# tkwa/iit

Hardware: AMD Instinct MI355X
Metric: IIT (base,source) intervened pairs/sec, IOI GPT-2-small, IOI_ModelPair IIT+strict+behavior step (higher is better)
Workload: dtype bf16; 1 GPU; model=gpt2-small 12L/768d/12H (TL GPT-2 cfg, LNPre, gelu_new, V=50257), global_batch=256, seq_len=16, parallelism=dp1, engine=native, graphs=True

## Files before the change

csrc/gemm_glds_body.h:

```cpp
#pragma once
#include <type_traits>

#include "common.h"

namespace {

enum : int { E_BF16 = 0, E_BF16_BIAS3 = 1, E_F32_RESID = 2, E_GELU = 3, E_DGELU = 4, E_F32_ACC = 5,
             E_F32_STORE = 7, E_GELU_ERF = 8, E_DGELU_ERF = 9, E_BF16_CS = 10 };

struct G2Args {
  const __bf16* A;
  const __bf16* B;
  void* C;
  void* C2;
  const float* bias0;
  const float* bias1;
  const float* bias2;
  const float* resid;
  long lda, ldb, ldc, ldc2, ldr;
  int M, N, K, bias_cols;
  int k_per_split;
  float* csum;
  float* ws;
  int* counters;
// ... 90 lines not shown
};

__device__ __forceinline__ unsigned lds_addr(const char* p) {
  return (unsigned)(uintptr_t)(const __attribute__((address_space(3))) char*)p;
}

template <bool KMAJ, int R>
struct Panels {
  static constexpr bool ON = KMAJ && (R > 128 || R % 64 != 0);
  static constexpr int PR = !ON ? R : (R % 64 == 0 ? 64 : 32);
  static constexpr int NP = R / PR;
};

template <bool KMAJ, int R, int NW = 4, int BK = 64, bool LEAN = false>
struct OperandStager {
  static constexpr bool PANELS = Panels<KMAJ, R>::ON;
  static constexpr int NP = Panels<KMAJ, R>::NP;
  static constexpr int PR = Panels<KMAJ, R>::PR;
  static constexpr int N = NP * Stager<KMAJ, PR, NW, BK, LEAN>::N;
  Stager<KMAJ, PR, NW, BK, LEAN> st[NP];

  __device__ __forceinline__ void init(const __bf16* base, long ld, int r0g, int kbeg, int wave, int lane) {
#pragma unroll
    for (int q = 0; q < NP; ++q) st[q].init(base, ld, r0g + q * PR, kbeg, wave, lane);
  }
  __device__ __forceinline__ void stage(int kt, char* img) const {
#pragma unroll
    for (int q = 0; q < NP; ++q) st[q].stage(kt, img + q * PR * BK * 2);
  }
};

typedef int i32x4 __attribute__((ext_vector_type(4)));
template <bool KMAJ> struct RawFrag;
template <> struct RawFrag<false> { i32x4 v; };
template <> struct RawFrag<true> { i16x4 lo, hi; };

template <bool KMAJ, int R, int BK = 64>
__device__ __forceinline__ void frag_issue(const char* img, int row0, int kbase, int lane, RawFrag<KMAJ>& f) {
  if constexpr (!KMAJ) {
    const int row = row0 + (lane & 15);
    const int c = (kbase >> 3) + (lane >> 4);
    const unsigned a = lds_addr(img + row * (BK * 2) + ((c ^ kcont_swz<BK>(row)) << 4));
    asm volatile("ds_read_b128 %0, %1" : "=v"(f.v) : "v"(a));
  } else {
    const int g = lane >> 4, q = (lane >> 2) & 3, pp = lane & 3;
    const int kr = kbase + 8 * g + q;
    const int col = row0 + 4 * pp;
    const unsigned a0 = lds_addr(img + kr * (R * 2) + ((((col >> 4) ^ kmaj_swz<R>(kr))) << 5) + ((col & 15) << 1));
    asm volatile("ds_read_b64_tr_b16 %0, %1" : "=v"(f.lo) : "v"(a0));
    asm volatile("ds_read_b64_tr_b16 %0, %1 offset:%2" : "=v"(f.hi) : "v"(a0), "i"(4 * R * 2));
  }
}

template <bool KMAJ, int R, int BK = 64>
__device__ __forceinline__ void frag_issue_t(const char* img, int row0, int kbase, int lane, RawFrag<KMAJ>& f) {
  using PN = Panels<KMAJ, R>;
  if constexpr (PN::ON) {
    frag_issue<KMAJ, PN::PR, BK>(img + (row0 / PN::PR) * PN::PR * BK * 2, row0 % PN::PR, kbase, lane, f);
  } else {
    frag_issue<KMAJ, R, BK>(img, row0, kbase, lane, f);
  }
}

template <bool KMAJ>
__device__ __forceinline__ bf16x8 frag_use(const RawFrag<KMAJ>& f) {
  if constexpr (!KMAJ) {
    return __builtin_bit_cast(bf16x8, f.v);
  } else {
    const i16x8 w = __builtin_shufflevector(f.lo, f.hi, 0, 1, 2, 3, 4, 5, 6, 7);
    return __builtin_bit_cast(bf16x8, w);
  }
}

template <bool TR>
__device__ __forceinline__ f32x4 mfma_tile(const bf16x8 a, const bf16x8 b, const f32x4 c) {
  if constexpr (TR) return __builtin_amdgcn_mfma_f32_16x16x32_bf16(b, a, c, 0, 0, 0);
  else return __builtin_amdgcn_mfma_f32_16x16x32_bf16(a, b, c, 0, 0, 0);
}

__device__ __forceinline__ int xcd_remap(int bid, int nwg) {
  const int xcd = bid % 8;
  const int q = nwg / 8, r = nwg % 8;
  return (xcd < r ? xcd * (q + 1) : r * (q + 1) + (xcd - r) * q) + bid / 8;
}

__device__ __forceinline__ void grouped_tile(int t, int tiles_m, int tiles_n, int& tm, int& tn, int GM = 8) {
  const int per_group = GM * tiles_n;
  const int first_m = (t / per_group) * GM;
  const int gsize = min(tiles_m - first_m, GM);
  const int r = t % per_group;
  tm = first_m + r % gsize;
  tn = r / gsize;
}

__device__ __forceinline__ float gelu_new_dev(float x) { return gelu_new_f(x); }

__device__ __forceinline__ void add8v(float* v, const float4 x, const float4 y) {
  v[0] += x.x; v[1] += x.y; v[2] += x.z; v[3] += x.w;
  v[4] += y.x; v[5] += y.y; v[6] += y.z; v[7] += y.w;
}

__device__ __forceinline__ void add8(float* v, const float* b) {
  const float4 x = *(const float4*)b, y = *(const float4*)(b + 4);
  v[0] += x.x; v[1] += x.y; v[2] += x.z; v[3] += x.w;
  v[4] += y.x; v[5] += y.y; v[6] += y.z; v[7] += y.w;
}

__device__ __forceinline__ void store16(void* dst, const f32x4 x, int mode) {
  if (mode == 1) {
    __builtin_nontemporal_store(x, (f32x4*)dst);
  } else if (mode == 2) {
    asm volatile("global_store_dwordx4 %0, %1, off sc1" ::"v"(dst), "v"(x) : "memory");
  } else {
    *(f32x4*)dst = x;
  }
}

__device__ __forceinline__ void store8_bf16(void* dst, const float* v, int mode = 0) {
  bf16x8 o;
#pragma unroll
  for (int e = 0; e < 8; ++e) o[e] = f2bf(v[e]);
  store16(dst, __builtin_bit_cast(f32x4, o), mode);
}

__device__ __forceinline__ void store8_f32(void* dst, const float* v, int mode = 0) {
  store16(dst, f32x4{v[0], v[1], v[2], v[3]}, mode);
  store16((float*)dst + 4, f32x4{v[4], v[5], v[6], v[7]}, mode);
}

template <int L>
__device__ __forceinline__ void wait_tiles(int tiles_in_flight) {
  constexpr int CAP = 63 / L;
  if (tiles_in_flight > CAP) tiles_in_flight = CAP;
  if (tiles_in_flight >= 7) asm volatile("s_waitcnt vmcnt(%0)" ::"n"((7 * L) < 63 ? 7 * L : 63) : "memory");
  else if (tiles_in_flight == 6) asm volatile("s_waitcnt vmcnt(%0)" ::"n"((6 * L) < 63 ? 6 * L : 63) : "memory");
  else if (tiles_in_flight == 5) asm volatile("s_waitcnt vmcnt(%0)" ::"n"((5 * L) < 63 ? 5 * L : 63) : "memory");
  else if (tiles_in_flight == 4) asm volatile("s_waitcnt vmcnt(%0)" ::"n"((4 * L) < 63 ? 4 * L : 63) : "memory");
  else if (tiles_in_flight == 3) asm volatile("s_waitcnt vmcnt(%0)" ::"n"((3 * L) < 63 ? 3 * L : 63) : "memory");
  else if (tiles_in_flight == 2) asm volatile("s_waitcnt vmcnt(%0)" ::"n"(2 * L) : "memory");
  else if (tiles_in_flight == 1) asm volatile("s_waitcnt vmcnt(%0)" ::"n"(L) : "memory");
  else asm volatile("s_waitcnt vmcnt(0)" ::: "memory");
}

template <int BM, int BN, int NS, int NW, int BK, int OCC>
struct GldsSmem {
  static constexpr int STAGE = (BM + BN) * BK * 2;
  static constexpr int EPS = BN + 4;
  static constexpr int LDS_BUDGET = 160 * 1024 / OCC;
  static constexpr int ECH = BM * EPS * 4 > LDS_BUDGET ? 2 : 1;
  static constexpr int EPI_BYTES = BM / ECH * EPS * 4;
  static constexpr int BYTES = NS * STAGE > EPI_BYTES ? NS * STAGE : EPI_BYTES;
};

template <int BM, int BN, int EPI, int NT, int ECH, int EPS, class WriteAcc>
__device__ __forceinline__ void glds_epilogue(const G2Args& p, char* smem, const int m0, const int n0, const int lin,
                                              WriteAcc&& write_acc) {
  const int tid = threadIdx.x, lane = tid & 63, wave = tid >> 6;
  constexpr int NW = NT / 64;
  float* E = (float*)smem;
  constexpr int ER = BM / ECH;
  constexpr int CPR = BN / 8;
  constexpr int ITEMS = (ER * CPR + NT - 1) / NT;
  constexpr bool PF32 = EPI == E_F32_RESID || EPI == E_F32_ACC;
  constexpr bool PF16 = EPI == E_DGELU || EPI == E_DGELU_ERF;
  float sq = 0.f;
  float cpiv = 0.f, cs1 = 0.f, cs2 = 0.f;
  for (int ch = 0; ch < ECH; ++ch) {
  float4 pf[PF32 ? 2 * ITEMS : 1];
  bf16x8 pb[PF16 ? ITEMS : 1];
#pragma unroll
  for (int k = 0; k < ITEMS; ++k) {
    const int id = tid + k * NT;
    if (id < ER * CPR) {
      const int row = m0 + ch * ER + id / CPR, col = n0 + (id % CPR) * 8;
      if constexpr (EPI == E_F32_RESID) {
        const float* src = p.resid + (long)row * p.ldr + col;
        pf[2 * k] = *(const float4*)src;
        pf[2 * k + 1] = *(const float4*)(src + 4);
      } else if constexpr (EPI == E_F32_ACC) {
        const float* src = (const float*)p.C + (long)row * p.ldc + col;
        pf[2 * k] = *(const float4*)src;
        pf[2 * k + 1] = *(const float4*)(src + 4);
      } else if constexpr (PF16) {
        pb[k] = *(const bf16x8*)((const __bf16*)p.C2 + (long)row * p.ldc2 + col);
      }
    }
  }
  __syncthreads();
  write_acc(E, ch);
  __syncthreads();
#pragma unroll
  for (int k = 0; k < ITEMS; ++k) {
    const int id = tid + k * NT;
    if (id >= ER * CPR) break;
    const int lr = id / CPR, lc = (id % CPR) * 8;
    const int row = m0 + ch * ER + lr, col = n0 + lc;
    float v[8];
    {
      const float4 x = *(const float4*)(E + lr * EPS + lc), y = *(const float4*)(E + lr * EPS + lc + 4);
      v[0] = x.x; v[1] = x.y; v[2] = x.z; v[3] = x.w; v[4] = y.x; v[5] = y.y; v[6] = y.z; v[7] = y.w;
    }
    if constexpr (EPI == E_BF16) {
      if (p.bias0) add8(v, p.bias0 + col);
      store8_bf16((__bf16*)p.C + (long)row * p.ldc + col, v, p.store_mode);
    } else if constexpr (EPI == E_BF16_CS) {
      if (p.bias0) add8(v, p.bias0 + col);
      store8_bf16((__bf16*)p.C + (long)row * p.ldc + col, v, p.store_mode);
#pragma unroll
      for (int e = 0; e < 8; ++e) v[e] = bf2f(f2bf(v[e]));
      *(float4*)(E + lr * EPS + lc) = make_float4(v[0], v[1], v[2], v[3]);
      *(float4*)(E + lr * EPS + lc + 4) = make_float4(v[4], v[5], v[6], v[7]);
    } else if constexpr (EPI == E_BF16_BIAS3) {
      const int w = col / p.bias_cols, o = col - w * p.bias_cols;
      const float* bb = w == 0 ? p.bias0 : (w == 1 ? p.bias1 : p.bias2);
      if (bb) add8(v, bb + o);
      store8_bf16((__bf16*)p.C + (long)row * p.ldc + col, v, p.store_mode);
    } else if constexpr (EPI == E_F32_RESID) {
      if (p.bias0) add8(v, p.bias0 + col);
      add8v(v, pf[2 * k], pf[2 * k + 1]);
      store8_f32((float*)p.C + (long)row * p.ldc + col, v, p.store_mode);
    } else if constexpr (EPI == E_GELU || EPI == E_GELU_ERF) {
      if (p.bias0) add8(v, p.bias0 + col);
      if (p.C2) store8_bf16((__bf16*)p.C2 + (long)row * p.ldc2 + col, v, p.store_mode);
      float g[8];
#pragma unroll
      for (int e = 0; e < 8; ++e) {
        const float x = bf2f(f2bf(v[e]));
        g[e] = EPI == E_GELU ? gelu_new_dev(x) : gelu_erf_f(x);
      }
      store8_bf16((__bf16*)p.C + (long)row * p.ldc + col, g, p.store_mode);
    } else if constexpr (EPI == E_DGELU || EPI == E_DGELU_ERF) {
      const bf16x8 pr = pb[k];
#pragma unroll
      for (int e = 0; e < 8; ++e) {
        const float x = bf2f(pr[e]);
        v[e] = bf2f(f2bf(v[e] * (EPI == E_DGELU ? gelu_new_grad_f(x) : gelu_erf_grad_f(x))));
      }
      store8_bf16((__bf16*)p.C + (long)row * p.ldc + col, v, p.store_mode);
      if (p.csum) {
        *(float4*)(E + lr * EPS + lc) = make_float4(v[0], v[1], v[2], v[3]);
        *(float4*)(E + lr * EPS + lc + 4) = make_float4(v[4], v[5], v[6], v[7]);
      }
    } else if constexpr (EPI == E_F32_ACC) {
      float* dst = (float*)p.C + (long)row * p.ldc + col;
      add8v(v, pf[2 * k], pf[2 * k + 1]);
      store8_f32(dst, v, p.store_mode);
    } else {
      if (p.bias0) add8(v, p.bias0 + col);
      store8_f32((float*)p.C + (long)row * p.ldc + col, v, p.store_mode);
      if (p.gsq) {
#pragma unroll
        for (int e = 0; e < 8; ++e) sq += v[e] * v[e];
      }
    }
  }
  if constexpr (EPI == E_DGELU || EPI == E_DGELU_ERF) {
    if (p.csum) {
      __syncthreads();
      constexpr int G = NT / BN > 0 ? NT / BN : 1;
      for (int c = tid; c < BN * G; c += NT) {
        const int col = c % BN, g = c / BN;
        float s[8] = {0.f, 0.f, 0.f, 0.f, 0.f, 0.f, 0.f, 0.f};
#pragma unroll
        for (int r0 = g; r0 < ER; r0 += 8 * G)
#pragma unroll
          for (int u = 0; u < 8; ++u)
            if (r0 + u * G < ER) s[u] += E[(r0 + u * G) * EPS + col];
        atomicAdd(p.csum + n0 + col, ((s[0] + s[1]) + (s[2] + s[3])) + ((s[4] + s[5]) + (s[6] + s[7])));
      }
    }
  }
  if constexpr (EPI == E_BF16_CS) {
    __syncthreads();
    static_assert(NT % BN == 0, "column groups");
    constexpr int G = NT / BN;
    const int col = tid % BN, g = tid / BN;
    if (ch == 0) cpiv = E[col];
    for (int r = g; r < ER; r += G) {
      const float d = E[r * EPS + col] - cpiv;
      cs1 += d;
      cs2 = __builtin_fmaf(d, d, cs2);
    }
  }
  }
  if constexpr (EPI == E_BF16_CS) {
    constexpr int G = NT / BN;
    float* red = (float*)smem;
    __syncthreads();
    red[tid] = cs1;
    red[NT + tid] = cs2;
    __syncthreads();
    if (tid < BN) {
      float a = 0.f, b = 0.f;
#pragma unroll
      for (int g = 0; g < G; ++g) {
        a += red[g * BN + tid];
        b += red[NT + g * BN + tid];
      }
      const long T = p.M / BM, tm = m0 / BM, c = n0 + tid;
      p.cstat[c * T + tm] = cpiv;
      p.cstat[((long)p.N + c) * T + tm] = a;
      p.cstat[(2L * p.N + c) * T + tm] = b;
    }
  }
  if constexpr (EPI == E_F32_STORE) {
    if (p.gsq) {
      sq = wave_sum(sq);
      float* red = (float*)smem;
      __syncthreads();
      if (lane == 0) red[wave] = sq;
      __syncthreads();
      if (tid == 0) {
        float t = 0.f;
#pragma unroll
        for (int w = 0; w < NW; ++w) t += red[w];
        atomicAdd(p.gsq + (lin & 63), t);
      }
    }
  }
}

template <int BM, int BN, int NS, bool AKM, bool BKM, int EPI, int NW, int BK = 64, int OCC = 1, bool LEAN = false,
          class ASTG = void, class BSTG = void>
__device__ __forceinline__ void gemm_glds_body(const G2Args& p, const int lin, const int nlin, const int split,
                                               const int nsplit, char* smem) {
  using SA = std::conditional_t<std::is_void_v<ASTG>, OperandStager<AKM, BM, NW, BK, LEAN>, ASTG>;
  using SB = std::conditional_t<std::is_void_v<BSTG>, OperandStager<BKM, BN, NW, BK, LEAN>, BSTG>;
  constexpr int HALVES = BK / 64;
  constexpr int NT = NW * 64;
  constexpr int WMR = NW / 2;
  constexpr int WM = BM / WMR, WN = BN / 2;
  constexpr int TM = WM / 16, TN = WN / 16;
  constexpr int A_BYTES = BM * BK * 2, B_BYTES = BN * BK * 2;
  constexpr int STAGE = A_BYTES + B_BYTES;
  constexpr int LOADS = SA::N + SB::N;
  using SM = GldsSmem<BM, BN, NS, NW, BK, OCC>;
  constexpr int EPS = SM::EPS;
  constexpr int ECH = SM::ECH;
  static_assert(SM::BYTES <= SM::LDS_BUDGET, "LDS budget");
  static_assert(STAGE == SM::STAGE, "stage size");

  constexpr bool TR = EPI != E_F32_ACC;
  const int tid = threadIdx.x, lane = tid & 63, wave = tid >> 6;
  const int wm = wave >> 1, wn = wave & 1;
  const int tiles_n = p.N / BN;
  const int t = xcd_remap(lin, nlin);
  int tm, tn;
  grouped_tile(t, p.M / BM, tiles_n, tm, tn, p.group_m > 0 ? p.group_m : 8);
  const int m0 = tm * BM, n0 = tn * BN;
  const int kbeg = split * p.k_per_split;
  const int nt = p.k_per_split / BK;
  const bool prof_on = p.prof != nullptr && tid == 0;
  const int prof_slot = split * nlin + lin;
  if (prof_on) {
    p.prof[(long)prof_slot * 64 + 63] = wall_clock64();
    prof_mark(p.prof, prof_slot, 0, true);
  }

  f32x4 acc[TM][TN];
  constexpr bool CS = AKM && BKM && (EPI == E_F32_ACC || EPI == E_F32_STORE);
  const bool do_cs = CS && p.bsum != nullptr && tm == 0 && wm == 0;
  float cs[CS ? TN : 1];
#pragma unroll
  for (int j = 0; j < (CS ? TN : 1); ++j) cs[j] = 0.f;
#pragma unroll
  for (int i = 0; i < TM; ++i)
#pragma unroll
    for (int j = 0; j < TN; ++j) acc[i][j] = f32x4{0.f, 0.f, 0.f, 0.f};

  RawFrag<AKM> ca[TM], na[TM];
  RawFrag<BKM> cb[TN], nb[TN];
  SA stA;
  SB stB;
  if constexpr (std::is_void_v<ASTG>) stA.init(p.A, p.lda, m0, kbeg, wave, lane);
  else stA.init(p, m0, kbeg, wave, lane);
  if constexpr (std::is_void_v<BSTG>) stB.init(p.B, p.ldb, n0, kbeg, wave, lane);
  else stB.init(p, n0, kbeg, wave, lane);
#pragma unroll
  for (int s = 0; s < NS; ++s)
    if (s < nt) {
      char* buf = smem + s * STAGE;
      stA.stage(s, buf);
      stB.stage(s, buf + A_BYTES);
    }
  wait_tiles<LOADS>(min(NS - 1, nt - 1));
  __builtin_amdgcn_s_barrier();
  prof_mark(p.prof, prof_slot, 1, prof_on);
#pragma unroll
  for (int i = 0; i < TM; ++i) frag_issue_t<AKM, BM, BK>(smem, wm * WM + i * 16, 0, lane, ca[i]);
#pragma unroll
  for (int j = 0; j < TN; ++j) frag_issue_t<BKM, BN, BK>(smem + A_BYTES, wn * WN + j * 16, 0, lane, cb[j]);

  for (int kt = 0; kt < nt; ++kt) {
    const char* sa = smem + (kt % NS) * STAGE;
    const char* sb = sa + A_BYTES;
#pragma unroll
    for (int h = 0; h < HALVES; ++h) {
    asm volatile("s_waitcnt lgkmcnt(0)" ::: "memory");
    __builtin_amdgcn_sched_barrier(0);
#pragma unroll
    for (int i = 0; i < TM; ++i) frag_issue_t<AKM, BM, BK>(sa, wm * WM + i * 16, h * 64 + 32, lane, na[i]);
#pragma unroll
    for (int j = 0; j < TN; ++j) frag_issue_t<BKM, BN, BK>(sb, wn * WN + j * 16, h * 64 + 32, lane, nb[j]);
    __builtin_amdgcn_sched_barrier(0);
    {
      bf16x8 a[TM], b[TN];
#pragma unroll
      for (int i = 0; i < TM; ++i) a[i] = frag_use<AKM>(ca[i]);
#pragma unroll
      for (int j = 0; j < TN; ++j) b[j] = frag_use<BKM>(cb[j]);
#pragma unroll
      for (int i = 0; i < TM; ++i)
#pragma unroll
        for (int j = 0; j < TN; ++j) acc[i][j] = mfma_tile<TR>(a[i], b[j], acc[i][j]);
      if constexpr (CS) {
        if (do_cs) {
#pragma unroll
          for (int j = 0; j < TN; ++j) {
            const i32x4 w = __builtin_bit_cast(i32x4, b[j]);
            float t = 0.f;
#pragma unroll
            for (int q = 0; q < 4; ++q)
              t += __builtin_bit_cast(float, (unsigned)w[q] << 16) + __builtin_bit_cast(float, (unsigned)w[q] & 0xffff0000u);
            cs[j] += t;
          }
        }
      }
    }
    __builtin_amdgcn_sched_barrier(0);
    asm volatile("s_waitcnt lgkmcnt(0)" ::: "memory");
    __builtin_amdgcn_sched_barrier(0);
    if (h + 1 < HALVES) {
#pragma unroll
      for (int i = 0; i < TM; ++i) frag_issue_t<AKM, BM, BK>(sa, wm * WM + i * 16, (h + 1) * 64, lane, ca[i]);
#pragma unroll
      for (int j = 0; j < TN; ++j) frag_issue_t<BKM, BN, BK>(sb, wn * WN + j * 16, (h + 1) * 64, lane, cb[j]);
    } else if (kt + 1 < nt) {
      wait_tiles<LOADS>(min(NS - 2, nt - 2 - kt));
      __builtin_amdgcn_s_barrier();
      if (kt + 2 < 61) prof_mark(p.prof, prof_slot, kt + 2, prof_on);
      if (kt + NS < nt) {
        char* buf = smem + (kt % NS) * STAGE;
        stA.stage(kt + NS, buf);
        stB.stage(kt + NS, buf + A_BYTES);
      }
      const char* ta = smem + ((kt + 1) % NS) * STAGE;
#pragma unroll
      for (int i = 0; i < TM; ++i) frag_issue_t<AKM, BM, BK>(ta, wm * WM + i * 16, 0, lane, ca[i]);
#pragma unroll
      for (int j = 0; j < TN; ++j) frag_issue_t<BKM, BN, BK>(ta + A_BYTES, wn * WN + j * 16, 0, lane, cb[j]);
    }
    __builtin_amdgcn_sched_barrier(0);
    {
      bf16x8 a[TM], b[TN];
#pragma unroll
      for (int i = 0; i < TM; ++i) a[i] = frag_use<AKM>(na[i]);
#pragma unroll
      for (int j = 0; j < TN; ++j) b[j] = frag_use<BKM>(nb[j]);
#pragma unroll
      for (int i = 0; i < TM; ++i)
#pragma unroll
        for (int j = 0; j < TN; ++j) acc[i][j] = mfma_tile<TR>(a[i], b[j], acc[i][j]);
      if constexpr (CS) {
        if (do_cs) {
#pragma unroll
          for (int j = 0; j < TN; ++j) {
            const i32x4 w = __builtin_bit_cast(i32x4, b[j]);
            float t = 0.f;
#pragma unroll
            for (int q = 0; q < 4; ++q)
              t += __builtin_bit_cast(float, (unsigned)w[q] << 16) + __builtin_bit_cast(float, (unsigned)w[q] & 0xffff0000u);
            cs[j] += t;
          }
        }
      }
    }
    __builtin_amdgcn_sched_barrier(0);
    }
  }
  prof_mark(p.prof, prof_slot, 61, prof_on);
  if constexpr (CS) {
    if (do_cs) {
#pragma unroll
      for (int j = 0; j < TN; ++j) {
        float v = cs[j];
        v += __shfl_xor(v, 16);
        v += __shfl_xor(v, 32);
        if (lane < 16) atomicAdd(p.bsum + n0 + wn * WN + j * 16 + lane, v);
      }
    }
  }
  if constexpr (EPI == E_F32_ACC || EPI == E_F32_STORE || EPI == E_F32_RESID || EPI == E_BF16 || EPI == E_BF16_CS) {
    if (p.ws != nullptr) {
      const long tile_elems = (long)BM * BN;
      f32x4* mine = (f32x4*)(p.ws + ((long)split * nlin + t) * tile_elems);
#pragma unroll
      for (int i = 0; i < TM; ++i)
#pragma unroll
        for (int j = 0; j < TN; ++j)
          asm volatile("global_store_dwordx4 %0, %1, off sc1" ::"v"(mine + (i * TN + j) * NT + tid), "v"(acc[i][j])
                       : "memory");
      asm volatile("s_waitcnt vmcnt(0)" ::: "memory");
      __syncthreads();
      int* flag = (int*)smem;
      if (tid == 0) {
        const int last = atomicAdd(p.counters + t, 1) == nsplit - 1;
        if (last) __hip_atomic_store(p.counters + t, 0, __ATOMIC_RELAXED, __HIP_MEMORY_SCOPE_AGENT);
        flag[0] = last;
      }
      __syncthreads();
      if (!flag[0]) return;
      f32x4 sum[TM][TN];
#pragma unroll
      for (int i = 0; i < TM; ++i)
#pragma unroll
        for (int j = 0; j < TN; ++j) sum[i][j] = f32x4{0.f, 0.f, 0.f, 0.f};
      for (int sp = 0; sp < nsplit; ++sp) {
        if (sp == split) {
#pragma unroll
          for (int i = 0; i < TM; ++i)
#pragma unroll
            for (int j = 0; j < TN; ++j) sum[i][j] += acc[i][j];
          continue;
        }
        const f32x4* other = (const f32x4*)(p.ws + ((long)sp * nlin + t) * tile_elems);
        f32x4 v[TM][TN];
#pragma unroll
        for (int i = 0; i < TM; ++i)
#pragma unroll
          for (int j = 0; j < TN; ++j)
            asm volatile("global_load_dwordx4 %0, %1, off sc1" : "=v"(v[i][j]) : "v"(other + (i * TN + j) * NT + tid)
                         : "memory");
        asm volatile("s_waitcnt vmcnt(0)" ::: "memory");
#pragma unroll
        for (int i = 0; i < TM; ++i)
#pragma unroll
          for (int j = 0; j < TN; ++j) sum[i][j] += v[i][j];
      }
#pragma unroll
      for (int i = 0; i < TM; ++i)
#pragma unroll
        for (int j = 0; j < TN; ++j) acc[i][j] = sum[i][j];
    }
  }
  if constexpr (EPI == E_F32_ACC) {
    if (nsplit > 1 && p.ws == nullptr) {
#pragma unroll
      for (int i = 0; i < TM; ++i)
#pragma unroll
        for (int j = 0; j < TN; ++j) {
          const int col = n0 + wn * WN + j * 16 + (lane & 15);
          const int row = m0 + wm * WM + i * 16 + 4 * (lane >> 4);
#pragma unroll
          for (int r = 0; r < 4; ++r) unsafeAtomicAdd((float*)p.C + (long)(row + r) * p.ldc + col, acc[i][j][r]);
        }
      return;
    }
  }
  glds_epilogue<BM, BN, EPI, NT, ECH, SM::EPS>(p, smem, m0, n0, lin, [&](float* E, int ch) {
    if (wm / (WMR / ECH) == ch) {
#pragma unroll
      for (int i = 0; i < TM; ++i)
#pragma unroll
        for (int j = 0; j < TN; ++j) {
          if constexpr (TR) {
            const int col = wn * WN + j * 16 + 4 * (lane >> 4);
            const int row = (wm % (WMR / ECH)) * WM + i * 16 + (lane & 15);
            *(f32x4*)(E + row * EPS + col) = acc[i][j];
          } else {
            const int col = wn * WN + j * 16 + (lane & 15);
            const int row = (wm % (WMR / ECH)) * WM + i * 16 + 4 * (lane >> 4);
#pragma unroll
            for (int r = 0; r < 4; ++r) E[(row + r) * EPS + col] = acc[i][j][r];
          }
        }
    }
  });
  if (p.prof != nullptr) {
    asm volatile("s_waitcnt vmcnt(0)" ::: "memory");
    __syncthreads();
    prof_mark(p.prof, prof_slot, 62, prof_on);
    if (prof_on) p.prof[(long)prof_slot * 64 + 60] = wall_clock64();
  }
}

}
```

csrc/kernels.hip:

```cpp
#include "common.h"
#include <stdlib.h>

__global__ void embed_pos_fwd_kernel(const long* __restrict__ tok, const float* __restrict__ WE,
                                     const float* __restrict__ Wpos, float* __restrict__ out, int T, int S, int d) {
  const int t = blockIdx.x;
  if (t >= T) return;
  const long v = tok[t];
  const int s = t % S;
  const float4* e = (const float4*)(WE + v * (long)d);
  const float4* p = (const float4*)(Wpos + (long)s * d);
  float4* o = (float4*)(out + (long)t * d);
  for (int i = threadIdx.x; i < d / 4; i += blockDim.x) {
    float4 a = e[i], b = p[i];
    o[i] = make_float4(a.x + b.x, a.y + b.y, a.z + b.z, a.w + b.w);
  }
}

IIT_EXPORT int iit_embed_pos_fwd(const long* tok, const float* WE, const float* Wpos, float* out, int T, int S,
                                 int d, void* stream) {
  hipLaunchKernelGGL(embed_pos_fwd_kernel, dim3(T), dim3(d >= 256 ? 64 : 64), 0, (hipStream_t)stream, tok, WE, Wpos,
                     out, T, S, d);
  return hipGetLastError();
}

// ... 815 lines not shown
  const int P = dh + 1, SP = S + 1;
  float* q = sm;
  float* k = q + S * P;
  float* v = k + S * P;
  float* g = v + S * P;
  float* pm = g + S * P;
  float* ds = pm + S * SP;
  for (int i = lane; i < S * dh; i += 64) {
    const int s = i / dh, e = i % dh;
    const __bf16* r = qkv + (row0 + s) * ld_qkv + h * dh + e;
    q[s * P + e] = bf2f(r[0]);
    k[s * P + e] = bf2f(r[HD]);
    v[s * P + e] = bf2f(r[2 * HD]);
    g[s * P + e] = bf2f(dz[(row0 + s) * ld_dz + h * dh + e]);
  }
  __syncthreads();
  for (int i = lane; i < S * S; i += 64) {
    const int qi = i / S, kj = i % S;
    float p = 0.f, dp = 0.f;
    if (!causal || kj <= qi) {
      float sc = 0.f;
      for (int e = 0; e < dh; ++e) sc += q[qi * P + e] * k[kj * P + e];
      p = __expf(sc * scale - lse[(long)bh * S + qi]);
      for (int e = 0; e < dh; ++e) dp += g[qi * P + e] * v[kj * P + e];
    }
    pm[qi * SP + kj] = p;
    ds[qi * SP + kj] = dp;
  }
  __syncthreads();
  for (int qi = lane; qi < S; qi += 64) {
    float dsum = 0.f;
    for (int kj = 0; kj < S; ++kj) dsum += pm[qi * SP + kj] * ds[qi * SP + kj];
    for (int kj = 0; kj < S; ++kj) ds[qi * SP + kj] = pm[qi * SP + kj] * (ds[qi * SP + kj] - dsum) * scale;
  }
  __syncthreads();
  for (int i = lane; i < S * dh; i += 64) {
    const int s = i / dh, e = i % dh;
    float dq = 0.f, dk = 0.f, dv = 0.f;
    for (int j = 0; j < S; ++j) {
      dq += ds[s * SP + j] * k[j * P + e];
      dk += ds[j * SP + s] * q[j * P + e];
      dv += pm[j * SP + s] * g[j * P + e];
    }
    __bf16* r = dqkv + (row0 + s) * ld_qkv + h * dh + e;
    r[0] = f2bf(dq);
    r[HD] = f2bf(dk);
    r[2 * HD] = f2bf(dv);
  }
}

IIT_EXPORT int iit_attn_small_bwd(const void* qkv, const void* dz, const float* lse, void* dqkv,
                                  unsigned long long head_mask, int B, int S, int H, int dh, long ld_qkv, long ld_dz,
                                  float scale, int causal, void* stream) {
  if (S > 64 || dh > 128) return (int)hipErrorInvalidValue;
  const size_t lds = (size_t)(4 * S * (dh + 1) + 2 * S * (S + 1)) * sizeof(float);
  if (lds > kAttnSmallLdsMax) return (int)hipErrorInvalidValue;
  hipLaunchKernelGGL(attn_small_bwd_kernel, dim3(B * H), dim3(64), lds, (hipStream_t)stream, (const __bf16*)qkv,
                     (const __bf16*)dz, lse, (__bf16*)dqkv, head_mask, B, S, H, dh, ld_qkv, ld_dz, scale, causal);
  return hipGetLastError();
}

__device__ __forceinline__ void online_add(float& m, float& s, int& mi, float v, int i) {
  if (v > m) {
    s = s * __expf(m - v) + 1.f;
    m = v;
    mi = i;
  } else {
    s += __expf(v - m);
  }
}

__device__ __forceinline__ void online_merge(float& m, float& s, int& mi, float om, float os, int oi) {
  if (om > m || (om == m && oi < mi)) {
    s = os + (m == -INFINITY ? 0.f : s * __expf(m - om));
    m = om;
    mi = oi;
  } else {
    s += (om == -INFINITY ? 0.f : os * __expf(om - m));
  }
}

__global__ __launch_bounds__(1024) void ce_fwd_kernel(const float* __restrict__ logits, long ld, const long* __restrict__ labels,
                                                      float* __restrict__ loss, float* __restrict__ lse_out,
                                                      long* __restrict__ amax, int V) {
  __shared__ float sm_m[16], sm_s[16];
  __shared__ int sm_i[16];
  const int row = blockIdx.x, tid = threadIdx.x, lane = tid & 63, w = tid >> 6;
  const float* x = logits + (long)row * ld;
  float m = -INFINITY, s = 0.f;
  int mi = 0x7fffffff;
  int head = 0;
  if ((((uintptr_t)x) & 15) == 0) {
    const int v4 = V / 4;
    for (int i = tid; i < v4; i += 1024) {
      const float4 q = ((const float4*)x)[i];
      online_add(m, s, mi, q.x, 4 * i);
      online_add(m, s, mi, q.y, 4 * i + 1);
      online_add(m, s, mi, q.z, 4 * i + 2);
      online_add(m, s, mi, q.w, 4 * i + 3);
    }
    head = v4 * 4;
  }
  for (int i = head + tid; i < V; i += 1024) online_add(m, s, mi, x[i], i);
#pragma unroll
  for (int o = 32; o > 0; o >>= 1) {
    const float om = __shfl_xor(m, o, 64), os = __shfl_xor(s, o, 64);
    const int oi = __shfl_xor(mi, o, 64);
    online_merge(m, s, mi, om, os, oi);
  }
  if (lane == 0) { sm_m[w] = m; sm_s[w] = s; sm_i[w] = mi; }
  __syncthreads();
  if (tid == 0) {
    for (int j = 1; j < 16; ++j) online_merge(m, s, mi, sm_m[j], sm_s[j], sm_i[j]);
    const float l = m + __logf(s);
    if (lse_out) lse_out[row] = l;
    if (loss && labels) loss[row] = l - x[labels[row]];
    if (amax) amax[row] = mi;
  }
}

IIT_EXPORT int iit_ce_fwd(const float* logits, long ld, const long* labels, float* loss, float* lse, long* amax, int R,
                          int V, void* stream) {
  hipLaunchKernelGGL(ce_fwd_kernel, dim3(R), dim3(1024), 0, (hipStream_t)stream, logits, ld, labels, loss, lse, amax, V);
  return hipGetLastError();
}

template <typename OUT>
__global__ __launch_bounds__(256) void ce_bwd_kernel(const float* __restrict__ logits, long ld, const long* __restrict__ labels,
                                                     const float* __restrict__ lse, const float* __restrict__ gscale,
                                                     float inv_rows, OUT* __restrict__ out, long ld_out, int V,
                                                     __bf16* __restrict__ out16) {
  const int row = blockIdx.y;
  const int i = blockIdx.x * 256 + threadIdx.x;
  if (i >= ld_out) return;
  float v = 0.f;
  if (i < V) {
    const float p = __expf(logits[(long)row * ld + i] - lse[row]);
    v = (p - (i == labels[row] ? 1.f : 0.f)) * gscale[0] * inv_rows;
  }
  out[(long)row * ld_out + i] = (OUT)v;
  if (out16) out16[(long)row * ld_out + i] = f2bf(v);
}

IIT_EXPORT int iit_ce_bwd(const float* logits, long ld, const long* labels, const float* lse, const float* gscale,
                          float inv_rows, void* out, long ld_out, int R, int V, int out_bf16, void* out16,
                          void* stream) {
  dim3 grid((unsigned)((ld_out + 255) / 256), R);
  if (out_bf16)
    hipLaunchKernelGGL(ce_bwd_kernel<__bf16>, grid, dim3(256), 0, (hipStream_t)stream, logits, ld, labels, lse, gscale,
                       inv_rows, (__bf16*)out, ld_out, V, (__bf16*)nullptr);
  else
    hipLaunchKernelGGL(ce_bwd_kernel<float>, grid, dim3(256), 0, (hipStream_t)stream, logits, ld, labels, lse, gscale,
                       inv_rows, (float*)out, ld_out, V, (__bf16*)out16);
  return hipGetLastError();
}

struct Span {
  long start4;
  long local4;
  int len4;
  int pad;
};

__global__ __launch_bounds__(256) void sumsq_span_kernel(const float* __restrict__ g, const Span* __restrict__ spans,
                                                         int nspans, float* __restrict__ part, int do_norm,
                                                         int* __restrict__ step, float* __restrict__ gsq) {
  __shared__ float sm[4];
  if (blockIdx.x == 0 && threadIdx.x == 0 && step) step[0] += 1;
  float s = 0.f;
  if (gsq && blockIdx.x == 0 && threadIdx.x < 64) {
    s = gsq[threadIdx.x];
    gsq[threadIdx.x] = 0.f;
  }
  if (!do_norm) return;
  const float4* g4 = (const float4*)g;
  for (int e = blockIdx.x; e < nspans; e += gridDim.x) {
    const Span sp = spans[e];
    for (int i = threadIdx.x; i < sp.len4; i += 256) {
      const float4 v = g4[sp.local4 + i];
      s += (v.x * v.x + v.y * v.y) + (v.z * v.z + v.w * v.w);
    }
  }
  s = wave_sum(s);
  if ((threadIdx.x & 63) == 0) sm[threadIdx.x >> 6] = s;
  __syncthreads();
  if (threadIdx.x == 0) part[blockIdx.x] = sm[0] + sm[1] + sm[2] + sm[3];
}

template <bool NT, int U>
__global__ __launch_bounds__(256) void adam_span_kernel(float* __restrict__ p, const float* __restrict__ g,
                                                        float* __restrict__ m, float* __restrict__ v,
                                                        __bf16* __restrict__ mirror, const Span* __restrict__ spans,
                                                        int nspans, const float* __restrict__ part, int nparts,
                                                        float clip, float lr, float b1, float b2, float eps, float wd,
                                                        const float* __restrict__ hyper, int* __restrict__ step,
                                                        int* __restrict__ skipped) {
  if (hyper) {
    lr = hyper[0];
    b1 = hyper[1];
    b2 = hyper[2];
    eps = hyper[3];
    wd = hyper[4];
  }
  __shared__ float coef_s;
  __shared__ int bad_s;
  if (threadIdx.x < 64) {
    float s = 0.f;
    if (clip > 0.f || skipped)
      for (int i = threadIdx.x; i < nparts; i += 64) s += part[i];
    s = wave_sum(s);
    if (threadIdx.x == 0) {
      coef_s = clip > 0.f ? fminf(1.f, clip / (sqrtf(s) + 1e-6f)) : 1.f;
      bad_s = skipped != nullptr && !isfinite(s);
    }
  }
  __syncthreads();
  if (bad_s) {
    if (blockIdx.x == 0 && threadIdx.x == 0) {
      step[0] -= 1;
      skipped[0] += 1;
    }
    return;
  }
  const float coef = coef_s;
  const float t = (float)step[0];
  const float bc1 = 1.f - powf(b1, t);
  const float bc2_sqrt = sqrtf(1.f - powf(b2, t));
  const float stepsz = lr / bc1;
  const float4* g4 = (const float4*)g;
  float4* p4 = (float4*)p;
  float4* m4 = (float4*)m;
  float4* v4 = (float4*)v;
  for (int e = blockIdx.x; e < nspans; e += gridDim.x) {
    const Span sp = spans[e];
    for (int j0 = threadIdx.x; j0 < sp.len4; j0 += 256 * U) {
      float4 gg[U], pp[U], mm[U], vv[U];
#pragma unroll
      for (int u = 0; u < U; ++u) {
        const int j = j0 + u * 256;
        if (j < sp.len4) {
          const long i = sp.start4 + j;
          const long li = sp.local4 + j;
          pp[u] = p4[i];
          if (NT) {
            gg[u] = __builtin_bit_cast(float4, __builtin_nontemporal_load((const f32x4*)g4 + li));
            mm[u] = __builtin_bit_cast(float4, __builtin_nontemporal_load((const f32x4*)m4 + li));
            vv[u] = __builtin_bit_cast(float4, __builtin_nontemporal_load((const f32x4*)v4 + li));
          } else {
            gg[u] = g4[li];
            mm[u] = m4[li];
            vv[u] = v4[li];
          }
        }
      }
#pragma unroll
      for (int u = 0; u < U; ++u) {
        const int j = j0 + u * 256;
        if (j >= sp.len4) break;
        const long i = sp.start4 + j;
        const long li = sp.local4 + j;
        float* gs = (float*)&gg[u];
        float* ps = (float*)&pp[u];
        float* ms = (float*)&mm[u];
        float* vs = (float*)&vv[u];
#pragma unroll
        for (int k = 0; k < 4; ++k) {
          float gr = gs[k] * coef;
          if (wd != 0.f) gr += wd * ps[k];
          ms[k] = b1 * ms[k] + (1.f - b1) * gr;
          vs[k] = b2 * vs[k] + (1.f - b2) * gr * gr;
          ps[k] -= stepsz * ms[k] / (sqrtf(vs[k]) / bc2_sqrt + eps);
        }
        p4[i] = pp[u];
        if (NT) {
          __builtin_nontemporal_store(__builtin_bit_cast(f32x4, mm[u]), (f32x4*)m4 + li);
          __builtin_nontemporal_store(__builtin_bit_cast(f32x4, vv[u]), (f32x4*)v4 + li);
        } else {
          m4[li] = mm[u];
          v4[li] = vv[u];
        }
        if (mirror) {
          bf16x4 o = {f2bf(ps[0]), f2bf(ps[1]), f2bf(ps[2]), f2bf(ps[3])};
          ((bf16x4*)mirror)[i] = o;
        }
      }
    }
  }
}

IIT_EXPORT int iit_adam_flat(float* p, float* g, float* m, float* v, void* mirror, const void* spans, int nspans,
                             float* part, int nparts, float clip, float lr, float b1, float b2, float eps, float wd,
                             const float* hyper, int* step, int* skipped, const void* sq_spans, int n_sq_spans,
                             float* gsq, void* stream) {
  hipStream_t s = (hipStream_t)stream;
  const bool norm = clip > 0.f || skipped != nullptr;
  const Span* sp = (const Span*)spans;
  const Span* ssp = sq_spans ? (const Span*)sq_spans : sp;
  hipLaunchKernelGGL(sumsq_span_kernel, dim3(norm ? nparts : 1), dim3(256), 0, s, g, ssp,
                     sq_spans ? n_sq_spans : nspans, part, (int)norm, step, gsq);
  static const int max_blocks = [] {
    const char* e = getenv("IIT_ADAM_MAX_BLOCKS");
    return e ? atoi(e) : 65536;
  }();
  const int blocks = min(nspans, max_blocks);
  static const int nt = [] {
    const char* e = getenv("IIT_ADAM_NT");
// ... 565 lines not shown
```

iit_amd/model_pairs/iit_behavior_model_pair.py:

```python
from __future__ import annotations

import torch
from torch import Tensor

from ..core.metric import MetricStore, MetricStoreCollection, MetricType
from .iit_model_pair import IITModelPair, labels_of


class IITBehaviorModelPair(IITModelPair):
    def __init__(self, hl_model, ll_model, corr, training_args=None):
        defaults = {
            "lr": 0.001,
            "atol": 5e-2,
            "early_stop": True,
            "use_single_loss": False,
            "iit_weight": 1.0,
            "behavior_weight": 1.0,
        }
        super().__init__(hl_model, ll_model, corr=corr, training_args={**defaults, **(training_args or {})})
        self.wandb_method = "iit_and_behavior"

    def _categorical(self) -> bool:
        try:
            return bool(self.hl_model.is_categorical())
        except AttributeError:
            return True

    @property
    def loss_fn(self):
        if self._loss_fn_override is not None:
            return self._loss_fn_override
        return torch.nn.CrossEntropyLoss() if self._categorical() else torch.nn.MSELoss()

    @loss_fn.setter
    def loss_fn(self, value):
        self._loss_fn_override = value

    @staticmethod
    def make_train_metrics():
        return MetricStoreCollection([
            MetricStore("train/iit_loss", MetricType.LOSS),
            MetricStore("train/behavior_loss", MetricType.LOSS),
        ])

    @staticmethod
    def make_test_metrics():
        return MetricStoreCollection([
            MetricStore("val/iit_loss", MetricType.LOSS),
            MetricStore("val/IIA", MetricType.ACCURACY),
            MetricStore("val/accuracy", MetricType.ACCURACY),
        ])

    def get_behaviour_loss_over_batch(self, base_input, loss_fn):
        base_x, base_y = base_input[0], base_input[1]
        output = self.ll_forward(base_x)
        if output.dim() > 1 and output.shape[0] == 1:
            return loss_fn(output, base_y)
        return loss_fn(output.squeeze(), base_y)

    def step_on_loss(self, loss: Tensor, optimizer) -> None:
        optimizer.zero_grad()
        self.backward(loss)
        self.clip_grad_fn(optimizer)
        self.optimizer_step(optimizer)

    def run_train_step(self, base_input, ablation_input, loss_fn, optimizer):
        args = self.training_args
        hl_node = self.sample_hl_name()

        def iit():
            return self.get_IIT_loss_over_batch(base_input, ablation_input, hl_node, loss_fn) * args["iit_weight"]

        def behavior():
            return self.get_behaviour_loss_over_batch(base_input, loss_fn) * args["behavior_weight"]

        if args["use_single_loss"]:
            def total():
                parts = {"iit": iit(), "behavior": behavior()}
                return parts["iit"] + parts["behavior"], parts

            _, parts = self.run_phase(("single", hl_node.name), total, optimizer, self.step_on_loss)
            return {"train/iit_loss": parts["iit"], "train/behavior_loss": parts["behavior"]}
        iit_loss = self.run_phase(("iit", hl_node.name), iit, optimizer, self.step_on_loss)
        behavior_loss = self.run_phase(("behavior",), behavior, optimizer, self.step_on_loss)
        return {"train/iit_loss": iit_loss, "train/behavior_loss": behavior_loss}

    def run_eval_step(self, base_input, ablation_input, loss_fn):
        atol = self.training_args["atol"]
        hl_node = self.sample_hl_name()
        hl_output, ll_output = self.do_intervention(base_input, ablation_input, hl_node)
        loss = loss_fn(ll_output, hl_output)
        if self._categorical():
            top1 = torch.argmax(ll_output, dim=-1)
            iia = (top1 == labels_of(hl_output, ll_output)).float().mean()
        else:
            iia = ((ll_output - hl_output).abs() < atol).float().mean()
        base_x, base_y = base_input[0], base_input[1]
        output = self.ll_forward(base_x)
        if self._categorical():
            accuracy = (torch.argmax(output, dim=-1) == labels_of(base_y, output)).float().mean()
        else:
            accuracy = ((output.squeeze() - base_y).abs() < atol).float().mean()
        return {"val/iit_loss": loss.detach(), "val/IIA": iia, "val/accuracy": accuracy}
```

iit_amd/model_pairs/strict_iit_model_pair.py:

```python
from __future__ import annotations

from ..core.metric import MetricStore, MetricStoreCollection, MetricType
from ..core.nodes import LLNode
from ..utils import node_picker
from .iit_behavior_model_pair import IITBehaviorModelPair


class StrictIITModelPair(IITBehaviorModelPair):
    def __init__(self, hl_model, ll_model, corr, training_args=None):
        defaults = {
            "batch_size": 256,
            "lr": 0.001,
            "num_workers": 0,
            "use_single_loss": False,
            "iit_weight": 1.0,
            "behavior_weight": 1.0,
            "strict_weight": 1.0,
            "clip_grad_norm": 1.0,
        }
        super().__init__(hl_model, ll_model, corr=corr, training_args={**defaults, **(training_args or {})})
        self.nodes_not_in_circuit = node_picker.get_nodes_not_in_circuit(self.ll_model, self.corr)

    @staticmethod
    def make_train_metrics():
        return MetricStoreCollection([
            MetricStore("train/iit_loss", MetricType.LOSS),
            MetricStore("train/behavior_loss", MetricType.LOSS),
            MetricStore("train/strict_loss", MetricType.LOSS),
        ])

    def sample_ll_node(self) -> LLNode:
        return self.rng.choice(self.nodes_not_in_circuit)

    def get_strict_loss_over_batch(self, base_input, ablation_input, ll_node: LLNode, loss_fn):
        base_x, base_y = base_input[0], base_input[1]
        out = self.ll_paired_intervention(base_x, ablation_input[0], [ll_node])
        if out is None:
            self.ll_cache = self.ll_source_cache(ablation_input[0], [ll_node])
            out = self.ll_intervened_forward(base_x, [ll_node])
        if out.dim() > 1 and out.shape[0] == 1:
            return loss_fn(out, base_y)
        return loss_fn(out.squeeze(), base_y)

    def run_train_step(self, base_input, ablation_input, loss_fn, optimizer):
        args = self.training_args
        hl_node = self.sample_hl_name()

        def iit():
            return self.get_IIT_loss_over_batch(base_input, ablation_input, hl_node, loss_fn) * args["iit_weight"]

        if args["use_single_loss"]:
            ll_node = self.sample_ll_node()

            def total():
                parts = {"iit": iit(),
                         "strict": self.get_strict_loss_over_batch(base_input, ablation_input, ll_node, loss_fn)
                         * args["strict_weight"],
                         "behavior": self.get_behaviour_loss_over_batch(base_input, loss_fn) * args["behavior_weight"]}
                return parts["iit"] + parts["behavior"] + parts["strict"], parts

            _, parts = self.run_phase(("single", hl_node.name, ll_node.name, repr(ll_node.index)), total, optimizer,
                                      self.step_on_loss)
            return {"train/iit_loss": parts["iit"], "train/behavior_loss": parts["behavior"],
                    "train/strict_loss": parts["strict"]}
        iit_loss = self.run_phase(("iit", hl_node.name), iit, optimizer, self.step_on_loss)
        ll_node = self.sample_ll_node()
        strict_loss = self.run_phase(
            ("strict", ll_node.name, repr(ll_node.index)),
            lambda: self.get_strict_loss_over_batch(base_input, ablation_input, ll_node, loss_fn) * args["strict_weight"],
            optimizer, self.step_on_loss)
        behavior_loss = self.run_phase(
            ("behavior",), lambda: self.get_behaviour_loss_over_batch(base_input, loss_fn) * args["behavior_weight"],
            optimizer, self.step_on_loss)
        return {"train/iit_loss": iit_loss, "train/behavior_loss": behavior_loss, "train/strict_loss": strict_loss}
```

iit_amd/ops/build.py:

```python
from __future__ import annotations

import hashlib
import os
import subprocess
import sys

ROOT = os.path.dirname(os.path.dirname(os.path.dirname(os.path.abspath(__file__))))
CSRC = os.path.join(ROOT, "csrc")
OUT_DIR = os.path.join(ROOT, "iit_amd", "_native")
LIB = os.path.join(OUT_DIR, "libiit_hip.so")
OBJ_CACHE = os.path.join(ROOT, "build", "objcache")
SOURCES = ["gemm.hip", "gemm_glds.hip", "gemm_dual.hip", "gemm_8ph.hip", "gemm_4w.hip", "conv_nhwc.hip", "kernels.hip", "attn_mfma.hip", "flash_attn.hip", "llama_ops.hip",
           "splice.hip", "ioi_hl.hip", "bn_nhwc.hip", "gemm_f32.hip"]
EXTRA_FLAGS = {"gemm_glds.hip": ["-mllvm", "-amdgpu-mfma-vgpr-form"], "conv_nhwc.hip": ["-mllvm", "-amdgpu-mfma-vgpr-form"], "gemm_dual.hip": ["-mllvm", "-amdgpu-mfma-vgpr-form"],
               "gemm_8ph.hip": ["-mllvm", "-amdgpu-mfma-vgpr-form"]}
HEADERS = ["common.h", "gemm_glds_body.h", "gemm_w4.h", "splice_spec.h"]
ARCH = os.environ.get("IIT_OFFLOAD_ARCH", "gfx950")


def _hipcc() -> str:
    for c in (os.environ.get("HIPCC"), "/opt/rocm/bin/hipcc"):
        if c and os.path.exists(c):
            return c
    return "hipcc"


def sources():
    return [os.path.join(CSRC, s) for s in SOURCES if os.path.exists(os.path.join(CSRC, s))]


def source_hash() -> str:
    h = hashlib.sha256()
    for p in sources() + [os.path.join(CSRC, h) for h in HEADERS]:
        with open(p, "rb") as f:
            h.update(f.read())
    h.update(ARCH.encode())
    h.update(repr(sorted(EXTRA_FLAGS.items())).encode())
    return h.hexdigest()[:16]


def is_up_to_date() -> bool:
    stamp = LIB + ".stamp"
    return os.path.exists(LIB) and os.path.exists(stamp) and open(stamp).read().strip() == source_hash()


def _obj_key(src: str) -> str:
    h = hashlib.sha256()
    for p in [src] + [os.path.join(CSRC, x) for x in HEADERS]:
        with open(p, "rb") as f:
            h.update(f.read())
    h.update(ARCH.encode())
    h.update(repr(EXTRA_FLAGS.get(os.path.basename(src), [])).encode())
    return h.hexdigest()[:16]


def build(force: bool = False, verbose: bool = False) -> str:
    if not force and is_up_to_date():
        return LIB
    os.makedirs(OBJ_CACHE, exist_ok=True)
    objs = []
    procs = []
    for src in sources():
        obj = os.path.join(OBJ_CACHE, f"{os.path.basename(src)}.{_obj_key(src)}.o")
        objs.append(obj)
        if os.path.exists(obj) and not force:
            continue
        cmd = [_hipcc(), f"--offload-arch={ARCH}", "-O3", "-std=c++17", "-fPIC", "-munsafe-fp-atomics",
               "-I", CSRC, "-c", src, "-o", obj + ".tmp"] + EXTRA_FLAGS.get(os.path.basename(src), [])
        procs.append((cmd, obj, subprocess.Popen(cmd, stdout=subprocess.PIPE, stderr=subprocess.STDOUT)))
    for cmd, obj, p in procs:
        out, _ = p.communicate()
        if p.returncode != 0:
            raise RuntimeError(f"hipcc failed: {' '.join(cmd)}\n{out.decode(errors='replace')}")
        os.replace(obj + ".tmp", obj)
        if verbose and out:
            print(out.decode(errors="replace"))
    tmp = LIB + ".tmp"
    cmd = [_hipcc(), f"--offload-arch={ARCH}", "-shared", "-fPIC", "-o", tmp] + objs
    res = subprocess.run(cmd, stdout=subprocess.PIPE, stderr=subprocess.STDOUT)
    if res.returncode != 0:
        raise RuntimeError(f"link failed: {res.stdout.decode(errors='replace')}")
    os.replace(tmp, LIB)
    keep = set(objs)
    for f in os.listdir(OBJ_CACHE):
        if os.path.join(OBJ_CACHE, f) not in keep:
            os.remove(os.path.join(OBJ_CACHE, f))
    with open(LIB + ".stamp", "w") as f:
        f.write(source_hash())
    return LIB


if __name__ == "__main__":
    print(build(force="--force" in sys.argv, verbose=True))
```

iit_amd/ops/gemm_dispatch.py:

```python
from __future__ import annotations

import os
import re
from typing import Dict, Optional, Tuple

import torch
import torch.nn.functional as F

from . import hip_kernels as K

POLICY = os.environ.get("IIT_GEMM", "auto")
DECISIONS: Dict[Tuple, Tuple[str, Dict[str, float]]] = {}
FORCE: Dict[Tuple, str] = {}
TIMING = None
BF16, F32 = torch.bfloat16, torch.float32
_BLAS_OK = {}
_BLAS_SELECTED = False


def select_graph_safe_blas() -> None:
    global _BLAS_SELECTED
    if _BLAS_SELECTED or not torch.cuda.is_available():
        return
    _BLAS_SELECTED = True
# ... 131 lines not shown
        if bias is None:
            torch.mm(a, b, out=c)
        else:
            torch.addmm(bias, a, b, out=c)
    elif epi == K.EPI_F32_RESID:
        c = _as(C, M, N, ldc)
        _addmm_f32(c, _as(resid, M, N, ldr), a, b)
        if bias0 is not None:
            c.add_(bias0.reshape(-1)[:N])
    elif epi in (K.EPI_GELU, K.EPI_GELU_ERF):
        pre = _as(C2, M, N, ldc2) if C2 is not None else torch.empty(M, N, dtype=BF16, device=A.device)
        torch.addmm(bias0.reshape(-1)[:N].to(BF16), a, b, out=pre)
        _gelu_into(pre, _as(C, M, N, ldc), erf=epi == K.EPI_GELU_ERF)
    elif epi in (K.EPI_DGELU, K.EPI_DGELU_ERF):
        tmp = torch.mm(a, b)
        K.dgelu(tmp, _as(aux, M, N, ldc2).contiguous(), _as(C, M, N, ldc), erf=epi == K.EPI_DGELU_ERF)
    elif epi == K.EPI_F32_ACC:
        c = _as(C, M, N, ldc)
        _addmm_f32(c, c, a, b)
    elif epi == K.EPI_F32_STORE:
        c = _as(C, M, N, ldc)
        if bias0 is not None:
            _addmm_f32(c, bias0.reshape(-1)[:N].float(), a, b)
        else:
            _mm_f32_into(c, a, b)
    else:
        raise NotImplementedError(epi)


def _blas_supported(epi, C) -> bool:
    if epi == K.EPI_F32_ACC_QKV:
        return False
    if epi in (K.EPI_DGELU, K.EPI_DGELU_ERF):
        return True
    return True


def _scratch(t, rows, ld):
    if t is None:
        return None
    return torch.zeros(rows * ld, dtype=t.dtype, device=t.device)


def _time(fn, reps: int = 10) -> float:
    fn()
    torch.cuda.synchronize()
    s, e = torch.cuda.Event(enable_timing=True), torch.cuda.Event(enable_timing=True)
    try:
        from ..engine.graphs import _CaptureGC
        g = torch.cuda.CUDAGraph()
        with _CaptureGC(collect=False), torch.cuda.graph(g, capture_error_mode="thread_local"):
            for _ in range(reps):
                fn()
        g.replay()
        s.record()
        g.replay()
        e.record()
        e.synchronize()
        return s.elapsed_time(e) / reps * 1e3
    except Exception:
        torch.cuda.synchronize()
        s.record()
        for _ in range(reps):
            fn()
        e.record()
        e.synchronize()
        return s.elapsed_time(e) / reps * 1e3


def _blas16(A, B, C, M, N, Kd, lda, ldb, ldc, mode, epi, bias0, resid, ldr):
    a, b = _operands(A, B, M, N, Kd, lda, ldb, mode)
    y = torch.mm(a, b)
    bias = None if bias0 is None else bias0.reshape(-1)[:N].float().contiguous()
    if epi == K.EPI_F32_RESID:
        K.add_bf16(C, ldc, resid, ldr, y, N, bias, M, N)
    else:
        K.add_bf16(C, ldc, C, ldc, y, N, None, M, N)


_BLAS16_EPIS = (K.EPI_F32_RESID, K.EPI_F32_ACC)


_EXCLUDE = [re.compile(x) for x in os.environ.get("IIT_GEMM_EXCLUDE", "").split(";" if ";" in
                                                                                 os.environ.get("IIT_GEMM_EXCLUDE", "")
                                                                                 else ",") if x]
_TRACE = os.environ.get("IIT_GEMM_TRACE", "0") == "1"
_TAIL_LIBRARY = os.environ.get("IIT_GEMM_TAIL_LIBRARY", "0") == "1"
_TRACED = set()


def _excluded(name: str, key=None) -> bool:
    if name == "hip":
        return False
    tagged = f"{name}@{key!r}"
    return any(r.fullmatch(tagged) if "@" in r.pattern else r.fullmatch(name) for r in _EXCLUDE)


def _candidates(A, B, C, C2, M, N, Kd, lda, ldb, ldc, mode, epi, bias0, bias1, bias2, resid, ldr, aux, ldc2,
                bias_cols, qkv, splits, blas_bias, policy, csum_box=None):
    calls = _candidates_plain(A, B, C, C2, M, N, Kd, lda, ldb, ldc, mode, epi, bias0, bias1, bias2, resid, ldr, aux,
                              ldc2, bias_cols, qkv, splits, blas_bias, policy, csum_box)
    if _EXCLUDE:
        calls = {n: f for n, f in calls.items() if not _excluded(n)}
    if csum_box is not None:
        for name in list(calls):
            if not name.startswith("glds"):
                calls[name] = lambda c=C, c2=C2, c3=None, f=calls[name]: (
                    f(c, c2, c3), K_.colsum_accum(c, ldc, csum_box[0], M, N))
    return calls


def _candidates_plain(A, B, C, C2, M, N, Kd, lda, ldb, ldc, mode, epi, bias0, bias1, bias2, resid, ldr, aux, ldc2,
                      bias_cols, qkv, splits, blas_bias, policy, csum_box):
    det = deterministic()
    if det:
        splits = 1
    hip_call = lambda c=C, c2=C2, c3=None: K_.gemm(
        A, B, c, M=M, N=N, K=Kd, lda=lda, ldb=ldb, ldc=ldc, mode=mode, epi=epi, C2=c2, C3=c3, bias0=bias0,
        bias1=bias1, bias2=bias2, resid=resid, ldr=ldr, aux=aux, ldc2=ldc2, bias_cols=bias_cols, qkv=qkv,
        splits=splits)
    calls = {"hip": hip_call}
    if not _blas_supported(epi, C):
        return calls
    calls["blas"] = lambda c=C, c2=C2, c3=None: _blas(A, B, c, M, N, Kd, lda, ldb, ldc, mode, epi, c2, c3,
                                                     bias0, bias1, bias2, resid, ldr, aux, ldc2, bias_cols, qkv,
                                                     blas_bias)
    if policy in ("auto", "glds") and A.is_cuda:
        split_opts = (1,)
        if epi == K_.EPI_F32_ACC and (M // 64) * (N // 64) < 1024 and not det:
            split_opts = (1, 2, 4, 8, 16) if (M // 64) * (N // 64) < 64 else (1, 2, 4)
        dg = epi in (K_.EPI_DGELU, K_.EPI_DGELU_ERF)
        for tile in K_.GLDS_DISPATCH_TILES:
            for sp in split_opts:
                if K_.gemm_glds_ok(A, B, C, M=M, N=N, K=Kd, lda=lda, ldb=ldb, ldc=ldc, mode=mode, epi=epi,
                                   C2=aux if dg else C2, resid=resid, ldc2=ldc2, ldr=ldr, bias_cols=bias_cols,
                                   tile=tile, splits=sp):
                    calls[f"glds{tile}" + (f"k{sp}" if sp > 1 else "")] = \
                        lambda c=C, c2=C2, c3=None, t=tile, sp=sp, bs=None, sq=None: K_.gemm_glds(
                            A, B, c, M=M, N=N, K=Kd, lda=lda, ldb=ldb, ldc=ldc, mode=mode, epi=epi,
                            C2=aux if dg else c2, bias0=bias0, bias1=bias1, bias2=bias2, resid=resid, ldc2=ldc2,
                            ldr=ldr, bias_cols=bias_cols, tile=t, splits=sp,
                            csum=csum_box[0] if csum_box is not None else None, bsum=bs, gsq=sq)
            if (mode == 3 and epi in (K_.EPI_F32_ACC, K_.EPI_F32_STORE)) or \
                    (mode == 2 and epi == K_.EPI_F32_RESID and Kd >= 2048 and bias_cols == 0):
                for sp in (2, 4):
                    if Kd // sp < 256 or not K_.gemm_glds_ok(A, B, C, M=M, N=N, K=Kd, lda=lda, ldb=ldb, ldc=ldc,
                                                             mode=mode, epi=epi, resid=resid, ldr=ldr, tile=tile,
                                                             splits=sp, reduce=True):
                        continue
                    calls[f"glds{tile}r{sp}"] = lambda c=C, c2=C2, c3=None, t=tile, sp=sp, bs=None, sq=None: \
                        K_.gemm_glds(A, B, c, M=M, N=N, K=Kd, lda=lda, ldb=ldb, ldc=ldc, mode=mode, epi=epi,
                                     bias0=bias0, resid=resid, ldr=ldr, tile=t, splits=sp, reduce=True, bsum=bs,
                                     gsq=sq)
    if epi in _BLAS16_EPIS:
        calls["blas16"] = lambda c=C, c2=C2, c3=None: _blas16(A, B, c, M, N, Kd, lda, ldb, ldc, mode, epi,
                                                             bias0, resid, ldr)
    mode_ss = _SPLIT_STORE
    if _SPLIT_STORE_KEY and (M, N, Kd) != _SPLIT_STORE_KEY:
        mode_ss = ""
    if (mode_ss and not det and epi in (K_.EPI_F32_STORE, K_.EPI_F32_RESID) and A.is_cuda and mode in (0, 2, 3)
            and Kd >= 256 and Kd % 64 == 0 and ((M + 63) // 64) * ((N + 63) // 64) < 64):
        sp = 1 if mode_ss in ("nosplit", "atomic1") else min(16, Kd // 64)

        def split_store(c=C, c2=C2, c3=None):
            cv = _as(c, M, N, ldc)
            b = None if bias0 is None else bias0.reshape(-1)[:N].float()
            if epi == K_.EPI_F32_RESID:
                r = _as(resid, M, N, ldr)
                if b is None:
                    cv.copy_(r)
                else:
                    torch.add(r, b, out=cv)
            elif b is not None:
                cv.copy_(b.expand(M, N))
            else:
                cv.zero_()
            if mode_ss == "sync" and not torch.cuda.is_current_stream_capturing():
                torch.cuda.synchronize()
            K_.gemm(A, B, c, M=M, N=N, K=Kd, lda=lda, ldb=ldb, ldc=ldc, mode=mode, epi=K_.EPI_F32_ACC, splits=sp,
                    atomic=mode_ss == "atomic1")

        calls["s+hip"] = split_store
    return calls


_SPLIT_STORE = os.environ.get("IIT_GEMM_SPLIT_STORE", "")
_FREEZE = os.environ.get("IIT_GEMM_FREEZE", "0") == "1"


def _frozen_miss(key) -> None:
    if _FREEZE:
        raise RuntimeError(f"IIT_GEMM_FREEZE=1: GEMM problem {key!r} is not in the decision table "
                           f"({os.environ.get('IIT_GEMM_TABLE', _TABLE_PATH)}); export one with IIT_GEMM_TABLE_EXPORT")
_SPLIT_STORE_KEY = tuple(int(x) for x in os.environ.get("IIT_GEMM_SPLIT_STORE_KEY", "").split(",") if x) or None


def _shift(t, off: int):
    if t is None:
        return None
    n = t.untyped_storage().nbytes() // t.element_size() - t.storage_offset() - off
    return torch.as_strided(t, (n,), (1,), t.storage_offset() + off)


RAGGED = {}


def _ragged_split(A, B, C, *, M, N, K, lda, ldb, mode, epi, C2, bias0, resid, aux, bsum=None, gsq=None):
    if epi in (K_.EPI_BF16, K_.EPI_F32_STORE, K_.EPI_F32_ACC) and N >= 4096 and N % 128:
        n0 = N // 128 * 128
        boff = n0 if mode & K_.MODE_BKM else n0 * ldb
        return [dict(A=A, B=B, C=C, M=M, N=n0, K=K, C2=C2, bias0=bias0, resid=resid, aux=aux, bsum=bsum, gsq=gsq),
                dict(A=A, B=_shift(B, boff), C=_shift(C, n0), M=M, N=N - n0, K=K, C2=_shift(C2, n0),
                     bias0=_shift(bias0, n0), resid=_shift(resid, n0), aux=_shift(aux, n0), bsum=_shift(bsum, n0),
                     gsq=gsq)]
    if epi == K_.EPI_F32_ACC and K >= 16384 and K % 1024:
        k0 = K // 1024 * 1024
        aoff = k0 * lda if mode & K_.MODE_AKM else k0
        boff = k0 * ldb if mode & K_.MODE_BKM else k0
        return [dict(A=A, B=B, C=C, M=M, N=N, K=k0, C2=C2, bias0=bias0, resid=resid, aux=aux, bsum=bsum, gsq=gsq),
                dict(A=_shift(A, aoff), B=_shift(B, boff), C=C, M=M, N=N, K=K - k0, C2=C2, bias0=None,
                     resid=resid, aux=aux, bsum=bsum, gsq=gsq)]
    return None


def gemm(A, B, C, *, M, N, K: int, lda, ldb, ldc, mode=0, epi=0, C2=None, C3=None, bias0=None, bias1=None,
         bias2=None, resid=None, ldr=0, aux=None, ldc2=0, bias_cols=0, qkv=(0, 0, 0), splits=None, blas_bias=None,
         fresh: bool = False, colsum=None, bsum=None, gsq=None, _decide_only: bool = False,
         _no_split: bool = False, _tail: bool = False):
    Kd = K
    if not _BLAS_SELECTED:
        select_graph_safe_blas()
        enable_tuned_library_gemms()
    policy = POLICY
    if policy in ("auto", "glds") and A.is_cuda and qkv[0] == 0 and colsum is None and not _no_split:
        parts = _ragged_split(A, B, C, M=M, N=N, K=K, lda=lda, ldb=ldb, mode=mode, epi=epi, C2=C2, bias0=bias0,
                              resid=resid, aux=aux, bsum=bsum, gsq=gsq)
        if parts is not None:
            bulk, tail = parts

            def run(kw, decide=False, tail=False):
                kw = dict(kw)
                return gemm(kw.pop("A"), kw.pop("B"), kw.pop("C"), lda=lda, ldb=ldb, ldc=ldc, mode=mode, epi=epi,
                            ldr=ldr, ldc2=ldc2, blas_bias=None, fresh=fresh, _decide_only=decide, _tail=tail, **kw)

            rkey = (M, N, K, mode, epi, bias0 is not None, fresh, deterministic())
            split = RAGGED.get(rkey)
            if split is None:
                shipped = _ragged_table().get(repr(rkey))
                if shipped is not None:
                    split = RAGGED[rkey] = (bool(shipped), float("nan"), [])
            if split is None and _FREEZE:
                split = RAGGED[rkey] = (True, float("nan"), [])
            if split is None and not torch.cuda.is_current_stream_capturing():
                whole = gemm(A, B, C, M=M, N=N, K=K, lda=lda, ldb=ldb, ldc=ldc, mode=mode, epi=epi, C2=C2, C3=C3,
                             bias0=bias0, bias1=bias1, bias2=bias2, resid=resid, ldr=ldr, aux=aux, ldc2=ldc2,
                             bias_cols=bias_cols, qkv=qkv, splits=splits, blas_bias=blas_bias, fresh=fresh,
                             bsum=bsum, gsq=gsq, _decide_only=True, _no_split=True)
                pieces = [run(bulk, True), run(tail, True, True)]
                split = RAGGED[rkey] = (None not in pieces and whole is not None and sum(pieces) < whole,
                                        whole, pieces)
            if split is not None and split[0]:
                choice = run(bulk)
                run(tail, tail=True)
                return choice
    fresh = fresh and epi == K_.EPI_F32_STORE and bias0 is None
    assert colsum is None or epi in (K_.EPI_DGELU, K_.EPI_DGELU_ERF), "fused column sums need a DGELU epilogue"
    box = [colsum] if colsum is not None else None
    args = (A, B, C, C2, M, N, Kd, lda, ldb, ldc, mode, epi, bias0, bias1, bias2, resid, ldr, aux, ldc2, bias_cols,
            qkv, splits, blas_bias, policy)
    calls = _candidates(*args, csum_box=box)
    if _tail and not _TAIL_LIBRARY:
        calls = {n: f for n, f in calls.items() if not n.startswith("blas")}
    hip_call = calls["hip"]
    if _decide_only and (policy != "auto" or (len(calls) == 1 and not _tail)):
        return None
    if bsum is not None or gsq is not None:
        assert bsum is None or mode == 3, "fused bias sums are the column sums of a weight gradient's dY"
        assert gsq is None or epi == K_.EPI_F32_STORE, "fused norm sums are of a stored gradient"
        def _run(name):
            if name.startswith("glds"):
                calls[name](C, C2, C3, bs=bsum, sq=gsq)
            else:
                calls[name](C, C2, C3)
                if bsum is not None:
                    K_.colsum_accum(B, ldb, bsum, Kd, N)
                if gsq is not None:
                    K_.sumsq_2d(C, ldc, M, N, gsq)
            return name
    else:
        def _run(name):
            calls[name](C, C2, C3)
            return name
    if policy == "hip" or (len(calls) == 1 and not _decide_only):
        _run("hip")
        return None
    if fresh:
        acc = _candidates(A, B, C, C2, M, N, Kd, lda, ldb, ldc, mode, K_.EPI_F32_ACC, None, None, None, resid, ldr,
                          aux, ldc2, bias_cols, qkv, None, blas_bias, policy)
        for name, f in acc.items():
            if _tail and not _TAIL_LIBRARY and name.startswith("blas"):
                continue
            calls["z+" + name] = lambda c=C, c2=C2, c3=None, f=f: (_as(c, M, N, ldc).zero_(), f(c, c2, c3))
    if policy == "glds":
        glds = [k for k in calls if k.startswith("glds")]
        _run(glds[0] if glds else "hip")
        return None
    if policy in calls:
        _run(policy)
        return None
    key = (M, N, Kd, mode, epi, bias0 is not None, fresh or (colsum is not None), deterministic())
    if _EXCLUDE:
        calls = {n: f for n, f in calls.items() if not _excluded(n, key)}
    choice = DECISIONS.get(key)
    if choice is None:
        shipped = None if _decide_only else _table().get(repr(key))
        if shipped in calls:
            choice = DECISIONS[key] = (shipped, {shipped: float("nan")})
    if choice is None:
        if torch.cuda.is_current_stream_capturing():
            if _decide_only:
                return None
            _run("hip")
            return None
        _frozen_miss(key)
        sc = _scratch(C, M, max(ldc, N))
        sc2 = _scratch(C2, M, max(ldc2, N))
        sc3 = _scratch(C3, M, max(ldc, N))
        if box is not None:
            box[0] = torch.zeros_like(colsum)
        timed = calls
        if bsum is not None or gsq is not None:
            sc_bs = torch.zeros_like(bsum) if bsum is not None else None
            sc_sq = torch.zeros_like(gsq) if gsq is not None else None

            def _passes(c):
                if sc_bs is not None:
                    K_.colsum_accum(B, ldb, sc_bs, Kd, N)
                if sc_sq is not None:
                    K_.sumsq_2d(c, ldc, M, N, sc_sq)

            timed = {name: (lambda c, c2, c3, f=f: f(c, c2, c3, bs=sc_bs, sq=sc_sq)) if name.startswith("glds") else
                     (lambda c, c2, c3, f=f: (f(c, c2, c3), _passes(c)))
                     for name, f in calls.items()}
        try:
            times = {name: min(_time(lambda f=f: f(sc, sc2, sc3)) for _ in range(2)) for name, f in timed.items()}
            for name in sorted(times, key=times.get)[:3] if len(times) > 1 else ():
                f = timed[name]
                times[name] = min(_time(lambda f=f: f(sc, sc2, sc3), reps=30) for _ in range(3))
        finally:
            if box is not None:
                box[0] = colsum
        best = min(times, key=times.get)
        choice = DECISIONS[key] = (best, times)
    if _decide_only:
        return choice[1][choice[0]]
    name = FORCE.get(key, choice[0])
    if name not in calls:
        name = choice[0]
    if _SPLIT_STORE and "s+hip" in calls:
        name = "s+hip"
    if _TRACE and key not in _TRACED:
        _TRACED.add(key)
        print(f"[gemm] {key!r} -> {name}", flush=True)
    if TIMING is not None:
        s_ev, e_ev = torch.cuda.Event(enable_timing=True), torch.cuda.Event(enable_timing=True)
        s_ev.record()
        _run(name)
        e_ev.record()
        TIMING.append((key, name, s_ev, e_ev))
        return name
    return _run(name)


K_ = K

DUAL = os.environ.get("IIT_GEMM_DUAL", "1") != "0"
DUAL_DECISIONS: Dict[Tuple, Tuple[str, Dict[str, float]]] = {}
_DUAL_X_EPIS = (K.EPI_BF16, K.EPI_DGELU)
_DUAL_W_EPIS = (K.EPI_F32_STORE, K.EPI_F32_ACC)


def _dual_eligible(x: dict, w: dict) -> bool:
    return (DUAL and POLICY == "auto" and x["A"].is_cuda and x.get("mode", 0) == 0 and x.get("epi", 0) in _DUAL_X_EPIS
            and w.get("mode") == (K.MODE_AKM | K.MODE_BKM) and w.get("epi") in _DUAL_W_EPIS
            and all(x.get(k) is None for k in ("bias0", "resid", "C2", "splits"))
            and all(w.get(k) is None for k in ("bias0", "resid", "C2", "splits", "aux", "colsum")))


def _dual_specs(x: dict, w: dict, xc, wc, csum, bsum=None, gsq=None):
    ws = dict(A=w["A"], B=w["B"], C=wc, M=w["M"], N=w["N"], K=w["K"], lda=w["lda"], ldb=w["ldb"], ldc=w["ldc"],
              epi=w["epi"], bsum=bsum, gsq=gsq)
    xs = dict(A=x["A"], B=x["B"], C=xc, C2=x.get("aux"), M=x["M"], N=x["N"], K=x["K"], lda=x["lda"], ldb=x["ldb"],
              ldc=x["ldc"], ldc2=x.get("ldc2", 0), epi=x["epi"], csum=csum)
    return ws, xs


def _dual_candidates(x: dict, w: dict, xc, wc, csum, bsum=None, gsq=None):
    ws, xs = _dual_specs(x, w, xc, wc, csum, bsum, gsq)
    det = deterministic()
    out = {}
    for wt in K.DUAL_W_TILES:
        for xt in K.DUAL_X_TILES:
            if not K.dual_family_ok(wt, xt):
                continue
            for sp, red in ((1, False), (2, True), (4, True), (8, True), (2, False), (4, False), (8, False)):
                if not red and sp > 1 and (w["epi"] != K.EPI_F32_ACC or det):
                    continue
                if sp > 1 and w["K"] // sp < 256:
                    continue
                if K.gemm_dual_ok(ws, xs, wt, xt, sp, red) and not _excluded(
                        f"dual{wt}.{xt}" + (f"{'r' if red else 'k'}{sp}" if sp > 1 else "")):
                    out[f"dual{wt}.{xt}" + (f"{'r' if red else 'k'}{sp}" if sp > 1 else "")] = \
                        lambda wt=wt, xt=xt, sp=sp, red=red: K.gemm_dual(ws, xs, wt, xt, sp, red)
    return out


def gemm_pair(x: dict, w: dict, prefetch=None) -> Optional[str]:
    def serial():
        gemm(**x)
        return gemm(**w)

    if not _dual_eligible(x, w):
        return serial()
    fresh = bool(w.get("fresh")) and w["epi"] == K.EPI_F32_STORE
    key = ("dual", x["M"], x["N"], x["K"], x["epi"], x.get("colsum") is not None,
           w["M"], w["N"], w["K"], w["epi"], fresh, deterministic())
    choice = DUAL_DECISIONS.get(key)
    if choice is None:
        shipped = _table().get(repr(key))
        if shipped is not None and not _excluded(shipped):
            choice = DUAL_DECISIONS[key] = (shipped, {shipped: float("nan")})
    if choice is None:
        if torch.cuda.is_current_stream_capturing():
            return serial()
        _frozen_miss(key)
        xc = _scratch(x["C"], x["M"], max(x["ldc"], x["N"]))
        wc = _scratch(w["C"], w["M"], max(w["ldc"], w["N"]))
        cs = torch.zeros_like(x["colsum"]) if x.get("colsum") is not None else None
        bs = torch.zeros_like(w["bsum"]) if w.get("bsum") is not None else None
        sq = torch.zeros_like(w["gsq"]) if w.get("gsq") is not None else None
        calls = _dual_candidates(x, w, xc, wc, cs, bs, sq)
        calls["serial"] = lambda: (gemm(**{**x, "C": xc, "colsum": cs}),
                                   gemm(**{**w, "C": wc, "bsum": bs, "gsq": sq}))
        times = {n: min(_time(f) for _ in range(2)) for n, f in calls.items()}
        for n in sorted(times, key=times.get)[:3] if len(times) > 1 else ():
            times[n] = min(_time(calls[n], reps=30) for _ in range(3))
        best = min(times, key=times.get)
        choice = DUAL_DECISIONS[key] = (best, times)
    name = FORCE.get(key, choice[0])
    cfg = _parse_dual(name)
    ws, xs = _dual_specs(x, w, x["C"], w["C"], x.get("colsum"), w.get("bsum"), w.get("gsq"))
    if cfg is None or not K.gemm_dual_ok(ws, xs, *cfg):
        name, cfg = "serial", None
    s_ev = e_ev = None
    if TIMING is not None:
        s_ev, e_ev = torch.cuda.Event(enable_timing=True), torch.cuda.Event(enable_timing=True)
        s_ev.record()
    if cfg is None:
        res = serial()
    else:
        K.gemm_dual(ws, xs, *cfg, prefetch=prefetch)
        res = name
    if TIMING is not None:
        e_ev.record()
        TIMING.append((key, name, s_ev, e_ev))
    return res


def _parse_dual(name: str):
    import re
    m = re.fullmatch(r"dual(\d+)\.(\d+)(?:([rk])(\d+))?", name)
    if m is None:
        return None
    return int(m.group(1)), int(m.group(2)), int(m.group(4) or 1), m.group(3) == "r"

_TABLE_PATH = os.path.join(os.path.dirname(os.path.abspath(__file__)), "tuned", "gemm_decisions_gfx950.json")
_TABLE = None
_RAGGED_TABLE: Dict[str, bool] = {}


def _ragged_table() -> Dict[str, bool]:
    _table()
    return _RAGGED_TABLE


def _table() -> Dict[str, str]:
    global _TABLE
    if _TABLE is None:
        _TABLE = {}
        _RAGGED_TABLE.clear()
        path = os.environ.get("IIT_GEMM_TABLE", _TABLE_PATH)
        if path != "0" and os.path.exists(path) and torch.cuda.is_available():
            import json
            try:
                with open(path) as f:
                    data = json.load(f)
                arch = getattr(torch.cuda.get_device_properties(0), "gcnArchName", "").split(":")[0]
                if data.get("arch") == arch:
                    _TABLE = dict(data.get("decisions", {}))
                    _RAGGED_TABLE.update({k: bool(v) for k, v in data.get("ragged", {}).items()})
            except (OSError, ValueError) as e:
                print(f"[iit] GEMM decision table not loaded ({e})")
    return _TABLE


def sync_decisions(group=None) -> int:
    import torch.distributed as dist
    if not (dist.is_available() and dist.is_initialized()) or dist.get_world_size(group) == 1:
        return 0
    ws = dist.get_world_size(group)
    mine = {"gemm": dict(DECISIONS), "dual": dict(DUAL_DECISIONS), "ragged": dict(RAGGED)}
    every = [None] * ws
    dist.all_gather_object(every, mine, group=group)
    changed = 0
    for name, table in (("gemm", DECISIONS), ("dual", DUAL_DECISIONS), ("ragged", RAGGED)):
        merged = {}
        for r in reversed(range(ws)):
            merged.update(every[r][name])
        for k, v in merged.items():
            old = table.get(k)
            if old is None or old[0] != v[0]:
                changed += 1
            table[k] = v
    return changed


def export_table(path: str) -> int:
    import json
    dec = {repr(k): v[0] for k, v in DECISIONS.items()}
    dec.update({repr(k): v[0] for k, v in DUAL_DECISIONS.items()})
    ragged = {repr(k): bool(v[0]) for k, v in RAGGED.items() if v[0] is not None}
    arch = getattr(torch.cuda.get_device_properties(0), "gcnArchName", "").split(":")[0] \
        if torch.cuda.is_available() else None
    with open(path, "w") as f:
        json.dump({"arch": arch, "device": torch.cuda.get_device_name(0) if torch.cuda.is_available() else None,
                   "decisions": dec, "ragged": ragged}, f, indent=0, sort_keys=True)
    return len(dec) + len(ragged)


def report() -> str:
    lines = [f"library fast paths: {dict(_BLAS_OK) or 'all available'}"]
    for (M, N, Kd, mode, epi, bias, fresh, _det), (c, times) in sorted(DECISIONS.items()):
        ts = "  ".join(f"{k} {v:8.1f}us" for k, v in times.items())
        lines.append(f"M={M:6d} N={N:6d} K={Kd:6d} mode={mode:2d} epi={epi}{'f' if fresh else ''} bias={int(bias)} "
                     f"-> {c:6s} {ts}")
    for (M, N, Kd, mode, epi, bias, fresh, _), (split, whole, pieces) in sorted(RAGGED.items()):
        lines.append(f"M={M:6d} N={N:6d} K={Kd:6d} mode={mode:2d} epi={epi}{'f' if fresh else ''} bias={int(bias)} "
                     f"-> {'bulk+tail' if split else 'whole'}  whole {whole}us  bulk+tail {pieces}us")
    for key, (c, times) in sorted(DUAL_DECISIONS.items()):
        ts = "  ".join(f"{k} {v:8.1f}us" for k, v in sorted(times.items(), key=lambda kv: kv[1])[:6])
        lines.append(f"pair dX {key[1:6]} dW {key[6:11]} -> {c}  {ts}")
    return "\n".join(lines)
```

iit_amd/ops/hip_kernels.py:

```python
from __future__ import annotations

import ctypes
import math
import os
from typing import Optional, Sequence

import numpy as np
import torch

from . import build as _build

c_void_p, c_long, c_int, c_float, c_ull = ctypes.c_void_p, ctypes.c_long, ctypes.c_int, ctypes.c_float, ctypes.c_ulonglong

EPI_BF16, EPI_BF16_BIAS3, EPI_F32_RESID, EPI_GELU, EPI_DGELU, EPI_F32_ACC, EPI_F32_ACC_QKV, EPI_F32_STORE = range(8)
EPI_GELU_ERF = 8
EPI_DGELU_ERF = 9
MODE_NN, MODE_AKM, MODE_BKM, MODE_AF32, MODE_BF32 = 0, 1, 2, 4, 8

_LIB = None
GEMM_GROUP_M = 4
GEMM_DUAL_GROUP_M = 2

_SIGS = {
    "iit_gemm": [c_void_p] * 10 + [c_long] * 5 + [c_int] * 12 + [c_void_p],
    "iit_gemm_f32": [c_void_p] * 6 + [c_long] * 4 + [c_int] * 7 + [c_void_p],
    "iit_gemm_f32_ok": [c_void_p] * 6 + [c_long] * 4 + [c_int] * 7,
    "iit_gemm_glds": [c_void_p] * 8 + [c_long] * 5 + [c_int] * 8 + [c_void_p] * 4,
    "iit_gemm_glds_ok": [c_void_p] * 5 + [c_long] * 5 + [c_int] * 9,
    "iit_gemm_glds_sm": [c_void_p] * 8 + [c_long] * 5 + [c_int] * 8 + [c_void_p] * 3 + [c_int] + [c_void_p] * 3,
    "iit_embed_pos_fwd": [c_void_p, c_void_p, c_void_p, c_void_p, c_int, c_int, c_int, c_void_p],
    "iit_embed_pos_bwd": [c_void_p, c_void_p, c_void_p, c_void_p, c_int, c_int, c_int, c_void_p],
    "iit_ln_fwd": [c_void_p] * 6 + [c_int, c_int, c_float, c_void_p],
    "iit_ln_bwd": [c_void_p, c_int] + [c_void_p] * 9 + [c_int, c_int, c_int, c_void_p],
    "iit_ln_fwd_sel": [c_void_p] * 6 + [c_int, c_int, c_float, c_ull, c_int, c_int, c_void_p],
    "iit_ln_bwd_xh16": [c_void_p, c_int] + [c_void_p] * 5 + [c_int, c_int, c_int, c_void_p],
    "iit_ln_bwd_sel": [c_void_p, c_int] + [c_void_p] * 9 + [c_int, c_int, c_int, c_ull, c_int, c_void_p],
    "iit_ln_bwd_part": [c_void_p, c_int] + [c_void_p] * 10 + [c_int, c_int, c_int, c_ull, c_int, c_void_p, c_void_p],
    "iit_ln_fwd_twin": [c_void_p] * 7 + [c_int, c_int, c_float, c_void_p],
    "iit_ln_bwd_part_rows": [],
    "iit_attn_small_fwd": [c_void_p] * 4 + [c_ull, c_int, c_int, c_int, c_int, c_long, c_long, c_long, c_float, c_int,
                                            c_void_p],
    "iit_attn_small_bwd": [c_void_p] * 4 + [c_ull, c_int, c_int, c_int, c_int, c_long, c_long, c_float, c_int, c_void_p],
    "iit_attn_mfma_fwd": [c_void_p] * 4 + [c_ull, c_int, c_int, c_int, c_int, c_long, c_long, c_long, c_float, c_int,
                                           c_void_p],
    "iit_attn_mfma_fwd_pair": [c_void_p] * 4 + [c_ull, c_int, c_int, c_int, c_int, c_long, c_long, c_long, c_float,
                                                c_int, c_void_p, c_int, c_ull, c_void_p],
    "iit_attn_mfma_bwd": [c_void_p] * 4 + [c_ull, c_int, c_int, c_int, c_int, c_long, c_long, c_float, c_int, c_void_p],
    "iit_attn_mfma_fwd_spec": [c_void_p] * 3 + [c_int] * 4 + [c_long, c_long, c_float, c_int, c_int, c_void_p,
                                                               c_void_p],
    "iit_attn_mfma_bwd_spec": [c_void_p] * 4 + [c_int] * 4 + [c_long, c_long, c_float, c_int, c_void_p, c_void_p],
    "iit_ce_fwd": [c_void_p, c_long, c_void_p, c_void_p, c_void_p, c_void_p, c_int, c_int, c_void_p],
    "iit_ce_bwd": [c_void_p, c_long, c_void_p, c_void_p, c_void_p, c_float, c_void_p, c_long, c_int, c_int, c_int,
                   c_void_p, c_void_p],
    "iit_adam_flat": [c_void_p] * 6 + [c_int, c_void_p, c_int] + [c_float] * 6 + [c_void_p] * 3
                     + [c_void_p, c_int, c_void_p, c_void_p],
    "iit_sumsq_2d": [c_void_p, c_long, c_int, c_int, c_void_p, c_void_p],
    "iit_kl_rows": [c_void_p, c_long, c_void_p, c_long, c_int, c_int, c_void_p, c_void_p],
    "iit_adam_span_size": [],
    "iit_sumsq_spans": [c_void_p, c_void_p, c_int, c_void_p, c_int, c_int, c_void_p, c_void_p],
    "iit_adam_spans": [c_void_p] * 6 + [c_int, c_void_p] + [c_float] * 6 + [c_void_p] * 4,
    "iit_gelu_fwd": [c_void_p, c_long, c_void_p, c_long, c_int, c_int, c_int, c_void_p],
    "iit_shadow_refresh": [c_void_p, c_int, c_void_p],
    "iit_shadow_desc_size": [],
    "iit_colsum_accum": [c_void_p, c_int, c_long, c_void_p, c_int, c_int, c_void_p],
    "iit_dgelu": [c_void_p, c_void_p, c_void_p, c_long, c_int, c_void_p],
    "iit_add_bf16": [c_void_p, c_long, c_void_p, c_long, c_void_p, c_long, c_void_p, c_int, c_int, c_void_p],
    "iit_device_sync": [],
    "iit_zero_chunks": [c_void_p, c_void_p, c_int, c_void_p],
    "iit_zero_ranges": [c_void_p, c_void_p, c_void_p, c_int, c_void_p],
    "iit_colsum_multi": [c_void_p] * 6 + [c_int, c_void_p],
    "iit_rms_fwd": [c_void_p, c_int, c_void_p, c_void_p, c_void_p, c_int, c_int, c_float, c_void_p],
    "iit_rms_bwd": [c_void_p, c_void_p, c_int, c_void_p, c_void_p, c_void_p, c_void_p, c_int, c_int, c_void_p],
    "iit_rms_bwd_res": [c_void_p, c_void_p, c_int, c_void_p, c_void_p, c_void_p, c_void_p, c_void_p, c_int, c_int,
                        c_void_p],
    "iit_rotary": [c_void_p, c_long, c_long, c_long, c_void_p, c_void_p, c_void_p] + [c_int] * 8 + [c_void_p],
    "iit_swiglu_fwd": [c_void_p, c_void_p, c_void_p, c_long, c_void_p],
    "iit_swiglu_bwd": [c_void_p] * 5 + [c_long, c_void_p],
    "iit_swiglu_splice_fwd": [c_void_p] * 4 + [c_long, c_void_p, c_void_p],
    "iit_sparse_pair": [c_void_p, c_long, c_long, c_void_p, c_int, c_void_p],
    "iit_gemm_dual_set_group_m": [c_int],
    "iit_swiglu_splice_bwd": [c_void_p] * 5 + [c_long, c_void_p, c_void_p],
    "iit_embed_splice_fwd": [c_void_p, c_void_p, c_long, c_void_p, c_void_p, c_long, c_int, c_void_p, c_void_p],
    "iit_embed_splice_bwd": [c_void_p, c_void_p, c_int, c_void_p, c_long, c_long, c_int, c_void_p, c_void_p],
    "iit_flash_fwd": [c_void_p] * 3 + [c_void_p, c_void_p, c_void_p, c_void_p, c_void_p, c_void_p, c_ull] + [c_int] * 5
                     + [c_float, c_int, c_void_p, c_void_p],
    "iit_flash_bwd": [c_void_p] * 3 + [c_void_p] * 11 + [c_ull] + [c_int] * 5 + [c_float, c_int, c_void_p, c_void_p],
    "iit_flash_fwd_blocks": [c_void_p] * 3 + [c_void_p, c_void_p, c_void_p, c_void_p, c_void_p, c_void_p, c_ull]
                            + [c_int] * 5 + [c_float, c_int, c_void_p, c_void_p, c_int],
    "iit_flash_bwd_blocks": [c_void_p] * 3 + [c_void_p] * 11 + [c_ull] + [c_int] * 5 + [c_float, c_int, c_void_p,
                                                                                       c_void_p, c_int],
    "iit_flash_plan": [c_int] * 6 + [c_void_p],
    "iit_splice": [c_void_p, c_void_p, c_void_p, c_long, c_void_p, c_int, c_int, c_float, c_void_p],
    "iit_splice_spec_size": [],
    "iit_bn_fwd": [c_void_p] * 8 + [c_long, c_int, c_float, c_int, c_int, c_void_p, c_float, c_void_p, c_void_p,
                                    c_void_p, c_int, c_int, c_int, c_int, c_void_p],
    "iit_bn_bwd": [c_void_p] * 7 + [c_long, c_int, c_int, c_void_p, c_void_p, c_void_p, c_void_p, c_void_p, c_void_p,
                                    c_int, c_int, c_int, c_int, c_void_p],
    "iit_gemm_glds_set_prof": [c_void_p],
    "iit_maxpool3s2_fwd": [c_void_p] * 3 + [c_int] * 5 + [c_void_p],
    "iit_bn_ws_floats": [c_int],
    "iit_maxpool3s2_bwd": [c_void_p] * 3 + [c_int] * 5 + [c_void_p],
    "iit_gemm_dual_ok": [c_void_p] * 3 + [c_long] * 3 + [c_int] * 7 + [c_void_p] * 4 + [c_long] * 4 + [c_int] * 5,
    "iit_gemm_dual": [c_void_p] * 3 + [c_long] * 3 + [c_int] * 6 + [c_void_p] * 2 + [c_void_p] * 4 + [c_long] * 4
                     + [c_int] * 5 + [c_void_p] * 3 + [c_void_p, c_long, c_void_p, c_long, c_int, c_void_p],
    "iit_gemm_glds_set_group_m": [c_int],
    "iit_ioi_hl_label": [c_void_p, c_void_p, c_void_p, c_int, c_int, c_int, c_int, c_int, c_void_p, c_void_p],
    "iit_conv3x3_tiles": [],
    "iit_conv3x3_ok": [c_long, c_int, c_int, c_int, c_int, c_int, c_int],
    "iit_conv3x3": [c_void_p] * 4 + [c_long, c_int, c_int, c_int, c_int, c_int, c_int, c_int, c_void_p, c_void_p,
                                     c_void_p, c_void_p],
    "iit_conv3x3_rows": [c_int],
    "iit_conv2d_ok": [c_long] + [c_int] * 12,
    "iit_conv2d": [c_void_p] * 4 + [c_long] + [c_int] * 12 + [c_void_p] * 4,
    "iit_conv2d_wgrad_ok": [c_long] + [c_int] * 11,
    "iit_conv2d_wgrad": [c_void_p] * 4 + [c_long] + [c_int] * 12 + [c_void_p] * 3,
    "iit_bn_fwd_tiles": [c_void_p] * 4 + [c_int, c_int] + [c_void_p] * 4 + [c_long, c_int, c_float, c_int, c_void_p,
                                                                           c_float, c_void_p, c_void_p],
    "iit_conv3x3_wgrad_tiles": [],
    "iit_conv3x3_wgrad_ok": [c_long, c_int, c_int, c_int, c_int, c_int, c_int],
    "iit_conv3x3_wgrad": [c_void_p] * 4 + [c_long, c_int, c_int, c_int, c_int, c_int, c_int, c_int, c_void_p, c_void_p,
                                           c_void_p],
}


def lib():
    global _LIB
    if _LIB is None:
        if not _build.is_up_to_date():
            _build.build()
        L = ctypes.CDLL(_build.LIB)
        for name, argtypes in _SIGS.items():
            fn = getattr(L, name)
            fn.argtypes = argtypes
            fn.restype = c_int
        _LIB = L
        gm = os.environ.get("IIT_GEMM_GROUP_M", str(GEMM_GROUP_M))
        if gm:
            L.iit_gemm_glds_set_group_m(int(gm))
        dgm = os.environ.get("IIT_GEMM_DUAL_GROUP_M", str(GEMM_DUAL_GROUP_M))
        if dgm:
            L.iit_gemm_dual_set_group_m(int(dgm))
    return _LIB


def available() -> bool:
    try:
        lib()
        return True
    except Exception:
        return False


def _p(t: Optional[torch.Tensor]):
    return None if t is None else t.data_ptr()


def _stream():
    return torch.cuda.current_stream().cuda_stream


CHECK_BOUNDS = os.environ.get("IIT_CHECK_BOUNDS", "0") == "1"


def _avail(t: torch.Tensor) -> int:
    st = t.untyped_storage()
    return (st.nbytes() - (t.data_ptr() - st.data_ptr())) // t.element_size()


def _bounds(what: str, *spans):
    for name, t, rows, cols, ld in spans:
        if t is None or rows <= 0 or cols <= 0:
            continue
        need = (rows - 1) * ld + cols
        have = _avail(t)
        if need > have or ld < cols and rows > 1:
            raise RuntimeError(f"{what}: operand {name} needs {rows}x{cols} (ld {ld}) = {need} elements, "
                               f"storage holds {have} (shape {tuple(t.shape)}, stride {t.stride()})")


def _check(rc: int, what: str):
    if rc != 0:
        raise RuntimeError(f"{what} failed with hip error {rc}")


N_CU = 256


def _tiling(M: int, N: int, K: int, allow_split: bool):
    t128 = math.ceil(M / 128) * math.ceil(N / 128)
    if t128 >= 240:
        return 1, 1
    t64 = math.ceil(M / 64) * math.ceil(N / 64)
    splits = 1
    if allow_split and t64 < 240 and K >= 1024:
        splits = max(1, min(math.ceil(480 / t64), K // 512))
    return 0, splits


def gemm(A, B, C, *, M: int, N: int, K: int, lda: int, ldb: int, ldc: int, mode: int = MODE_NN, epi: int = EPI_BF16,
         C2=None, C3=None, bias0=None, bias1=None, bias2=None, resid=None, ldr: int = 0, aux=None, ldc2: int = 0,
         bias_cols: int = 0, qkv=(0, 0, 0), atomic: bool = False, splits: Optional[int] = None):
    can_split = epi in (EPI_F32_ACC, EPI_F32_ACC_QKV)
    big, auto_splits = _tiling(M, N, K, can_split)
    if splits is None:
        splits = auto_splits
    if CHECK_BOUNDS:
        _gemm_bounds("iit_gemm", A, B, C, C2, resid, M, N, K, lda, ldb, ldc, ldc2, ldr, mode, qkv)
    rc = lib().iit_gemm(_p(A), _p(B), _p(C), _p(C2), _p(C3), _p(bias0), _p(bias1), _p(bias2), _p(resid), _p(aux),
                        lda, ldb, ldc, ldc2, ldr, M, N, K, mode, epi, splits, big, bias_cols, qkv[0], qkv[1], qkv[2],
                        int(atomic), _stream())
    _check(rc, "iit_gemm")


GLDS_TILES = {0: (128, 128), 1: (128, 64), 2: (64, 128), 3: (64, 64), 4: (128, 128),
              5: (256, 192),
              6: (128, 128), 7: (256, 128),
              8: (96, 96),
              9: (128, 96),
              10: (96, 192), 11: (192, 96),
              12: (96, 96), 13: (128, 96), 14: (64, 64),
              15: (128, 96), 16: (96, 96), 17: (64, 64), 18: (128, 128),
              20: (192, 192),
              21: (192, 128), 22: (128, 192),
              23: (128, 96), 24: (64, 96), 25: (128, 128), 26: (96, 96), 27: (128, 192), 28: (64, 192),
              29: (64, 96), 30: (64, 64), 31: (64, 128),
              32: (256, 128), 33: (128, 256), 34: (256, 256),
              40: (256, 256),
              41: (256, 256), 42: (256, 256)}
GLDS_DISPATCH_TILES = tuple(t for t in GLDS_TILES if t not in (12, 13, 14, 32, 33, 34, 42))


def _gemm_bounds(what, A, B, C, C2, resid, M, N, K, lda, ldb, ldc, ldc2, ldr, mode, qkv=(0, 0, 0)):
    a = ("A", A, K, M, lda) if mode & MODE_AKM else ("A", A, M, K, lda)
    b = ("B", B, K, N, ldb) if mode & MODE_BKM else ("B", B, N, K, ldb)
    if qkv[0]:
        dh, H, d = qkv
        per = ("C", C, 1, H * d * dh, H * d * dh)
        _bounds(what, a, b, per, ("C2",) + per[1:] if C2 is None else ("C2", C2, 1, H * d * dh, H * d * dh))
        return
    _bounds(what, a, b, ("C", C, M, N, ldc), ("C2", C2, M, N, ldc2 or ldc), ("resid", resid, M, N, ldr or ldc))


def gemm_glds_ok(A, B, C, *, M, N, K, lda, ldb, ldc, mode, epi, C2=None, resid=None, ldc2=0, ldr=0, bias_cols=0,
                 tile=0, splits=1, reduce=False) -> bool:
    if any(t is not None and (not t.is_cuda or t.dtype not in (torch.bfloat16,)) for t in (A, B)):
        return False
    return bool(lib().iit_gemm_glds_ok(_p(A), _p(B), _p(C), _p(C2), _p(resid), lda, ldb, ldc, ldc2, ldr, M, N, K,
                                       mode, epi, bias_cols, tile, splits, int(reduce)))


_SPLIT_WS = {}


def split_workspace(M: int, N: int, tile, splits: int, device) -> tuple:
    stream = torch.cuda.current_stream(device).cuda_stream
    key = (str(device), stream)
    ent = _SPLIT_WS.get(key)
    bm, bn = GLDS_TILES[tile] if isinstance(tile, int) else tile
    need_ws, need_cnt = splits * M * N, (M // bm) * (N // bn)
    if ent is None:
        ent = _SPLIT_WS[key] = [None, None, []]
    if ent[0] is None or ent[0].numel() < need_ws:
        if ent[0] is not None:
            ent[2].append(ent[0])
        ent[0] = torch.empty(need_ws, dtype=torch.float32, device=device)
    if ent[1] is None or ent[1].numel() < need_cnt:
        if ent[1] is not None:
            ent[2].append(ent[1])
        ent[1] = torch.zeros(max(need_cnt, 1024), dtype=torch.int32, device=device)
    return ent[0], ent[1]


GLDS_STORE_MODE = int(os.environ.get("IIT_GEMM_STORE", "0"))


def gemm_glds(A, B, C, *, M, N, K, lda, ldb, ldc, mode, epi, C2=None, bias0=None, bias1=None, bias2=None, resid=None,
              ldc2=0, ldr=0, bias_cols=0, tile=0, splits=1, csum=None, reduce=False, store_mode=None, bsum=None,
              gsq=None):
    ws = cnt = None
    if reduce:
        ws, cnt = split_workspace(M, N, tile, splits, A.device)
    if CHECK_BOUNDS:
        _gemm_bounds("iit_gemm_glds", A, B, C, C2, resid, M, N, K, lda, ldb, ldc, ldc2, ldr, mode)
        _bounds("iit_gemm_glds", ("csum", csum, 1, N, N))
    sm = GLDS_STORE_MODE if store_mode is None else store_mode
    _check(lib().iit_gemm_glds_sm(_p(A), _p(B), _p(C), _p(C2), _p(bias0), _p(bias1), _p(bias2), _p(resid), lda, ldb,
                                  ldc, ldc2, ldr, M, N, K, mode, epi, bias_cols, tile, splits, _p(csum), _p(ws),
                                  _p(cnt), int(sm), _p(bsum) if mode == 3 else None,
                                  _p(gsq) if epi == EPI_F32_STORE else None, _stream()),
           "iit_gemm_glds")


GEMM_F32_TILES = {0: (64, 64), 1: (128, 128)}


def _f32_cuda(*ts) -> bool:
    return all(t is None or (t.is_cuda and t.dtype == torch.float32) for t in ts)


def gemm_f32_ok(A, B, C, *, M, N, K, lda, ldb, ldc, mode, epi, bias=None, resid=None, ldr=0, tile=0, splits=1) -> bool:
    if not _f32_cuda(A, B, C, bias, resid) or tile not in GEMM_F32_TILES:
        return False
    ws = 16 if splits > 1 else None
    return bool(lib().iit_gemm_f32_ok(_p(A), _p(B), _p(C), _p(bias), _p(resid), ws, lda, ldb, ldc, ldr, M, N, K, mode,
                                      epi, tile, splits))


def gemm_f32_splits(M: int, N: int, K: int, tile: int = 0) -> int:
    bm, bn = GEMM_F32_TILES[tile]
    tiles = math.ceil(M / bm) * math.ceil(N / bn)
    return max(1, min(N_CU // tiles, K // 128, 64))


def gemm_f32(A, B, C, *, M, N, K, lda, ldb, ldc, mode, epi, bias=None, resid=None, ldr=0, tile=0, splits=1):
    if not gemm_f32_ok(A, B, C, M=M, N=N, K=K, lda=lda, ldb=ldb, ldc=ldc, mode=mode, epi=epi, bias=bias, resid=resid,
                       ldr=ldr, tile=tile, splits=splits):
        raise RuntimeError(f"iit_gemm_f32: unsupported problem M={M} N={N} K={K} lda={lda} ldb={ldb} ldc={ldc} "
                           f"ldr={ldr} mode={mode} epi={epi} tile={tile} splits={splits} (fp32 GPU operands, 16-byte "
                           f"aligned pointers, leading dimensions multiples of 4)")
    if CHECK_BOUNDS:
        _gemm_bounds("iit_gemm_f32", A, B, C, None, resid, M, N, K, lda, ldb, ldc, 0, ldr, mode)
        _bounds("iit_gemm_f32", ("bias", bias, 1, N, N))
    ws = torch.empty(splits * M * N, dtype=torch.float32, device=A.device) if splits > 1 else None
    _check(lib().iit_gemm_f32(_p(A), _p(B), _p(C), _p(bias), _p(resid), _p(ws), lda, ldb, ldc, ldr, M, N, K, mode, epi,
                              tile, splits, _stream()), "iit_gemm_f32")


DUAL_W_TILES = {0: (128, 96), 1: (128, 128), 2: (96, 96), 3: (64, 96), 4: (64, 64),
                5: (256, 128), 6: (128, 128), 7: (128, 128), 8: (128, 96)}
DUAL_X_TILES = {0: (128, 96), 1: (64, 96), 2: (128, 192), 3: (128, 128),
                4: (256, 192), 5: (256, 128), 6: (128, 128), 7: (128, 128), 8: (128, 192)}


def _dual_family(t: int, first_big: int) -> int:
    return 2 if t >= 7 else (1 if t >= first_big else 0)


def dual_family_ok(wtile: int, xtile: int) -> bool:
    return _dual_family(wtile, 5) == _dual_family(xtile, 4)


def _bf16_cuda(*ts) -> bool:
    return all(t is not None and t.is_cuda and t.dtype == torch.bfloat16 for t in ts)


def gemm_dual_ok(w: dict, x: dict, wtile: int, xtile: int, splits: int = 1, reduce: bool = False) -> bool:
    if not _bf16_cuda(w["A"], w["B"], x["A"], x["B"]):
        return False
    return bool(lib().iit_gemm_dual_ok(
        _p(w["A"]), _p(w["B"]), _p(w["C"]), w["lda"], w["ldb"], w["ldc"], w["M"], w["N"], w["K"], w["epi"], wtile,
        splits, int(reduce), _p(x["A"]), _p(x["B"]), _p(x["C"]), _p(x.get("C2")), x["lda"], x["ldb"], x["ldc"],
        x.get("ldc2", 0), x["M"], x["N"], x["K"], x["epi"], xtile))


def gemm_dual(w: dict, x: dict, wtile: int, xtile: int, splits: int = 1, reduce: bool = False,
              prefetch=None) -> None:
    ws = cnt = None
    if reduce:
        ws, cnt = split_workspace(w["M"], w["N"], DUAL_W_TILES[wtile], splits, w["A"].device)
    if CHECK_BOUNDS:
        _gemm_bounds("iit_gemm_dual(dW)", w["A"], w["B"], w["C"], None, None, w["M"], w["N"], w["K"], w["lda"],
                     w["ldb"], w["ldc"], 0, 0, MODE_AKM | MODE_BKM)
        _gemm_bounds("iit_gemm_dual(dX)", x["A"], x["B"], x["C"], x.get("C2"), None, x["M"], x["N"], x["K"],
                     x["lda"], x["ldb"], x["ldc"], x.get("ldc2", 0), 0, MODE_NN)
        _bounds("iit_gemm_dual", ("csum", x.get("csum"), 1, x["N"], x["N"]))
    _check(lib().iit_gemm_dual(
        _p(w["A"]), _p(w["B"]), _p(w["C"]), w["lda"], w["ldb"], w["ldc"], w["M"], w["N"], w["K"], w["epi"], wtile,
        splits, _p(ws), _p(cnt), _p(x["A"]), _p(x["B"]), _p(x["C"]), _p(x.get("C2")), x["lda"], x["ldb"], x["ldc"],
        x.get("ldc2", 0), x["M"], x["N"], x["K"], x["epi"], xtile, _p(x.get("csum")), _p(w.get("bsum")),
        _p(w.get("gsq")) if w["epi"] == EPI_F32_STORE else None, *_prefetch_args(prefetch), _stream()),
        "iit_gemm_dual")


_PF_PER_MB = float(os.environ.get("IIT_DUAL_PREFETCH_WGS_PER_MB", "16"))


def _prefetch_args(prefetch):
    ts = [t for t in (prefetch or ()) if t is not None and t.is_cuda and t.is_contiguous()
          and t.numel() * t.element_size() >= 64][:2]
    if not ts or _PF_PER_MB <= 0:
        return (None, 0, None, 0, 0)
    ts += [None] * (2 - len(ts))
    nb = [t.numel() * t.element_size() // 64 * 64 if t is not None else 0 for t in ts]
    wgs = max(8, min(1024, int(sum(nb) / 2 ** 20 * _PF_PER_MB)))
    return (_p(ts[0]), nb[0], _p(ts[1]), nb[1], wgs)


def kl_rows(a, b):
    R, V = a.shape
    out = torch.empty(R, 4, dtype=torch.float32, device=a.device)
    if CHECK_BOUNDS:
        _bounds("kl_rows", ("a", a, R, V, a.stride(0)), ("b", b, R, V, b.stride(0)))
    _check(lib().iit_kl_rows(_p(a), a.stride(0), _p(b), b.stride(0), R, V, _p(out), _stream()), "kl_rows")
    return out


_ADAM_SPAN4 = int(os.environ.get("IIT_ADAM_SPAN4", "1024"))


def sumsq_2d(c, ldc: int, M: int, N: int, gsq) -> None:
    if CHECK_BOUNDS:
        _bounds("sumsq_2d", ("c", c, M, N, ldc))
    _check(lib().iit_sumsq_2d(_p(c), ldc, M, N, _p(gsq), _stream()), "sumsq_2d")


def sumsq_spans(g, spans, nspans, part, step_dev, do_norm: bool):
    _check(lib().iit_sumsq_spans(_p(g), _p(spans), nspans, _p(part), part.numel(), int(do_norm), _p(step_dev),
                                 _stream()), "sumsq_spans")


def adam_spans(flat, g, m, v, spans, nspans, total, step_dev, *, lr, b1, b2, eps, wd, clip_norm, skipped=None,
               hyper=None):
    _check(lib().iit_adam_spans(_p(flat.data), _p(g), _p(m), _p(v), _p(flat.shadow), _p(spans), nspans, _p(total),
                                float(clip_norm or 0.0), lr, b1, b2, eps, wd, _p(hyper), _p(step_dev), _p(skipped),
                                _stream()), "adam_spans")


def splice(act, src, out, n, spec_ptr, f32, mode, scale=1.0):
    if CHECK_BOUNDS:
        _bounds("iit_splice", ("act", act, 1, n, n), ("out", out, 1, n, n))
    _check(lib().iit_splice(_p(act), _p(src), _p(out), n, spec_ptr, int(f32), int(mode), float(scale), _stream()),
           "iit_splice")


def embed_pos_fwd(tokens, W_E, W_pos, out, B, S, d):
    _check(lib().iit_embed_pos_fwd(_p(tokens), _p(W_E), _p(W_pos), _p(out), B * S, S, d, _stream()), "embed_pos_fwd")


def embed_pos_bwd(tokens, g, dWE, dWpos, B, S, d):
    _check(lib().iit_embed_pos_bwd(_p(tokens), _p(g), _p(dWE), _p(dWpos), B, S, d, _stream()), "embed_pos_bwd")


def ln_fwd(x, w, b, y, mean, rstd, T, d, eps):
    if CHECK_BOUNDS:
        _bounds("ln_fwd", ("x", x, T, d, d), ("y", y, T, d, d), ("mean", mean, 1, T, T), ("rstd", rstd, 1, T, T))
    _check(lib().iit_ln_fwd(_p(x), _p(w), _p(b), _p(y), _p(mean), _p(rstd), T, d, eps, _stream()), "ln_fwd")


def ln_fwd_twin(x, w, b, y, y32, mean, rstd, T, d, eps) -> bool:
    if CHECK_BOUNDS:
        _bounds("ln_fwd_twin", ("x", x, T, d, d), ("y", y, T, d, d), ("y32", y32, T, d, d))
    return lib().iit_ln_fwd_twin(_p(x), _p(w), _p(b), _p(y), _p(y32), _p(mean), _p(rstd), T, d, eps, _stream()) == 0


def _ln_part(dw, T: int, d: int):
# ... 274 lines not shown

CONV_WG_TILES = {0: (64, 64), 1: (128, 64), 2: (128, 128), 3: (64, 128)}


def conv3x3_wgrad_splits(pixels: int) -> list:
    nkt = pixels // 64
    out = []
    for target in (1, 2, 4, 8, 16, 32, 64):
        d = max(x for x in range(1, target + 1) if nkt % x == 0)
        if d not in out:
            out.append(d)
    return out


def conv3x3_wgrad_ok(N: int, H: int, W: int, Cin: int, Cout: int, tile: int, splits: int) -> bool:
    return bool(lib().iit_conv3x3_wgrad_ok(N, H, W, Cin, Cout, tile, splits))


def conv3x3_wgrad(dy, x, dw, N: int, H: int, W: int, Cin: int, Cout: int, acc: bool, tile: int, splits: int = 1):
    ws = cnt = None
    if splits > 1:
        ws, cnt = split_workspace(Cout, 9 * Cin, CONV_WG_TILES[tile], splits, dy.device)
    if CHECK_BOUNDS:
        assert dw.dtype == torch.float32 and dw.numel() >= 9 * Cin * Cout
        assert dy.numel() >= N * H * W * Cout and x.numel() >= N * H * W * Cin
    _check(lib().iit_conv3x3_wgrad(_p(dy), _p(x), _p(dw), _p(zero_page(x.device)), N, H, W, Cin, Cout, int(acc), tile,
                                   splits, _p(ws), _p(cnt), _stream()), "conv3x3_wgrad")


def maxpool3s2_bwd(dy, idx, dx, N: int, H: int, W: int, C: int):
    _check(lib().iit_maxpool3s2_bwd(_p(dy), _p(idx), _p(dx), N, H, W, C, int(dy.dtype == torch.float32), _stream()),
           "maxpool3s2_bwd")


def bn_two_level() -> bool:
    if os.environ.get("IIT_BN_REDUCE", "") == "two":
        return True
    return os.environ.get("IIT_DETERMINISTIC", "0") == "1" or torch.are_deterministic_algorithms_enabled()


def bn_fwd(x, res, y, ws, rmean, rvar, w, b, M: int, C: int, eps: float, relu: bool, training: bool, save,
           momentum: float, nbt, src=None, spec=None, H: int = 0, W: int = 0):
    if CHECK_BOUNDS:
        for t in (x, y) + ((res,) if res is not None else ()):
            assert _avail(t) >= M * C and t.dtype == x.dtype, "bn_fwd: activation smaller than M x C / dtype"
        assert ws.numel() >= bn_ws_floats(C) and save.numel() >= 2 * C
    _check(lib().iit_bn_fwd(_p(x), _p(res), _p(y), _p(ws), _p(rmean), _p(rvar), _p(w), _p(b), M, C, eps, int(relu),
                            int(training), _p(save), momentum, _p(nbt), _p(src), None if spec is None else spec.ptr,
                            H, W, int(x.dtype == torch.float32), int(bn_two_level()), _stream()), "bn_fwd")


def bn_fwd_tiles(x, res, y, cstat, T: int, R: int, rmean, rvar, w, b, M: int, C: int, eps: float, relu: bool, save,
                 momentum: float, nbt):
    if CHECK_BOUNDS:
        for t in (x, y) + ((res,) if res is not None else ()):
            assert _avail(t) >= M * C and t.dtype == torch.bfloat16, "bn_fwd_tiles: activation smaller than M x C"
        assert T * R == M and cstat.numel() >= 3 * C * T and save.numel() >= 2 * C
    _check(lib().iit_bn_fwd_tiles(_p(x), _p(res), _p(y), _p(cstat), T, R, _p(rmean), _p(rvar), _p(w), _p(b), M, C,
                                  eps, int(relu), _p(save), momentum, _p(nbt), _stream()), "bn_fwd_tiles")


def bn_bwd(dy, y, x, save, w, ws, coef, M: int, C: int, training: bool, dx, dres, dw, db, src=None, spec=None,
           H: int = 0, W: int = 0):
    if CHECK_BOUNDS:
        for t in (dy, x, dx):
            assert _avail(t) >= M * C, "bn_bwd: activation smaller than M x C"
    _check(lib().iit_bn_bwd(_p(dy), _p(y), _p(x), _p(save), _p(w), _p(ws), _p(coef), M, C, int(training), _p(dx),
                            _p(dres), _p(dw), _p(db), _p(src), None if spec is None else spec.ptr, H, W,
                            int(x.dtype == torch.float32), int(bn_two_level()), _stream()), "bn_bwd")


def zero_ranges(base, starts, lens):
    import numpy as np
    starts = np.ascontiguousarray(starts, dtype=np.int64)
    lens = np.ascontiguousarray(lens, dtype=np.int64)
    if CHECK_BOUNDS and len(lens):
        assert int((starts + lens).max()) <= _avail(base) and int(starts.min()) >= 0, "zero_ranges out of bounds"
    _check(lib().iit_zero_ranges(_p(base), starts.ctypes.data, lens.ctypes.data, len(lens), _stream()),
           "zero_ranges")


def zero_chunks(base, chunks, n: int):
    _check(lib().iit_zero_chunks(_p(base), _p(chunks), n, _stream()), "zero_chunks")


def rms_fwd(x, w, y, rstd, T: int, d: int, eps: float):
    _check(lib().iit_rms_fwd(_p(x), int(x.dtype == torch.float32), _p(w), _p(y), _p(rstd), T, d, eps, _stream()),
           "rms_fwd")


def rms_bwd(dy, x, rstd, w, dx, dw, T: int, d: int, dres=None):
    _check(lib().iit_rms_bwd_res(_p(dy), _p(x), int(x.dtype == torch.float32), _p(rstd), _p(w), _p(dx), _p(dres),
                                 _p(dw), T, d, _stream()), "rms_bwd")


def rotary(x, out, cos, sin, rd: int, offset: int, adjacent: bool, inverse: bool):
    B, S, H, D = x.shape
    _check(lib().iit_rotary(_p(x), x.stride(0), x.stride(1), x.stride(2), _p(out), _p(cos), _p(sin), int(inverse),
                            B, S, H, D, rd, offset, int(adjacent), _stream()), "rotary")


def swiglu_fwd(gate, up, post):
    _check(lib().iit_swiglu_fwd(_p(gate), _p(up), _p(post), gate.numel(), _stream()), "swiglu_fwd")


def sparse_pair(act, T: int, ld: int, spec_ptr, mode: int) -> None:
    if CHECK_BOUNDS:
        _bounds("sparse_pair", ("act", act, 2 * T if mode == 0 else T, ld, ld))
    _check(lib().iit_sparse_pair(_p(act), T, ld, spec_ptr, int(mode), _stream()), "sparse_pair")


def swiglu_splice_fwd(gate, up, post, src, spec_ptr):
    _check(lib().iit_swiglu_splice_fwd(_p(gate), _p(up), _p(post), _p(src), gate.numel(), spec_ptr, _stream()),
           "swiglu_splice_fwd")


def embed_splice_fwd(tokens, W16, out, src, spec_ptr):
    T, d = tokens.numel(), out.shape[-1]
    if CHECK_BOUNDS:
        _bounds("embed_splice_fwd", ("out", out, T, d, d))
    _check(lib().iit_embed_splice_fwd(_p(tokens), _p(W16), W16.stride(0), _p(out), _p(src), T, d, spec_ptr,
                                      _stream()), "embed_splice_fwd")


def embed_splice_bwd(tokens, dout, grad, spec_ptr):
    T, d = tokens.numel(), dout.shape[-1]
    _check(lib().iit_embed_splice_bwd(_p(tokens), _p(dout), int(dout.dtype == torch.float32), _p(grad),
                                      grad.stride(0), T, d, spec_ptr, _stream()), "embed_splice_bwd")


def swiglu_splice_bwd(dpost, gate, up, dgate, dup, spec_ptr):
    _check(lib().iit_swiglu_splice_bwd(_p(dpost), _p(gate), _p(up), _p(dgate), _p(dup), gate.numel(), spec_ptr,
                                       _stream()), "swiglu_splice_bwd")


def swiglu_bwd(dpost, gate, up, dgate, dup):
    _check(lib().iit_swiglu_bwd(_p(dpost), _p(gate), _p(up), _p(dgate), _p(dup), gate.numel(), _stream()),
           "swiglu_bwd")


def ce_fwd(logits, ld, labels, loss, lse, amax, R, V):
    if CHECK_BOUNDS:
        _bounds("ce_fwd", ("logits", logits, R, V, ld))
    _check(lib().iit_ce_fwd(_p(logits), ld, _p(labels), _p(loss), _p(lse), _p(amax), R, V, _stream()), "ce_fwd")


def ce_bwd(logits, ld, labels, lse, gscale, inv_rows, out, ld_out, R, V, out16=None):
    if CHECK_BOUNDS:
        _bounds("ce_bwd", ("logits", logits, R, V, ld), ("out", out, R, V, ld_out))
    _check(lib().iit_ce_bwd(_p(logits), ld, _p(labels), _p(lse), _p(gscale), inv_rows, _p(out), ld_out, R, V,
                            int(out.dtype == torch.bfloat16), _p(out16), _stream()), "ce_bwd")


def colsum_accum(x, ld, out, T, N):
    if CHECK_BOUNDS:
        _bounds("colsum", ("x", x, T, N, ld), ("out", out, 1, N, N))
    _check(lib().iit_colsum_accum(_p(x), int(x.dtype == torch.float32), ld, _p(out), T, N, _stream()), "colsum")


def colsum_vec_ok(x, ld, out, N) -> bool:
    cpt = 4 if x.dtype == torch.float32 else 8
    return (x.dtype in (torch.float32, torch.bfloat16) and out.dtype == torch.float32 and N % cpt == 0
            and ld % cpt == 0 and x.data_ptr() % 16 == 0)


def colsum_multi(items):
    import numpy as np
    if not items:
        return
    xs = np.array([it[0].data_ptr() for it in items], dtype=np.int64)
    outs = np.array([it[2].data_ptr() for it in items], dtype=np.int64)
    lds = np.array([it[1] for it in items], dtype=np.int64)
    Ts = np.array([it[3] for it in items], dtype=np.int32)
    Ns = np.array([it[4] for it in items], dtype=np.int32)
    f32s = np.array([int(it[0].dtype == torch.float32) for it in items], dtype=np.int32)
    if CHECK_BOUNDS:
        for x, ld, out, T, N in items:
            _bounds("colsum_multi", ("x", x, T, N, ld), ("out", out, 1, N, N))
    _check(lib().iit_colsum_multi(xs.ctypes.data, outs.ctypes.data, lds.ctypes.data, Ts.ctypes.data, Ns.ctypes.data,
                                  f32s.ctypes.data, len(items), _stream()), "colsum_multi")


def colsum3_accum(x, ld, outs, T, N):
    for i, o in enumerate(outs):
        colsum_accum(x[:, i * N:], ld, o, T, N)


def gelu_fwd(pre, out, M, N, erf=False):
    _check(lib().iit_gelu_fwd(_p(pre), pre.stride(0), _p(out), out.stride(0), M, N, int(erf), _stream()), "gelu_fwd")


def dgelu(dpost, pre, out, erf=False):
    _check(lib().iit_dgelu(_p(dpost), _p(pre), _p(out), dpost.numel(), int(erf), _stream()), "dgelu")


def add_bf16(out, ldo, base, ldb, y, ldy, bias, M, N):
    if CHECK_BOUNDS:
        _bounds("add_bf16", ("out", out, M, N, ldo), ("base", base, M, N, ldb), ("y", y, M, N, ldy))
    _check(lib().iit_add_bf16(_p(out), ldo, _p(base), ldb, _p(y), ldy, _p(bias), M, N, _stream()), "add_bf16")


def shadow_refresh(descs: torch.Tensor, n: int):
    _check(lib().iit_shadow_refresh(_p(descs), n, _stream()), "shadow_refresh")


_SHADOW_DTYPE = np.dtype([("src", np.uint64), ("dst", np.uint64), ("rows", np.int32), ("cols", np.int32),
                          ("ld", np.int64), ("heads", np.int32), ("transpose", np.int32), ("src_hs", np.int64),
                          ("dst_hs", np.int64)])


def make_shadow_descs(entries, device) -> torch.Tensor:
    assert _SHADOW_DTYPE.itemsize == lib().iit_shadow_desc_size()
    arr = np.zeros(len(entries), dtype=_SHADOW_DTYPE)
    for i, e in enumerate(entries):
        src_ptr, dst_ptr, rows, cols, ld, tr = e[:6]
        heads, shs, dhs = (e[6], e[7], e[8]) if len(e) > 6 else (1, 0, 0)
        arr[i] = (src_ptr, dst_ptr, rows, cols, ld, heads, int(tr), shs, dhs)
    return torch.from_numpy(arr.view(np.uint8).copy()).to(device)


def adam_step(flat, exp_avg, exp_avg_sq, step_dev, *, lr, b1, b2, eps, wd, clip_norm, skipped=None, hyper=None):
    nparts = 1024
    part = getattr(flat, "_norm_parts", None)
    if part is None or part.numel() < nparts:
        part = flat._norm_parts = torch.zeros(nparts, dtype=torch.float32, device=flat.data.device)
    spans, nspans = flat.span_table(lib().iit_adam_span_size(), max_len4=_ADAM_SPAN4)
    sq_spans, n_sq, gsq = flat.norm_spans(lib().iit_adam_span_size())
    _check(lib().iit_adam_flat(_p(flat.data), _p(flat.grad), _p(exp_avg), _p(exp_avg_sq), _p(flat.shadow),
                               _p(spans), nspans, _p(part), nparts, float(clip_norm or 0.0), lr, b1, b2, eps, wd,
                               _p(hyper), _p(step_dev), _p(skipped), _p(sq_spans), n_sq, _p(gsq), _stream()),
           "adam_flat")
    flat.after_step(mirror_written=flat.shadow is not None)


IOI_HL_NODES = {"all_nodes_hook": 0, "hook_duplicate": 1, "hook_s_inhibition": 2, "hook_name_mover": 3}


def ioi_hl_label(base, src, name_table, V: int, node: int, out):
    B, S = base.shape
    _check(lib().iit_ioi_hl_label(_p(base), _p(src), _p(name_table), name_table.numel(), B, S, V, node, _p(out),
                                  _stream()), "ioi_hl_label")


def gemm_glds_set_prof(buf) -> None:
    lib().iit_gemm_glds_set_prof(_p(buf))


def gemm_glds_set_group_m(gm: int) -> None:
    lib().iit_gemm_glds_set_group_m(int(gm))


def gemm_dual_set_group_m(gm: int) -> None:
    lib().iit_gemm_dual_set_group_m(int(gm))
```

iit_amd/ops/hip_ops.py:

```python
from __future__ import annotations

import math
import os
from typing import Optional, Sequence

import torch
from torch.autograd import Function

from ..engine import grad_hooks
from . import hip_kernels as K
from .gemm_dispatch import gemm, gemm_pair
from .torch_ops import TorchOps, act_fn

BF16 = torch.bfloat16
F32 = torch.float32


def _pad8(n: int) -> int:
    return (n + 7) // 8 * 8


def _grad_slot(p: Optional[torch.Tensor]) -> Optional[torch.Tensor]:
    if p is None or not p.requires_grad:
        return None
# ... 795 lines not shown
    @staticmethod
    def backward(ctx, dpost):
        gate, up = ctx.saved_tensors
        dg, du = torch.empty_like(gate), torch.empty_like(up)
        K.swiglu_splice_bwd(_c16(dpost.to(BF16)), gate, up, dg, du, ctx.spec.ptr)
        return dg, du, None, None


def swiglu_spliced(pre, pre_linear, index, src) -> Optional[torch.Tensor]:
    from .splice import patch_spec
    if os.environ.get("IIT_SWIGLU_SPLICE", "1") == "0" or pre.shape[-1] % 8 or pre.dtype != BF16:
        return None
    if src.dtype != BF16 or src.device != pre.device:
        src = src.to(device=pre.device, dtype=BF16)
    spec = patch_spec(index, tuple(pre.shape), src)
    if spec is None or spec.dims[3][0] % 8:
        return None
    return SwiGLUSpliceFn.apply(pre, pre_linear, src, spec)


class EmbedSpliceFn(Function):

    @staticmethod
    def forward(ctx, tokens, W_E, flat, src, spec):
        tok = tokens.reshape(-1).to(torch.int64).contiguous()
        W16 = flat.shadow_view(W_E)
        out = torch.empty(*tokens.shape, W_E.shape[-1], dtype=BF16, device=W_E.device)
        K.embed_splice_fwd(tok, W16, out, src, spec.ptr)
        ctx.save_for_backward(tok)
        ctx.p, ctx.flat, ctx.spec = W_E, flat, spec
        return out

    @staticmethod
    def backward(ctx, g):
        (tok,) = ctx.saved_tensors
        from ..engine import grad_hooks
        W_E = ctx.p
        slot = W_E.grad
        if slot is None:
            slot = ctx.flat.bind_zero(W_E)
        g = g.reshape(-1, g.shape[-1])
        if g.dtype not in (BF16, torch.float32):
            g = g.float()
        K.embed_splice_bwd(tok, g.contiguous(), slot, ctx.spec.ptr)
        grad_hooks.notify(W_E)
        return None, None, None, None, None


def embed_spliced(tokens, W_E, flat, index, src) -> Optional[torch.Tensor]:
    from .splice import patch_spec
    d = W_E.shape[-1]
    if os.environ.get("IIT_EMBED_SPLICE", "1") == "0" or d % 8 or W_E.stride(-1) != 1 or W_E.stride(0) % 8:
        return None
    if src.dtype != BF16 or src.device != W_E.device:
        src = src.to(device=W_E.device, dtype=BF16)
    shape = tuple(tokens.shape) + (d,)
    spec = patch_spec(index, shape, src)
    if spec is None or spec.dims[3][0] % 8:
        return None
    return EmbedSpliceFn.apply(tokens, W_E, flat, src, spec)


def llama_fused_ok(x: torch.Tensor) -> bool:
    return x.is_cuda and x.dtype == BF16 and os.environ.get("IIT_LLAMA_FUSED", "1") != "0"


class LinearFn(Function):

    @staticmethod
    def forward(ctx, x, W, b, w, ldw, resid, out_kind):
        ctx.set_materialize_grads(False)
        lead = x.shape[:-1]
        Kd = x.shape[-1]
        N = W.shape[-1]
        x2 = _flat2(x.to(BF16).contiguous())
        T = x2.shape[0]
        dev = x.device
        if out_kind == "bf16":
            out = torch.empty(T, N, dtype=BF16, device=dev)
            gemm(x2, w, out, M=T, N=N, K=Kd, lda=Kd, ldb=ldw, ldc=N, mode=K.MODE_BKM, epi=K.EPI_BF16, bias0=b)
            res = out.view(*lead, N)
        elif out_kind == "f32":
            Np = _pad8(N)
            out = torch.empty(T, Np, dtype=F32, device=dev)
            gemm(x2, w, out, M=T, N=N, K=Kd, lda=Kd, ldb=ldw, ldc=Np, mode=K.MODE_BKM, epi=K.EPI_F32_STORE, bias0=b)
            res = out[:, :N]
            res = res.unflatten(0, lead) if len(lead) != 1 else res
        else:
            r2 = _flat2(resid.float().contiguous())
            out = torch.empty(T, N, dtype=F32, device=dev)
            gemm(x2, w, out, M=T, N=N, K=Kd, lda=Kd, ldb=ldw, ldc=N, mode=K.MODE_BKM, epi=K.EPI_F32_RESID, bias0=b,
                 resid=r2, ldr=N)
            res = out.view(*lead, N)
        ctx.save_for_backward(x2)
        ctx.params = (W, b)
        ctx.w = w
        _pf_register(ctx, x2, w)
        ctx.ldw = ldw
        ctx.meta = (lead, Kd, N, out_kind, x.dtype)
        return res

    @staticmethod
    def backward(ctx, gy):
        if gy is None:
            return (None,) * 7
        (x2,) = ctx.saved_tensors
        W, b = ctx.params
        lead, Kd, N, out_kind, x_dtype = ctx.meta
        T = x2.shape[0]
        gres = gy if out_kind == "resid" else None
        g16 = _bf16_of(gy)
        g2 = _aligned_rows(g16, T, N)
        ldg = g2.stride(0)
        dx = xspec = dxb = None
        if ctx.needs_input_grad[0]:
            amode = K.MODE_NN
            _, splits = K._tiling(T, Kd, N, True)
            if splits == 1:
                dxb = torch.empty(T, Kd, dtype=BF16, device=g2.device)
                xspec = dict(A=g2, B=ctx.w, C=dxb, M=T, N=Kd, K=N, lda=ldg, ldb=ctx.ldw, ldc=Kd, mode=amode,
                             epi=K.EPI_BF16)
            else:
                dxf = torch.zeros(T, Kd, dtype=F32, device=g2.device)
                gemm(g2, ctx.w, dxf, M=T, N=Kd, K=N, lda=ldg, ldb=ctx.ldw, ldc=Kd, mode=amode, epi=K.EPI_F32_ACC,
                     splits=splits)
                dx = dxf.to(x_dtype).view(*lead, Kd)
        store = _claim_store(W)
        gW = W.grad if store else _grad_slot(W)
        gb = _grad_slot(b)
        bs = _fused_bias(gb, N) if gW is not None else None
        if gW is not None:
            mode = K.MODE_AKM | K.MODE_BKM
            gW2 = gW.reshape(Kd, N) if gW.is_contiguous() else gW
            assert gW2.stride(-1) == 1 and gW2.dim() == 2, "weight gradient must have unit column stride"
            wspec = dict(A=x2, B=g2, C=gW2, M=Kd, N=N, K=T, lda=Kd, ldb=ldg, ldc=gW2.stride(0), mode=mode,
                         epi=K.EPI_F32_STORE if store else K.EPI_F32_ACC, fresh=store, bsum=bs,
                         gsq=_norm_slots(store, W))
            choice = gemm_pair(xspec, wspec, prefetch=_pf_next(ctx)) if xspec is not None else gemm(**wspec)
            if store:
                _settle_claim(choice, W)
        elif xspec is not None:
            gemm(**xspec)
        if dxb is not None:
            dx = (dxb if x_dtype == BF16 else dxb.to(x_dtype)).view(*lead, Kd)
        if gb is not None:
            if bs is not None:
                _done(b)
            else:
                _BIAS_SUMS.add(g2, ldg, gb, T, N, b)
        _done(W)
        return dx, None, None, None, None, gres, None


class MLPInFn(Function):

    @staticmethod
    def forward(ctx, x, W_in, b_in, w, erf=False):
        ctx.set_materialize_grads(False)
        ctx.erf = erf
        lead = x.shape[:-1]
        d = x.shape[-1]
        dm = W_in.shape[1]
        x2 = _flat2(x.to(BF16).contiguous())
        T = x2.shape[0]
        post = torch.empty(T, dm, dtype=BF16, device=x.device)
        pre = torch.empty(T, dm, dtype=BF16, device=x.device)
        gemm(x2, w, post, C2=pre, M=T, N=dm, K=d, lda=d, ldb=dm, ldc=dm, ldc2=dm, mode=K.MODE_BKM, epi=K.EPI_GELU_ERF if erf else K.EPI_GELU,
             bias0=b_in)
        ctx.save_for_backward(x2, pre)
        ctx.params = (W_in, b_in)
        ctx.w = w
        _pf_register(ctx, x2, w)
        ctx.meta = (lead, d, dm)
        return pre.view(*lead, dm), post.view(*lead, dm)

    @staticmethod
    def backward(ctx, gpre, gpost):
        if gpre is None and gpost is None:
            return None, None, None, None, None
        x2, pre = ctx.saved_tensors
        W_in, b_in = ctx.params
        lead, d, dm = ctx.meta
        T = x2.shape[0]
        if gpost is not None:
            dpre = torch.empty(T, dm, dtype=BF16, device=x2.device)
            K.dgelu(gpost.to(BF16).contiguous().view(T, dm), pre, dpre, erf=ctx.erf)
            zs = getattr(ctx, "zero_spec", None)
            if zs is not None:
                K.sparse_pair(dpre, T, dm, zs.ptr, 1)
            if gpre is not None:
                dpre = (dpre.float() + gpre.float().reshape(T, dm)).to(BF16)
        else:
            dpre = gpre.to(BF16).contiguous().view(T, dm)
        dx = torch.empty(T, d, dtype=BF16, device=x2.device)
        xspec = dict(A=dpre, B=ctx.w, C=dx, M=T, N=d, K=dm, lda=dm, ldb=dm, ldc=d, epi=K.EPI_BF16)
        store = W_in.is_contiguous() and _claim_store(W_in)
        gW = W_in.grad if store else _grad_slot(W_in)
        summed = _bias_sum_done(gpre if gpost is None else None, b_in)
        gb = None if summed else _grad_slot(b_in)
        bs = _fused_bias(gb, dm) if gW is not None else None
        if gW is not None:
            choice = gemm_pair(xspec, dict(A=x2, B=dpre, C=gW, M=d, N=dm, K=T, lda=d, ldb=dm, ldc=dm,
                                           mode=K.MODE_AKM | K.MODE_BKM,
                                           epi=K.EPI_F32_STORE if store else K.EPI_F32_ACC, fresh=store, bsum=bs,
                                           gsq=_norm_slots(store, W_in)), prefetch=_pf_next(ctx))
            if store:
                _settle_claim(choice, W_in)
        else:
            gemm(**xspec)
        if gb is not None and bs is None:
            _BIAS_SUMS.add(dpre, dm, gb, T, dm, b_in)
        else:
            _done(b_in)
        _done(W_in)
        return dx.view(*lead, d), None, None, None, None


def _bias_sum_done(g: Optional[torch.Tensor], b: Optional[torch.Tensor]) -> bool:
    tag = getattr(g, "_iit_bias_sum", None) if g is not None else None
    return tag is not None and b is not None and tag == (g.data_ptr(), g._version, id(b))


class MLPOutGeluFn(Function):

    @staticmethod
    def forward(ctx, pre, post, W, b, w, ldw, resid, b_in, erf=False):
        ctx.set_materialize_grads(False)
        ctx.erf = erf
        lead = post.shape[:-1]
        Kd = post.shape[-1]
        N = W.shape[-1]
        x2 = _flat2(post)
        T = x2.shape[0]
        r2 = _flat2(resid.float().contiguous())
        out = torch.empty(T, N, dtype=F32, device=post.device)
        gemm(x2, w, out, M=T, N=N, K=Kd, lda=Kd, ldb=ldw, ldc=N, mode=K.MODE_BKM, epi=K.EPI_F32_RESID, bias0=b,
             resid=r2, ldr=N)
        ctx.save_for_backward(x2, _flat2(pre))
        ctx.params = (W, b, b_in)
        ctx.w = w
        _pf_register(ctx, x2, w)
        ctx.ldw = ldw
        ctx.meta = (lead, Kd, N)
        return out.view(*lead, N)

    @staticmethod
    def backward(ctx, gy):
        if gy is None:
            return (None,) * 9
        x2, pre2 = ctx.saved_tensors
        W, b, b_in = ctx.params
        lead, Kd, N = ctx.meta
        T = x2.shape[0]
        g16 = _bf16_of(gy)
        g2 = _aligned_rows(g16, T, N)
        ldg = g2.stride(0)
        dpre = xspec = gbi = None
        if ctx.needs_input_grad[0]:
            dpre = torch.empty(T, Kd, dtype=BF16, device=g2.device)
            gbi = _grad_slot(b_in)
            xspec = dict(A=g2, B=ctx.w, C=dpre, M=T, N=Kd, K=N, lda=ldg, ldb=ctx.ldw, ldc=Kd, mode=K.MODE_NN,
                         epi=K.EPI_DGELU_ERF if ctx.erf else K.EPI_DGELU, aux=pre2, ldc2=pre2.stride(0), colsum=gbi)
        store = _claim_store(W)
        gW = W.grad if store else _grad_slot(W)
        gb = _grad_slot(b)
        bs = _fused_bias(gb, N) if gW is not None else None
        if gW is not None:
            gW2 = gW.reshape(Kd, N) if gW.is_contiguous() else gW
            assert gW2.stride(-1) == 1 and gW2.dim() == 2, "weight gradient must have unit column stride"
            wspec = dict(A=x2, B=g2, C=gW2, M=Kd, N=N, K=T, lda=Kd, ldb=ldg, ldc=gW2.stride(0),
                         mode=K.MODE_AKM | K.MODE_BKM, epi=K.EPI_F32_STORE if store else K.EPI_F32_ACC, fresh=store,
                         bsum=bs, gsq=_norm_slots(store, W))
            choice = gemm_pair(xspec, wspec, prefetch=_pf_next(ctx)) if xspec is not None else gemm(**wspec)
            if store:
                _settle_claim(choice, W)
        elif xspec is not None:
            gemm(**xspec)
        if dpre is not None:
            dpre = dpre.view(*lead, Kd)
            if gbi is not None:
                dpre._iit_bias_sum = (dpre.data_ptr(), dpre._version, id(b_in))
        if gb is not None:
            if bs is not None:
                _done(b)
            else:
                _BIAS_SUMS.add(g2, ldg, gb, T, N, b)
        _done(W)
        return dpre, None, None, None, None, None, gy, None, None


class CrossEntropyFn(Function):

    @staticmethod
    def forward(ctx, logits, labels):
        ctx.set_materialize_grads(False)
        R, V = logits.shape
        if logits.stride(1) != 1:
            logits = logits.contiguous()
        ld = logits.stride(0)
        loss = torch.empty(R, dtype=F32, device=logits.device)
        lse = torch.empty(R, dtype=F32, device=logits.device)
        lab = labels.contiguous()
        K.ce_fwd(logits, ld, lab, loss, lse, None, R, V)
        ctx.save_for_backward(logits, lab, lse)
        return loss.mean()

    @staticmethod
    def backward(ctx, g):
        if g is None:
            return None, None
        logits, lab, lse = ctx.saved_tensors
        R, V = logits.shape
        ld = logits.stride(0)
        ldo = _pad8(V)
        buf = torch.empty(R, ldo, dtype=F32, device=logits.device)
        buf16 = torch.empty(R, ldo, dtype=BF16, device=logits.device)
        gs = g.reshape(1).float().contiguous()
        K.ce_bwd(logits, ld, lab, lse, gs, 1.0 / R, buf, ldo, R, V, out16=buf16)
        res = buf[:, :V]
        _set_bf16_twin(res, buf16[:, :V])
        return res, None


def cross_entropy(logits: torch.Tensor, labels: torch.Tensor) -> torch.Tensor:
    return CrossEntropyFn.apply(logits.float(), labels)




class Paired:

    __slots__ = ("base", "full", "f32")

    def __init__(self, base: torch.Tensor, full: torch.Tensor, f32=None):
        self.base, self.full, self.f32 = base, full, f32

    def resid_operands(self):
        if self.f32 is not None:
            return self.f32
        return self.base, self.full.float().contiguous()

    @property
    def nb(self) -> int:
        return self.base.shape[0]

    @property
    def src(self) -> torch.Tensor:
        return self.full[self.nb:]


class EmbedPosPairFn(EmbedPosFn):
    @staticmethod
    def forward(ctx, tokens, W_E, W_pos, tokens_full, box):
        ctx.set_materialize_grads(False)
        B2, S = tokens_full.shape
        d = W_E.shape[1]
        B = tokens.shape[0]
        out = torch.empty(B2, S, d, dtype=F32, device=tokens.device)
        K.embed_pos_fwd(tokens_full, W_E, W_pos, out, B2, S, d)
        ctx.save_for_backward(tokens_full[:B])
        ctx.params = (W_E, W_pos)
        box.append(out)
        return out[:B]

    @staticmethod
    def backward(ctx, g):
        return EmbedPosFn.backward(ctx, g) + (None, None)


class LayerNormForkPairFn(LayerNormForkFn):
    @staticmethod
    def forward(ctx, x, w, b, eps, x_full, box):
        ctx.set_materialize_grads(False)
        d = x.shape[-1]
        B = x.shape[0]
        x2 = _flat2(x_full)
        T2 = x2.shape[0]
        T = T2 * B // x_full.shape[0]
        y = torch.empty(T2, d, dtype=BF16, device=x.device)
        mean = torch.empty(T2, dtype=F32, device=x.device)
        rstd = torch.empty(T2, dtype=F32, device=x.device)
        K.ln_fwd(x2, w, b, y, mean, rstd, T2, d, eps)
        ctx.save_for_backward(y[:T] if _xhat16(w, b, d) else x2[:T], mean[:T], rstd[:T])
        ctx.params = (w, b)
        ctx.in_dtype = x.dtype
        yf = y.view(*x_full.shape[:-1], d)
        box.append(yf)
        return yf[:B], x.view_as(x)

    @staticmethod
    def backward(ctx, dy, dpass):
        return LayerNormForkFn.backward(ctx, dy, dpass) + (None, None)


class LayerNormPairTwinFn(Function):

    @staticmethod
    def forward(ctx, x, w, b, eps, x_full, box):
        ctx.set_materialize_grads(False)
        d = x.shape[-1]
        B = x.shape[0]
        x2 = _flat2(x_full)
        T2 = x2.shape[0]
        T = T2 * B // x_full.shape[0]
        y = torch.empty(T2, d, dtype=BF16, device=x.device)
        y32 = torch.empty(T2, d, dtype=F32, device=x.device)
        mean = torch.empty(T2, dtype=F32, device=x.device)
        rstd = torch.empty(T2, dtype=F32, device=x.device)
        if not K.ln_fwd_twin(x2, w, b, y, y32, mean, rstd, T2, d, eps):
            K.ln_fwd(x2, w, b, y, mean, rstd, T2, d, eps)
            y32.copy_(y)
        ctx.save_for_backward(x2[:T], mean[:T], rstd[:T])
        ctx.params = (w, b)
        ctx.in_dtype = x.dtype
        yf = y.view(*x_full.shape[:-1], d)
        yf32 = y32.view(*x_full.shape[:-1], d)
        box.append((yf, yf32))
        return yf[:B], yf32[:B]

    @staticmethod
    def backward(ctx, dy, dy32):
        return LayerNormTwinFn.backward(ctx, dy, dy32) + (None, None)


class LayerNormPairFn(LayerNormFn):

    @staticmethod
    def forward(ctx, x, w, b, eps, x_full, box, pos_mask=0):
        ctx.set_materialize_grads(False)
        d = x.shape[-1]
        B = x.shape[0]
        x2 = _flat2(x_full)
        T2 = x2.shape[0]
        T = T2 * B // x_full.shape[0]
        y = torch.empty(T2, d, dtype=BF16, device=x.device)
        mean = torch.empty(T2, dtype=F32, device=x.device)
        rstd = torch.empty(T2, dtype=F32, device=x.device)
        S = x.shape[1] if x.dim() == 3 else 1
        if pos_mask:
            K.ln_fwd_sel(x2, w, b, y, mean, rstd, T2, d, eps, pos_mask, S, T)
        else:
            K.ln_fwd(x2, w, b, y, mean, rstd, T2, d, eps)
        ctx.save_for_backward(x2[:T], mean[:T], rstd[:T])
        ctx.params = (w, b)
        ctx.in_dtype = x.dtype
        ctx.sel = (pos_mask, S)
        yf = y.view(*x_full.shape[:-1], d)
        box.append(yf)
        return yf[:B]

    @staticmethod
    def backward(ctx, dy):
        pos_mask, S = ctx.sel
        if not pos_mask:
            return LayerNormFn.backward(ctx, dy) + (None, None, None)
        if dy is None:
            return (None,) * 7
        x2, mean, rstd = ctx.saved_tensors
        w, b = ctx.params
        T, d = x2.shape
        dx = torch.empty(T, d, dtype=F32, device=x2.device)
        dx16 = torch.empty(T, d, dtype=BF16, device=x2.device) if ctx.in_dtype == F32 else None
        dw = _grad_slot(w) if w is not None else None
        db = _grad_slot(b) if b is not None else None
        K.ln_bwd_sel(_flat2(dy.contiguous()), x2, mean, rstd, w, dx, dw, db, T, d, pos_mask, S, dx16=dx16)
        _done(w, b)
        dx = dx.view(*dy.shape[:-1], d)
        if dx16 is None:
            return (dx.to(ctx.in_dtype),) + (None,) * 6
        _set_bf16_twin(dx, dx16)
        return (dx,) + (None,) * 6


class QKVPairFn(QKVFn):
    @staticmethod
    def forward(ctx, x, layer, bias_bf16, W_Q, W_K, W_V, b_Q, b_K, b_V, x_full, box):
        ctx.set_materialize_grads(False)
        B, S, d = x.shape
# ... 183 lines not shown
        box.append(out)
        return out[:B]

    @staticmethod
    def backward(ctx, g):
        if g is None:
            return None, None, None, None, None
        g = g.contiguous()
        out = torch.empty_like(g)
        K.splice(g, None, out, g.numel(), ctx.spec.ptr, g.dtype == F32, 1)
        return out, None, None, None, None


def _one(fn, *args):
    box = []
    out = fn.apply(*args, box)
    return out, box[0]


class HipOps(TorchOps):
    name = "hip"
    fused = True

    def __init__(self, model):
        super().__init__(BF16)
        self.model = model
        self.shadow = ModelShadow(model)
        pol = os.environ.get("IIT_DUAL_PREFETCH", "auto")
        self.prefetch = pol == "1" or (pol == "auto" and type(model).__name__ != "HookedEncoder")
        self._layer_of = {}
        for i, blk in enumerate(model.blocks):
            self._layer_of[id(blk.attn.W_Q)] = i
            self._layer_of[id(blk.attn.W_O)] = i
            if not model.cfg.attn_only:
                self._layer_of[id(blk.mlp.W_in)] = i
                self._layer_of[id(blk.mlp.W_out)] = i

    def begin_forward(self):
        self.shadow.ensure()
        _PF_SEQ.clear()
        _PF_ON[0] = self.prefetch

    def _L(self, p):
        return self.shadow.layers[self._layer_of[id(p)]]

    def embed(self, tokens, W_E):
        return W_E[tokens]

    def pos_embed(self, batch, seq, W_pos, offset: int = 0):
        return W_pos[offset:offset + seq].unsqueeze(0).expand(batch, seq, W_pos.shape[-1])

    def embed_pos(self, tokens, W_E, W_pos):
        return EmbedPosFn.apply(tokens, W_E, W_pos)

    def residual(self, a, b):
        return a.float() + b.float()

    def w(self, p: torch.Tensor) -> torch.Tensor:
        return p.to(BF16)

    def layer_norm(self, x, w, b, eps):
        return LayerNormFn.apply(x, w, b, eps)

    def layer_norm_twin(self, x, w, b, eps):
        if os.environ.get("IIT_LN_TWIN", "1") == "0":
            return LayerNormFn.apply(x, w, b, eps)
        y, y32 = LayerNormTwinFn.apply(x, w, b, eps)
        y._iit_f32 = (y.data_ptr(), y._version, y32)
        return y

    def layer_norm_fork(self, x, w, b, eps):
        return LayerNormForkFn.apply(x, w, b, eps)

    def qkv(self, x, W_Q, W_K, W_V, b_Q, b_K, b_V):
        i = self._layer_of[id(W_Q)]
        packed = QKVFn.apply(x, self.shadow.layers[i], self.shadow.biases[i], W_Q, W_K, W_V, b_Q, b_K, b_V)
        q, k, v = packed[:, :, 0], packed[:, :, 1], packed[:, :, 2]
        q._iit_packed = k._iit_packed = v._iit_packed = packed
        return q, k, v

    def attention(self, q, k, v, causal, attn_scale, patch_heads: Optional[Sequence[int]] = None, patch_src=None,
                  hook_scores=None, hook_pattern=None, ignore=float("-inf")):
        S, dh = q.shape[1], q.shape[-1]
        if S > 16 and flash_supported(q):
            packed = getattr(q, "_iit_packed", None)
            if packed is not None and getattr(k, "_iit_packed", None) is packed and \
                    getattr(v, "_iit_packed", None) is packed and packed.is_contiguous():
                return FlashPackedFn.apply(packed, patch_src, K.heads_to_mask(patch_heads), causal, 1.0 / attn_scale)
            z = flash_attention(q, k, v, causal, attn_scale)
            if patch_heads:
                z = z.clone()
                z[:, :, list(patch_heads)] = patch_src[:, :, list(patch_heads)].to(z.dtype)
            return z
        if not K.attn_small_ok(S, dh):
            z = TorchOps.attention(self, q, k, v, causal, attn_scale)
            if patch_heads:
                z = z.clone()
                z[:, :, list(patch_heads)] = patch_src[:, :, list(patch_heads)].to(z.dtype)
            return z
        packed = getattr(q, "_iit_packed", None)
        if packed is None or getattr(k, "_iit_packed", None) is not packed or getattr(v, "_iit_packed", None) is not packed:
            packed = torch.stack([q, k, v], dim=2).to(BF16)
        mask = K.heads_to_mask(patch_heads)
        return AttnFn.apply(packed, patch_src, mask, causal, 1.0 / attn_scale)

    def o_proj(self, z, W_O, b_O):
        B, S, H, dh = z.shape
        return LinearFn.apply(z.reshape(B, S, H * dh), W_O, b_O, self._L(W_O)["o"], W_O.shape[-1], None, "bf16")

    def o_proj_residual(self, z, W_O, b_O, resid):
        resid = _f32_of(resid)
        B, S, H, dh = z.shape
        return LinearFn.apply(z.reshape(B, S, H * dh), W_O, b_O, self._L(W_O)["o"], W_O.shape[-1], resid, "resid")

    def o_result(self, z, W_O):
        return torch.einsum("bshe,hed->bshd", z.to(BF16), W_O.to(BF16))

    def mlp_in(self, x, W_in, b_in, act: str, hook_pre=None):
        w = self._L(W_in)["in"]
        if hook_pre is None and act in ("gelu_new", "gelu_fast", "gelu_pytorch_tanh", "gelu"):
            return MLPInFn.apply(x, W_in, b_in, w, act == "gelu")
        pre = LinearFn.apply(x, W_in, b_in, w, W_in.shape[1], None, "bf16")
        if hook_pre is not None:
            pre = hook_pre(pre)
        return pre, act_fn(act)(pre)

    def mlp_gelu_residual(self, x, W_in, b_in, W_out, b_out, resid, erf: bool = False):
        resid = _f32_of(resid)
        if not torch.is_grad_enabled():
            lead, d, dm, N = x.shape[:-1], x.shape[-1], W_in.shape[1], W_out.shape[1]
            x2 = _flat2(x.to(BF16).contiguous())
            T = x2.shape[0]
            post = torch.empty(T, dm, dtype=BF16, device=x.device)
            gemm(x2, self._L(W_in)["in"], post, C2=None, M=T, N=dm, K=d, lda=d, ldb=dm, ldc=dm, ldc2=dm,
                 mode=K.MODE_BKM, epi=K.EPI_GELU_ERF if erf else K.EPI_GELU, bias0=b_in)
            r2 = _flat2(resid.float().contiguous())
            out = torch.empty(T, N, dtype=F32, device=x.device)
            gemm(post, self._L(W_out)["out"], out, M=T, N=N, K=dm, lda=dm, ldb=W_out.shape[1], ldc=N,
                 mode=K.MODE_BKM, epi=K.EPI_F32_RESID, bias0=b_out, resid=r2, ldr=N)
            return out.view(*lead, N)
        pre, post = MLPInFn.apply(x, W_in, b_in, self._L(W_in)["in"], erf)
        return MLPOutGeluFn.apply(pre, post.detach(), W_out, b_out, self._L(W_out)["out"], W_out.shape[1], resid,
                                  b_in, erf)

    def mlp_out(self, post, W_out, b_out):
        return LinearFn.apply(post, W_out, b_out, self._L(W_out)["out"], W_out.shape[1], None, "bf16")

    def mlp_out_residual(self, post, W_out, b_out, resid):
        resid = _f32_of(resid)
        return LinearFn.apply(post, W_out, b_out, self._L(W_out)["out"], W_out.shape[1], resid, "resid")

    def unembed(self, x, W_U, b_U):
        sh = self.shadow
        return LinearFn.apply(x, W_U, b_U, sh.U, sh.Vp, None, "f32")

    def unembed_argmax(self, x, W_U, b_U, chunk: int = 8192):
        sh = self.shadow
        lead = x.shape[:-1]
        d = x.shape[-1]
        x2 = _flat2(x.to(BF16).contiguous())
        T = x2.shape[0]
        V = W_U.shape[1]
        buf = torch.empty(T, chunk, dtype=F32, device=x.device)
        best_v = best_i = None
        for s in range(0, V, chunk):
            n = min(chunk, V - s)
            gemm(x2, sh.U[:, s:], buf, M=T, N=n, K=d, lda=d, ldb=sh.Vp, ldc=chunk, mode=K.MODE_BKM,
                 epi=K.EPI_F32_STORE, bias0=b_U[s:s + n])
            v, i = buf[:, :n].max(dim=-1)
            i = i + s
            if best_v is None:
                best_v, best_i = v, i
            else:
                upd = v > best_v
                best_v = torch.where(upd, v, best_v)
                best_i = torch.where(upd, i, best_i)
        return best_i.view(*lead)


    supports_pairs = True

    def pair_embed_pos(self, tokens, src_tokens, W_E, W_pos) -> Paired:
        full_tok = torch.cat([tokens, src_tokens]).contiguous()
        out, full = _one(EmbedPosPairFn, tokens, W_E, W_pos, full_tok)
        return Paired(out, full)

    def pair_layer_norm_fork(self, p: Paired, w, b, eps):
        box = []
        y, x_pass = LayerNormForkPairFn.apply(p.base, w, b, eps, p.full.float().contiguous(), box)
        return Paired(y, box[0]), Paired(x_pass, p.full)

    def pair_layer_norm(self, p: Paired, w, b, eps, pos_mask: int = 0, twin: bool = False) -> Paired:
        box = []
        if twin and not pos_mask and w is not None and os.environ.get("IIT_LN_TWIN", "1") != "0":
            y, y32 = LayerNormPairTwinFn.apply(p.base, w, b, eps, p.full.float().contiguous(), box)
            yf, yf32 = box[0]
            y._iit_f32 = (y.data_ptr(), y._version, y32)
            return Paired(y, yf, (y32, yf32))
        y = LayerNormPairFn.apply(p.base, w, b, eps, p.full.float().contiguous(), box, int(pos_mask))
        return Paired(y, box[0])

    @staticmethod
    def position_mask(index, shape) -> int:
        if len(shape) != 3 or shape[1] > 64:
            return 0
        ranges = index.to_ranges(tuple(shape))
        if ranges is None or ranges[0] != [(0, shape[0])] or ranges[2] != [(0, shape[2])]:
            return 0
        m = 0
        for lo, hi in ranges[1]:
            for s_ in range(lo, hi):
                m |= 1 << s_
        return m

    def pair_qkv(self, p: Paired, W_Q, W_K, W_V, b_Q, b_K, b_V) -> Paired:
        i = self._layer_of[id(W_Q)]
        out, full = _one(QKVPairFn, p.base, self.shadow.layers[i], self.shadow.biases[i], W_Q, W_K, W_V, b_Q, b_K,
                         b_V, p.full)
        return Paired(out, full)

    def pair_attention(self, p: Paired, causal: bool, attn_scale: float, heads: Optional[Sequence[int]] = None
                       ) -> Paired:
        out, full = _one(AttnPairFn, p.base, causal, 1.0 / attn_scale, K.heads_to_mask(heads) if heads else 0,
                         p.full)
        return Paired(out, full)

    def pair_attention_spliced(self, p: Paired, causal: bool, attn_scale: float, index) -> Optional[Paired]:
        from .splice import patch_spec
        if os.environ.get("IIT_ATTN_SPLICE", "1") == "0":
            return None
        B2, S, _, H, dh = p.full.shape
        B = p.base.shape[0]
        spec = patch_spec(index, (B, S, H, dh))
        if spec is None or [d[0] for d in spec.dims] != [B, S, H, dh]:
            return None
        out, full = _one(AttnPairSpecFn, p.base, causal, 1.0 / attn_scale, spec, p.full)
        return Paired(out, full)

    def attention_dual(self, q, causal: bool, attn_scale: float) -> torch.Tensor:
        packed = q._iit_packed
        B, S, _, H, dh = packed.shape
        zf = torch.empty(2 * B, S, H, dh, dtype=BF16, device=packed.device)
        K.attn_pair_fwd(packed, zf[B:], None, B, S, H, dh, 3 * H * dh, H * dh, 1.0 / attn_scale, causal, z2=zf[:B])
        return zf

    def pair_heads_ok(self, S: int, dh: int) -> bool:
        return K.attn_pair_ok(S, dh)

    def pair_o_proj_residual(self, z: Paired, W_O, b_O, resid: Paired) -> Paired:
        B2, S, H, dh = z.full.shape
        B = z.base.shape[0]
        rb, rf = resid.resid_operands()
        out, full = _one(LinearPairFn, z.base.reshape(B, S, H * dh), W_O, b_O, self._L(W_O)["o"], W_O.shape[-1],
                         rb, "resid", z.full.reshape(B2, S, H * dh), rf)
        return Paired(out, full)

    def pair_mlp_in(self, x: Paired, W_in, b_in, erf: bool = False, index=None):
        spec = None
        if index is not None:
            from .splice import patch_spec
            B, S = x.base.shape[0], x.base.shape[1]
            spec = patch_spec(index, (B, S, W_in.shape[1])) if os.environ.get("IIT_MLP_SPLICE", "1") != "0" else None
            if spec is None:
                return None
        (pre, post), (pf, qf) = _one(MLPInPairFn, x.base, W_in, b_in, self._L(W_in)["in"], erf, x.full, spec)
        return Paired(pre, pf), Paired(post, qf)

    def pair_mlp_out_residual(self, post: Paired, W_out, b_out, resid: Paired) -> Paired:
        rb, rf = resid.resid_operands()
        out, full = _one(LinearPairFn, post.base, W_out, b_out, self._L(W_out)["out"], W_out.shape[1], rb,
                         "resid", post.full, rf)
        return Paired(out, full)

    def pair_mlp_gelu_residual(self, x: Paired, W_in, b_in, W_out, b_out, resid: Paired, erf: bool = False):
        pre, post = self.pair_mlp_in(x, W_in, b_in, erf)
        rb, rf = resid.resid_operands()
        out, full = _one(MLPOutGeluPairFn, pre.base, post.base.detach(), W_out, b_out, self._L(W_out)["out"],
                         W_out.shape[1], rb, b_in, erf, post.full, rf)
        return Paired(out, full)

    def pair_splice(self, p: Paired, index) -> Optional[Paired]:
        if not p.full.is_contiguous():
            return None
        specs = pair_specs(index, tuple(p.base.shape))
        if specs is None:
            return None
        out, full = _one(PairSpliceFn, p.base, p.full, specs[0], specs[1])
        return Paired(out, full)


def pair_specs(index, shape):
    from . import splice as _sp
    key = ("pair",) + tuple(shape)
    cache = getattr(index, "_iit_specs", None)
    if cache is not None and key in cache:
        return cache[key]
    ranges = index.to_ranges(tuple(shape))
    base_spec = _sp.patch_spec(index, tuple(shape))
    out = None
    if ranges is not None and base_spec is not None:
        B = shape[0]
        rest = list(shape[1:])
        row = 1
        for n in rest:
            row *= n
        cstr = []
        acc = 1
# ... 23 lines not shown
```

Baseline: 16790 pairs/s.

## Add ragged-edge GLDS GEMM and bf16-only cross-entropy backward for unembed

Adds a GLDS GEMM variant that handles N not divisible by the tile. Out-of-range B chunks are redirected to a zero buffer and the epilogue masks partial stores, so the vocab-sized unembed GEMMs can run as one kernel instead of being split into bulk and tail launches. It also adds a bf16-only cross-entropy backward, routed through a side handle returned by a new UnembedFn. This skips materialising the fp32 logits gradient and passes bf16 directly into the unembed backward GEMMs. Edge kernels are only chosen when the tuned table lists them, and the autograd handle trick adds complexity and correctness risk.

```diff
diff --git a/csrc/gemm_edge.hip b/csrc/gemm_edge.hip
--- /dev/null
+++ b/csrc/gemm_edge.hip
@@ -0,0 +1,139 @@
+#include "gemm_glds_body.h"
+
+namespace {
+
+__device__ __attribute__((aligned(16))) unsigned int g_edge_zero[4];
+
+template <int R, int NW, int BK>
+struct EdgeBStager {
+  using Base = OperandStager<true, R, NW, BK, false>;
+  static constexpr int NP = Base::NP, PR = Base::PR;
+  static constexpr int SN = Stager<true, PR, NW, BK, false>::N;
+  static constexpr int N = Base::N;
+  static_assert(NP * SN <= 32, "one bit per DMA instruction");
+  Base st;
+  unsigned oob;
+
+  __device__ __forceinline__ void init(const G2Args& p, int n0, int kbeg, int wave, int lane) {
+    st.init(p.B, p.ldb, n0, kbeg, wave, lane);
+    constexpr int CH = PR / 8, KRI = 64 / CH;
+    oob = 0;
+#pragma unroll
+    for (int q = 0; q < NP; ++q)
+#pragma unroll
+      for (int i = 0; i < SN; ++i) {
+        const int kr = (i * NW + wave) * KRI + lane / CH;
+        const int ch = lane % CH;
+        const int col = (((ch >> 1) ^ kmaj_swz<PR>(kr)) << 4) + ((ch & 1) << 3);
+        if (edge_redirect(n0 + q * PR + col, p.N)) oob |= 1u << (q * SN + i);
+      }
+  }
+
+  __device__ __forceinline__ void stage(int kt, char* img) const {
+#pragma unroll
+    for (int q = 0; q < NP; ++q) {
+      const long k = kt * st.st[q].kstep;
+#pragma unroll
+      for (int i = 0; i < SN; ++i) {
+        const __bf16* src = (oob >> (q * SN + i)) & 1 ? (const __bf16*)g_edge_zero : st.st[q].ptr[i] + k;
+        glds16(src, img + q * PR * BK * 2 + st.st[q].off[i]);
+      }
+    }
+  }
+};
+
+template <int BM, int BN, int NS, bool AKM, int EPI, int NW, int OCC>
+__global__ __launch_bounds__(NW * 64, OCC) void gemm_glds_edge_kernel(G2Args p) {
+  __shared__ __attribute__((aligned(16))) char smem[GldsSmem<BM, BN, NS, NW, 64, OCC>::BYTES];
+  gemm_glds_body<BM, BN, NS, AKM, true, EPI, NW, 64, OCC, false, void, EdgeBStager<BN, NW, 64>, true>(
+      p, blockIdx.x, gridDim.x, 0, 1, smem);
+}
+
+template <int BM, int BN, int NS, bool AKM, int EPI, int NW = 4, int OCC = 1>
+hipError_t launch(const G2Args& a, hipStream_t s) {
+  const int tiles = (a.M / BM) * ((a.N + BN - 1) / BN);
+  hipLaunchKernelGGL((gemm_glds_edge_kernel<BM, BN, NS, AKM, EPI, NW, OCC>), dim3(tiles), dim3(NW * 64), 0, s, a);
+  return hipGetLastError();
+}
+
+template <bool AKM, int EPI>
+hipError_t launch_tile(const G2Args& a, int tile, hipStream_t s) {
+  switch (tile) {
+    case 0: return launch<128, 128, 3, AKM, EPI>(a, s);
+    case 7: return launch<256, 128, 2, AKM, EPI, 8>(a, s);
+    case 25: return launch<128, 128, 2, AKM, EPI, 4, 2>(a, s);
+    default: return hipErrorInvalidValue;
+  }
+}
+
+bool edge_tile(int tile, int* bm, int* bn) {
+  switch (tile) {
+    case 0: case 25: *bm = 128; *bn = 128; return true;
+    case 7: *bm = 256; *bn = 128; return true;
+    default: return false;
+  }
+}
+
+inline long pad8l(long n) { return (n + 7) / 8 * 8; }
+
+}
+
+IIT_EXPORT int iit_gemm_edge_plan(int rows, int N, long ld, int elem, int tile, long* out6) {
+  int bm, bn;
+  if (!edge_tile(tile, &bm, &bn) || rows <= 0 || N <= 0 || ld < pad8l(N) || (elem != 2 && elem != 4))
+    return (int)hipErrorInvalidValue;
+  const int tiles_n = (N + bn - 1) / bn;
+  long used = 0, redirected = 0, straddle = 0, last = 0;
+  for (int r = 0; r < rows; ++r)
+    for (int c = 0; c < tiles_n * bn; c += 8) {
+      if (edge_redirect(c, N)) {
+        redirected += r == 0;
+        continue;
+      }
+      used += r == 0;
+      const int nv = edge_valid(c, N);
+      if (nv < 8) straddle = nv;
+      const long end = ((long)r * ld + c + 8) * elem;
+      if (end > last) last = end;
+    }
+  out6[0] = tiles_n; out6[1] = used; out6[2] = redirected; out6[3] = straddle; out6[4] = last;
+  out6[5] = ((long)(rows - 1) * ld + pad8l(N)) * elem;
+  return 0;
+}
+
+IIT_EXPORT int iit_gemm_glds_edge_ok(const void* A, const void* B, const void* C, const void* bias0, long lda,
+                                     long ldb, long ldc, int M, int N, int K, int mode, int epi, int tile) {
+  int bm, bn;
+  if (!edge_tile(tile, &bm, &bn)) return 0;
+  if (!(mode == 2 || mode == 3)) return 0;
+  if (!(epi == E_F32_ACC || epi == E_F32_STORE || (mode == 2 && epi == E_BF16))) return 0;
+  if (M <= 0 || N <= 0 || K <= 0 || M % bm || K % 64) return 0;
+  if (lda % 8 || ldb % 8 || ldc % 8 || ldb < pad8l(N) || ldc < pad8l(N)) return 0;
+  if (((uintptr_t)A | (uintptr_t)B | (uintptr_t)C | (uintptr_t)bias0) & 15) return 0;
+  return 1;
+}
+
+IIT_EXPORT int iit_gemm_glds_edge(const void* A, const void* B, void* C, const float* bias0, long lda, long ldb,
+                                  long ldc, int M, int N, int K, int mode, int epi, int tile, int store_mode,
+                                  float* bsum, float* gsq, int group_m, void* stream) {
+  if (!iit_gemm_glds_edge_ok(A, B, C, bias0, lda, ldb, ldc, M, N, K, mode, epi, tile)) return (int)hipErrorInvalidValue;
+  G2Args a{};
+  a.A = (const __bf16*)A; a.B = (const __bf16*)B; a.C = C;
+  a.bias0 = epi == E_F32_ACC ? nullptr : bias0;
+  a.lda = lda; a.ldb = ldb; a.ldc = ldc;
+  a.M = M; a.N = N; a.K = K; a.k_per_split = K;
+  a.store_mode = store_mode;
+  a.group_m = group_m;
+  a.bsum = mode == 3 ? bsum : nullptr;
+  a.gsq = epi == E_F32_STORE ? gsq : nullptr;
+  hipStream_t s = (hipStream_t)stream;
+#define GE(MODE, AK, EPI) \
+  if (mode == (MODE) && epi == (EPI)) return (int)launch_tile<AK, EPI>(a, tile, s);
+  GE(2, false, E_BF16)
+  GE(2, false, E_F32_STORE)
+  GE(2, false, E_F32_ACC)
+  GE(3, true, E_F32_ACC)
+  GE(3, true, E_F32_STORE)
+#undef GE
+  return (int)hipErrorInvalidValue;
+}
diff --git a/csrc/gemm_glds_body.h b/csrc/gemm_glds_body.h
--- a/csrc/gemm_glds_body.h
+++ b/csrc/gemm_glds_body.h
@@ -266,7 +266,10 @@
   static constexpr int BYTES = NS * STAGE > EPI_BYTES ? NS * STAGE : EPI_BYTES;
 };
 
-template <int BM, int BN, int EPI, int NT, int ECH, int EPS, class WriteAcc>
+__host__ __device__ __forceinline__ bool edge_redirect(int c, int N) { return c >= N; }
+__host__ __device__ __forceinline__ int edge_valid(int c, int N) { return c + 8 <= N ? 8 : (c < N ? N - c : 0); }
+
+template <int BM, int BN, int EPI, int NT, int ECH, int EPS, bool EDGE = false, class WriteAcc>
 __device__ __forceinline__ void glds_epilogue(const G2Args& p, char* smem, const int m0, const int n0, const int lin,
                                               WriteAcc&& write_acc) {
   const int tid = threadIdx.x, lane = tid & 63, wave = tid >> 6;
@@ -293,8 +296,16 @@
         pf[2 * k + 1] = *(const float4*)(src + 4);
       } else if constexpr (EPI == E_F32_ACC) {
         const float* src = (const float*)p.C + (long)row * p.ldc + col;
-        pf[2 * k] = *(const float4*)src;
-        pf[2 * k + 1] = *(const float4*)(src + 4);
+        if (!EDGE || edge_valid(col, p.N) == 8) {
+          pf[2 * k] = *(const float4*)src;
+          pf[2 * k + 1] = *(const float4*)(src + 4);
+        } else {
+          float t[8];
+#pragma unroll
+          for (int e = 0; e < 8; ++e) t[e] = e < edge_valid(col, p.N) ? src[e] : 0.f;
+          pf[2 * k] = make_float4(t[0], t[1], t[2], t[3]);
+          pf[2 * k + 1] = make_float4(t[4], t[5], t[6], t[7]);
+        }
       } else if constexpr (PF16) {
         pb[k] = *(const bf16x8*)((const __bf16*)p.C2 + (long)row * p.ldc2 + col);
       }
@@ -313,6 +324,30 @@
     {
       const float4 x = *(const float4*)(E + lr * EPS + lc), y = *(const float4*)(E + lr * EPS + lc + 4);
       v[0] = x.x; v[1] = x.y; v[2] = x.z; v[3] = x.w; v[4] = y.x; v[5] = y.y; v[6] = y.z; v[7] = y.w;
+    }
+    if constexpr (EDGE) {
+      static_assert(EPI == E_BF16 || EPI == E_F32_ACC || EPI == E_F32_STORE, "edge epilogues");
+      const int nv = edge_valid(col, p.N);
+      if (nv == 0) continue;
+      if (nv < 8) {
+        if constexpr (EPI == E_F32_ACC) {
+          add8v(v, pf[2 * k], pf[2 * k + 1]);
+        } else if (p.bias0) {
+#pragma unroll
+          for (int e = 0; e < 8; ++e)
+            if (e < nv) v[e] += p.bias0[col + e];
+        }
+#pragma unroll
+        for (int e = 0; e < 8; ++e)
+          if (e < nv) {
+            if constexpr (EPI == E_BF16) ((__bf16*)p.C)[(long)row * p.ldc + col + e] = f2bf(v[e]);
+            else ((float*)p.C)[(long)row * p.ldc + col + e] = v[e];
+            if constexpr (EPI == E_F32_STORE) {
+              if (p.gsq) sq += v[e] * v[e];
+            }
+          }
+        continue;
+      }
     }
     if constexpr (EPI == E_BF16) {
       if (p.bias0) add8(v, p.bias0 + col);
@@ -435,7 +470,7 @@
 }
 
 template <int BM, int BN, int NS, bool AKM, bool BKM, int EPI, int NW, int BK = 64, int OCC = 1, bool LEAN = false,
-          class ASTG = void, class BSTG = void>
+          class ASTG = void, class BSTG = void, bool EDGE = false>
 __device__ __forceinline__ void gemm_glds_body(const G2Args& p, const int lin, const int nlin, const int split,
                                                const int nsplit, char* smem) {
   using SA = std::conditional_t<std::is_void_v<ASTG>, OperandStager<AKM, BM, NW, BK, LEAN>, ASTG>;
@@ -457,7 +492,8 @@
   constexpr bool TR = EPI != E_F32_ACC;
   const int tid = threadIdx.x, lane = tid & 63, wave = tid >> 6;
   const int wm = wave >> 1, wn = wave & 1;
-  const int tiles_n = p.N / BN;
+  static_assert(!EDGE || (BKM && !std::is_void_v<BSTG>), "the edge variant stages its k-major B itself");
+  const int tiles_n = EDGE ? (p.N + BN - 1) / BN : p.N / BN;
   const int t = xcd_remap(lin, nlin);
   int tm, tn;
   grouped_tile(t, p.M / BM, tiles_n, tm, tn, p.group_m > 0 ? p.group_m : 8);
@@ -600,7 +636,8 @@
         float v = cs[j];
         v += __shfl_xor(v, 16);
         v += __shfl_xor(v, 32);
-        if (lane < 16) atomicAdd(p.bsum + n0 + wn * WN + j * 16 + lane, v);
+        if (lane < 16 && (!EDGE || n0 + wn * WN + j * 16 + lane < p.N))
+          atomicAdd(p.bsum + n0 + wn * WN + j * 16 + lane, v);
       }
     }
   }
@@ -671,7 +708,7 @@
       return;
     }
   }
-  glds_epilogue<BM, BN, EPI, NT, ECH, SM::EPS>(p, smem, m0, n0, lin, [&](float* E, int ch) {
+  glds_epilogue<BM, BN, EPI, NT, ECH, SM::EPS, EDGE>(p, smem, m0, n0, lin, [&](float* E, int ch) {
     if (wm / (WMR / ECH) == ch) {
 #pragma unroll
       for (int i = 0; i < TM; ++i)
diff --git a/csrc/kernels.hip b/csrc/kernels.hip
--- a/csrc/kernels.hip
+++ b/csrc/kernels.hip
@@ -991,6 +991,53 @@
   else
     hipLaunchKernelGGL(ce_bwd_kernel<float>, grid, dim3(256), 0, (hipStream_t)stream, logits, ld, labels, lse, gscale,
                        inv_rows, (float*)out, ld_out, V, (__bf16*)out16);
+  return hipGetLastError();
+}
+
+template <bool VEC>
+__global__ __launch_bounds__(256) void ce_bwd16_kernel(const float* __restrict__ logits, long ld,
+                                                       const long* __restrict__ labels, const float* __restrict__ lse,
+                                                       const float* __restrict__ gscale, float inv_rows,
+                                                       __bf16* __restrict__ out16, long ld_out, int V) {
+  const int row = blockIdx.y;
+  const int c0 = (blockIdx.x * 256 + threadIdx.x) * 8;
+  if (c0 >= ld_out) return;
+  const float* x = logits + (long)row * ld;
+  const float l = lse[row], gs = gscale[0];
+  const long lab = labels[row];
+  float v[8];
+  if (VEC && c0 + 8 <= V) {
+    const float4 a = *(const float4*)(x + c0), b = *(const float4*)(x + c0 + 4);
+    v[0] = a.x; v[1] = a.y; v[2] = a.z; v[3] = a.w; v[4] = b.x; v[5] = b.y; v[6] = b.z; v[7] = b.w;
+  } else {
+#pragma unroll
+    for (int e = 0; e < 8; ++e) v[e] = c0 + e < V ? x[c0 + e] : 0.f;
+  }
+  bf16x8 o;
+#pragma unroll
+  for (int e = 0; e < 8; ++e) {
+    const int i = c0 + e;
+    float g = 0.f;
+    if (i < V) {
+      const float p = __expf(v[e] - l);
+      g = (p - (i == lab ? 1.f : 0.f)) * gs * inv_rows;
+    }
+    o[e] = f2bf(g);
+  }
+  *(bf16x8*)(out16 + (long)row * ld_out + c0) = o;
+}
+
+IIT_EXPORT int iit_ce_bwd16(const float* logits, long ld, const long* labels, const float* lse, const float* gscale,
+                            float inv_rows, void* out16, long ld_out, int R, int V, void* stream) {
+  if (R <= 0 || V <= 0 || ld < V || ld_out < V || ld_out % 8 || ((uintptr_t)out16 & 15)) return (int)hipErrorInvalidValue;
+  dim3 grid((unsigned)((ld_out / 8 + 255) / 256), R);
+  const bool vec = (((uintptr_t)logits | (uintptr_t)(ld * 4)) & 15) == 0;
+  if (vec)
+    hipLaunchKernelGGL(ce_bwd16_kernel<true>, grid, dim3(256), 0, (hipStream_t)stream, logits, ld, labels, lse, gscale,
+                       inv_rows, (__bf16*)out16, ld_out, V);
+  else
+    hipLaunchKernelGGL(ce_bwd16_kernel<false>, grid, dim3(256), 0, (hipStream_t)stream, logits, ld, labels, lse,
+                       gscale, inv_rows, (__bf16*)out16, ld_out, V);
   return hipGetLastError();
 }
 
diff --git a/iit_amd/model_pairs/iit_behavior_model_pair.py b/iit_amd/model_pairs/iit_behavior_model_pair.py
--- a/iit_amd/model_pairs/iit_behavior_model_pair.py
+++ b/iit_amd/model_pairs/iit_behavior_model_pair.py
@@ -56,7 +56,7 @@
         output = self.ll_forward(base_x)
         if output.dim() > 1 and output.shape[0] == 1:
             return loss_fn(output, base_y)
-        return loss_fn(output.squeeze(), base_y)
+        return loss_fn(output.squeeze() if 1 in output.shape else output, base_y)
 
     def step_on_loss(self, loss: Tensor, optimizer) -> None:
         optimizer.zero_grad()
diff --git a/iit_amd/model_pairs/strict_iit_model_pair.py b/iit_amd/model_pairs/strict_iit_model_pair.py
--- a/iit_amd/model_pairs/strict_iit_model_pair.py
+++ b/iit_amd/model_pairs/strict_iit_model_pair.py
@@ -40,7 +40,7 @@
             out = self.ll_intervened_forward(base_x, [ll_node])
         if out.dim() > 1 and out.shape[0] == 1:
             return loss_fn(out, base_y)
-        return loss_fn(out.squeeze(), base_y)
+        return loss_fn(out.squeeze() if 1 in out.shape else out, base_y)
 
     def run_train_step(self, base_input, ablation_input, loss_fn, optimizer):
         args = self.training_args
diff --git a/iit_amd/ops/build.py b/iit_amd/ops/build.py
--- a/iit_amd/ops/build.py
+++ b/iit_amd/ops/build.py
@@ -10,9 +10,9 @@
 OUT_DIR = os.path.join(ROOT, "iit_amd", "_native")
 LIB = os.path.join(OUT_DIR, "libiit_hip.so")
 OBJ_CACHE = os.path.join(ROOT, "build", "objcache")
-SOURCES = ["gemm.hip", "gemm_glds.hip", "gemm_dual.hip", "gemm_8ph.hip", "gemm_4w.hip", "conv_nhwc.hip", "kernels.hip", "attn_mfma.hip", "flash_attn.hip", "llama_ops.hip",
+SOURCES = ["gemm.hip", "gemm_glds.hip", "gemm_edge.hip", "gemm_dual.hip", "gemm_8ph.hip", "gemm_4w.hip", "conv_nhwc.hip", "kernels.hip", "attn_mfma.hip", "flash_attn.hip", "llama_ops.hip",
            "splice.hip", "ioi_hl.hip", "bn_nhwc.hip", "gemm_f32.hip"]
-EXTRA_FLAGS = {"gemm_glds.hip": ["-mllvm", "-amdgpu-mfma-vgpr-form"], "conv_nhwc.hip": ["-mllvm", "-amdgpu-mfma-vgpr-form"], "gemm_dual.hip": ["-mllvm", "-amdgpu-mfma-vgpr-form"],
+EXTRA_FLAGS = {"gemm_glds.hip": ["-mllvm", "-amdgpu-mfma-vgpr-form"], "gemm_edge.hip": ["-mllvm", "-amdgpu-mfma-vgpr-form"], "conv_nhwc.hip": ["-mllvm", "-amdgpu-mfma-vgpr-form"], "gemm_dual.hip": ["-mllvm", "-amdgpu-mfma-vgpr-form"],
                "gemm_8ph.hip": ["-mllvm", "-amdgpu-mfma-vgpr-form"]}
 HEADERS = ["common.h", "gemm_glds_body.h", "gemm_w4.h", "splice_spec.h"]
 ARCH = os.environ.get("IIT_OFFLOAD_ARCH", "gfx950")
diff --git a/iit_amd/ops/gemm_dispatch.py b/iit_amd/ops/gemm_dispatch.py
--- a/iit_amd/ops/gemm_dispatch.py
+++ b/iit_amd/ops/gemm_dispatch.py
@@ -307,6 +307,14 @@
                         K_.gemm_glds(A, B, c, M=M, N=N, K=Kd, lda=lda, ldb=ldb, ldc=ldc, mode=mode, epi=epi,
                                      bias0=bias0, resid=resid, ldr=ldr, tile=t, splits=sp, reduce=True, bsum=bs,
                                      gsq=sq)
+        if N % 128 and mode in (2, 3) and C2 is None and resid is None and aux is None and bias1 is None \
+                and csum_box is None:
+            for tile in K_.GLDS_EDGE_TILES:
+                if K_.gemm_glds_edge_ok(A, B, C, M=M, N=N, K=Kd, lda=lda, ldb=ldb, ldc=ldc, mode=mode, epi=epi,
+                                        bias0=bias0, tile=tile):
+                    calls[f"glds{tile}e"] = lambda c=C, c2=C2, c3=None, t=tile, bs=None, sq=None: \
+                        K_.gemm_glds_edge(A, B, c, M=M, N=N, K=Kd, lda=lda, ldb=ldb, ldc=ldc, mode=mode, epi=epi,
+                                          bias0=bias0, tile=t, bsum=bs, gsq=sq)
     if epi in _BLAS16_EPIS:
         calls["blas16"] = lambda c=C, c2=C2, c3=None: _blas16(A, B, c, M, N, Kd, lda, ldb, ldc, mode, epi,
                                                              bias0, resid, ldr)
@@ -360,6 +368,18 @@
 RAGGED = {}
 
 
+EDGE: Dict[Tuple, str] = {}
+
+
+def _edge_whole(rkey) -> Optional[str]:
+    name = EDGE.get(rkey)
+    if name is None:
+        name = EDGE[rkey] = _edge_table().get(repr(rkey), "")
+    if not name or re.fullmatch(r"glds\d+e", name) is None or _excluded(name, rkey):
+        return None
+    return name
+
+
 def _ragged_split(A, B, C, *, M, N, K, lda, ldb, mode, epi, C2, bias0, resid, aux, bsum=None, gsq=None):
     if epi in (K_.EPI_BF16, K_.EPI_F32_STORE, K_.EPI_F32_ACC) and N >= 4096 and N % 128:
         n0 = N // 128 * 128
@@ -415,6 +435,13 @@
                 split = RAGGED[rkey] = (None not in pieces and whole is not None and sum(pieces) < whole,
                                         whole, pieces)
             if split is not None and split[0]:
+                edge = None if _TAIL_LIBRARY else _edge_whole(rkey)
+                if edge is not None and C2 is None and resid is None and aux is None and bias1 is None:
+                    tile = int(edge[4:-1])
+                    ekw = dict(M=M, N=N, K=K, lda=lda, ldb=ldb, ldc=ldc, mode=mode, epi=epi, bias0=bias0, tile=tile)
+                    if K_.gemm_glds_edge_ok(A, B, C, **ekw):
+                        K_.gemm_glds_edge(A, B, C, bsum=bsum, gsq=gsq, **ekw)
+                        return edge
                 choice = run(bulk)
                 run(tail, tail=True)
                 return choice
@@ -632,6 +659,12 @@
 _TABLE_PATH = os.path.join(os.path.dirname(os.path.abspath(__file__)), "tuned", "gemm_decisions_gfx950.json")
 _TABLE = None
 _RAGGED_TABLE: Dict[str, bool] = {}
+_EDGE_TABLE: Dict[str, str] = {}
+
+
+def _edge_table() -> Dict[str, str]:
+    _table()
+    return _EDGE_TABLE
 
 
 def _ragged_table() -> Dict[str, bool]:
@@ -644,6 +677,7 @@
     if _TABLE is None:
         _TABLE = {}
         _RAGGED_TABLE.clear()
+        _EDGE_TABLE.clear()
         path = os.environ.get("IIT_GEMM_TABLE", _TABLE_PATH)
         if path != "0" and os.path.exists(path) and torch.cuda.is_available():
             import json
@@ -654,6 +688,7 @@
                 if data.get("arch") == arch:
                     _TABLE = dict(data.get("decisions", {}))
                     _RAGGED_TABLE.update({k: bool(v) for k, v in data.get("ragged", {}).items()})
+                    _EDGE_TABLE.update({k: str(v) for k, v in data.get("edge", {}).items()})
             except (OSError, ValueError) as e:
                 print(f"[iit] GEMM decision table not loaded ({e})")
     return _TABLE
@@ -689,7 +724,8 @@
         if torch.cuda.is_available() else None
     with open(path, "w") as f:
         json.dump({"arch": arch, "device": torch.cuda.get_device_name(0) if torch.cuda.is_available() else None,
-                   "decisions": dec, "ragged": ragged}, f, indent=0, sort_keys=True)
+                   "decisions": dec, "ragged": ragged, "edge": {repr(k): v for k, v in EDGE.items() if v}}, f,
+                  indent=0, sort_keys=True)
     return len(dec) + len(ragged)
 
 
diff --git a/iit_amd/ops/hip_kernels.py b/iit_amd/ops/hip_kernels.py
--- a/iit_amd/ops/hip_kernels.py
+++ b/iit_amd/ops/hip_kernels.py
@@ -52,6 +52,10 @@
     "iit_ce_fwd": [c_void_p, c_long, c_void_p, c_void_p, c_void_p, c_void_p, c_int, c_int, c_void_p],
     "iit_ce_bwd": [c_void_p, c_long, c_void_p, c_void_p, c_void_p, c_float, c_void_p, c_long, c_int, c_int, c_int,
                    c_void_p, c_void_p],
+    "iit_gemm_glds_edge_ok": [c_void_p] * 4 + [c_long] * 3 + [c_int] * 6,
+    "iit_gemm_glds_edge": [c_void_p] * 4 + [c_long] * 3 + [c_int] * 7 + [c_void_p, c_void_p, c_int, c_void_p],
+    "iit_gemm_edge_plan": [c_int, c_int, c_long, c_int, c_int, c_void_p],
+    "iit_ce_bwd16": [c_void_p, c_long, c_void_p, c_void_p, c_void_p, c_float, c_void_p, c_long, c_int, c_int, c_void_p],
     "iit_adam_flat": [c_void_p] * 6 + [c_int, c_void_p, c_int] + [c_float] * 6 + [c_void_p] * 3
                      + [c_void_p, c_int, c_void_p, c_void_p],
     "iit_sumsq_2d": [c_void_p, c_long, c_int, c_int, c_void_p, c_void_p],
@@ -291,6 +295,35 @@
            "iit_gemm_glds")
 
 
+GLDS_EDGE_TILES = (0, 7, 25)
+
+
+def gemm_glds_edge_ok(A, B, C, *, M, N, K, lda, ldb, ldc, mode, epi, bias0=None, tile=25) -> bool:
+    if any(t is None or not t.is_cuda or t.dtype != torch.bfloat16 for t in (A, B)):
+        return False
+    return bool(lib().iit_gemm_glds_edge_ok(_p(A), _p(B), _p(C), _p(bias0), lda, ldb, ldc, M, N, K, mode, epi, tile))
+
+
+def gemm_glds_edge(A, B, C, *, M, N, K, lda, ldb, ldc, mode, epi, bias0=None, tile=25, store_mode=None, bsum=None,
+                   gsq=None):
+    if CHECK_BOUNDS:
+        a = ("A", A, K, M, lda) if mode & MODE_AKM else ("A", A, M, K, lda)
+        _bounds("iit_gemm_glds_edge", a, ("B", B, K, (N + 7) // 8 * 8, ldb), ("C", C, M, N, ldc),
+                ("bias0", bias0, 1, N, N), ("bsum", bsum, 1, N, N))
+    sm = GLDS_STORE_MODE if store_mode is None else store_mode
+    gm = int(os.environ.get("IIT_GEMM_GROUP_M", str(GEMM_GROUP_M)) or 0)
+    _check(lib().iit_gemm_glds_edge(_p(A), _p(B), _p(C), _p(bias0), lda, ldb, ldc, M, N, K, mode, epi, tile, int(sm),
+                                    _p(bsum) if mode == 3 else None, _p(gsq) if epi == EPI_F32_STORE else None, gm,
+                                    _stream()), "iit_gemm_glds_edge")
+
+
+def gemm_edge_plan(rows: int, N: int, ld: int, elem: int, tile: int) -> Optional[dict]:
+    out = (ctypes.c_long * 6)()
+    if lib().iit_gemm_edge_plan(rows, N, ld, elem, tile, ctypes.cast(out, c_void_p)) != 0:
+        return None
+    return dict(zip(("tiles_n", "used", "redirected", "straddle", "last_byte", "valid_bytes"), list(out)))
+
+
 GEMM_F32_TILES = {0: (64, 64), 1: (128, 128)}
 
 
@@ -871,6 +904,14 @@
                             int(out.dtype == torch.bfloat16), _p(out16), _stream()), "ce_bwd")
 
 
+def ce_bwd16(logits, ld, labels, lse, gscale, inv_rows, out16, ld_out, R, V):
+    assert logits.dtype == torch.float32 and out16.dtype == torch.bfloat16 and gscale.dtype == torch.float32
+    if CHECK_BOUNDS:
+        _bounds("ce_bwd16", ("logits", logits, R, V, ld), ("out16", out16, R, ld_out, ld_out))
+    _check(lib().iit_ce_bwd16(_p(logits), ld, _p(labels), _p(lse), _p(gscale), inv_rows, _p(out16), ld_out, R, V,
+                              _stream()), "ce_bwd16")
+
+
 def colsum_accum(x, ld, out, T, N):
     if CHECK_BOUNDS:
         _bounds("colsum", ("x", x, T, N, ld), ("out", out, 1, N, N))
diff --git a/iit_amd/ops/hip_ops.py b/iit_amd/ops/hip_ops.py
--- a/iit_amd/ops/hip_ops.py
+++ b/iit_amd/ops/hip_ops.py
@@ -971,6 +971,21 @@
         return dx, None, None, None, None, gres, None
 
 
+class UnembedFn(LinearFn):
+
+    @staticmethod
+    def forward(ctx, x, W, b, w, ldw):
+        res = LinearFn.forward(ctx, x, W, b, w, ldw, None, "f32")
+        handle = torch.empty(1, dtype=BF16, device=res.device).expand(res.shape)
+        return res, handle
+
+    @staticmethod
+    def backward(ctx, gy, gh=None):
+        if gh is not None:
+            gy = gh if gy is None else gy.float() + gh.float()
+        return LinearFn.backward(ctx, gy)[:5]
+
+
 class MLPInFn(Function):
 
     @staticmethod
@@ -1111,7 +1126,7 @@
 class CrossEntropyFn(Function):
 
     @staticmethod
-    def forward(ctx, logits, labels):
+    def forward(ctx, logits, labels, handle=None):
         ctx.set_materialize_grads(False)
         R, V = logits.shape
         if logits.stride(1) != 1:
@@ -1122,27 +1137,47 @@
         lab = labels.contiguous()
         K.ce_fwd(logits, ld, lab, loss, lse, None, R, V)
         ctx.save_for_backward(logits, lab, lse)
+        ctx.only16 = handle is not None
         return loss.mean()
 
     @staticmethod
     def backward(ctx, g):
         if g is None:
-            return None, None
+            return None, None, None
         logits, lab, lse = ctx.saved_tensors
         R, V = logits.shape
         ld = logits.stride(0)
         ldo = _pad8(V)
-        buf = torch.empty(R, ldo, dtype=F32, device=logits.device)
         buf16 = torch.empty(R, ldo, dtype=BF16, device=logits.device)
         gs = g.reshape(1).float().contiguous()
+        if ctx.only16:
+            K.ce_bwd16(logits, ld, lab, lse, gs, 1.0 / R, buf16, ldo, R, V)
+            return None, None, buf16[:, :V]
+        buf = torch.empty(R, ldo, dtype=F32, device=logits.device)
         K.ce_bwd(logits, ld, lab, lse, gs, 1.0 / R, buf, ldo, R, V, out16=buf16)
         res = buf[:, :V]
         _set_bf16_twin(res, buf16[:, :V])
-        return res, None
+        return res, None, None
+
+
+def _grad16_handle(logits: torch.Tensor) -> Optional[torch.Tensor]:
+    tag = getattr(logits, "_iit_grad16", None)
+    if tag is None or tag[0] != logits.data_ptr() or tag[1] != logits._version or tag[2].shape != logits.shape:
+        return None
+    if not (torch.is_grad_enabled() and tag[2].requires_grad) or logits._backward_hooks or logits.retains_grad:
+        return None
+    if os.environ.get("IIT_CE_BF16_ONLY", "1") == "0":
+        return None
+    return tag[2]
 
 
 def cross_entropy(logits: torch.Tensor, labels: torch.Tensor) -> torch.Tensor:
-    return CrossEntropyFn.apply(logits.float(), labels)
+    logits = logits.float()
+    handle = _grad16_handle(logits) if logits.dim() == 2 else None
+    if handle is not None:
+        logits._iit_grad16 = None
+        return CrossEntropyFn.apply(logits.detach(), labels, handle)
+    return CrossEntropyFn.apply(logits, labels)
 
 
 
@@ -1632,7 +1667,11 @@
 
     def unembed(self, x, W_U, b_U):
         sh = self.shadow
-        return LinearFn.apply(x, W_U, b_U, sh.U, sh.Vp, None, "f32")
+        if sh.U is None:
+            raise RuntimeError("unembed before begin_forward(): the bf16 shadow of W_U is not bound")
+        logits, handle = UnembedFn.apply(x, W_U, b_U, sh.U, sh.Vp)
+        logits._iit_grad16 = (logits.data_ptr(), logits._version, handle)
+        return logits
 
     def unembed_argmax(self, x, W_U, b_U, chunk: int = 8192):
         sh = self.shadow
```

Result: faster. 17030 pairs/s, median of 6 (+1.4%).
